# PalamaraLab/FastSMC

Measured on AMD Instinct MI355X. Metric: haplotype-pairs decoded/sec (whole node) + GB/s vs HBM roofline, 69-state HMM, higher is better.
Workload: dtype f32; 1 GPU; synthetic 1000 haplotypes x 50000 sites, K=69, all 499500 pairs per GPU, FastSMC-mode IBD + posterior-mean/MAP ages, no hashing; mode=ibd, resident_waves=2048, n_cu=256, chunk_sites=512, chunks_per_window=98, resident_chunks=24, beta_stride=2, kernel_member=69, record_gather=none, lib_hash=5bd750a2cb04e671

## Files before the change

### fastsmc_amd/capi.py

```python
from __future__ import annotations

import ctypes as C
import os

import numpy as np

_HERE = os.path.dirname(os.path.abspath(__file__))
LIB_PATH = os.environ.get("FSMC_HIP_LIB") or os.path.join(_HERE, "libfastsmc_hip.so")

FSMC_WANT_MEAN = 1
FSMC_WANT_MAP = 2
FSMC_WANT_SUMS = 4
FSMC_WANT_MAJOR_MINOR_SUMS = 8

FSMC_EOVERFLOW = -6

SYMBOLS = [
    "fsmc_ctx_create", "fsmc_ctx_destroy", "fsmc_last_error", "fsmc_ctx_info", "fsmc_ctx_set_workspace_limit",
    "fsmc_ctx_expect_work",
    "fsmc_ctx_set_chunk_sites", "fsmc_ctx_set_beta_stride", "fsmc_ctx_last_beta_stride", "fsmc_ctx_last_plan",
    "fsmc_ctx_last_kernel", "fsmc_ctx_set_pairing", "fsmc_ctx_last_items", "fsmc_ctx_set_two_wave_windows", "fsmc_ctx_last_waves_per_window", "fsmc_ctx_last_segment_sums_in_lds", "fsmc_ctx_set_resident_chunks",
    "fsmc_ctx_last_resident_chunks",
    "fsmc_model_create", "fsmc_model_destroy", "fsmc_haps_upload", "fsmc_worklist_upload",
    "fsmc_decode_ibd_launch", "fsmc_decode_ibd_fetch", "fsmc_sync", "fsmc_last_kernel_ms", "fsmc_phase_cycles",
    "fsmc_decode_ibd",
    "fsmc_decode_posteriors", "fsmc_decode_per_pair", "fsmc_decode_sums", "fsmc_decode_sums_batches",
    "fsmc_decode_pair_posteriors", "fsmc_ctx_set_pair_posterior_slice", "fsmc_ctx_last_pair_posterior_slices",
    "fsmc_decode_pair_minima", "fsmc_ctx_set_pair_minima_slice", "fsmc_ctx_last_pair_minima_slices",
    "fsmc_decode_pair_bins", "fsmc_ctx_set_pair_bins_slice", "fsmc_ctx_last_pair_bins_slices",
    "fsmc_decode_pair_cdf", "fsmc_ctx_set_pair_cdf_slice", "fsmc_ctx_last_pair_cdf_slices",
    "fsmc_decode_pair_tail_summaries", "fsmc_ctx_set_pair_tail_slice", "fsmc_ctx_last_pair_tail_slices",
    "fsmc_decode_pair_loglik", "fsmc_ctx_set_pair_loglik_slice", "fsmc_ctx_last_pair_loglik_slices",
    "fsmc_decode_pair_viterbi", "fsmc_ctx_set_pair_viterbi_slice", "fsmc_ctx_last_pair_viterbi_slices",
    "fsmc_identify", "fsmc_identify_ex", "fsmc_identify_fetch",
]

PAIR_DTYPE = np.dtype([("hap_a", "<u4"), ("hap_b", "<u4")])
GROUP_DTYPE = np.dtype([("first_pair", "<u4"), ("n_pairs", "<u4"), ("from", "<u4"), ("to", "<u4"),
                        ("scan_from", "<u4"), ("scan_to", "<u4")])
CANDIDATE_DTYPE = np.dtype([("hap_a", "<u4"), ("hap_b", "<u4"), ("from", "<u4"), ("to", "<u4"), ("flush_word", "<u4")])
IBD_DTYPE = np.dtype([("pair", "<u4"), ("start", "<i4"), ("end", "<i4"), ("prob", "<f4"), ("post_mean", "<f4"),
                      ("map", "<f4")])


def log_likelihood(mant, expo):
    with np.errstate(divide="ignore"):
        return np.log(np.asarray(mant, np.float64)) + np.asarray(expo, np.float64) * np.log(2.0)


class FsmcError(RuntimeError):
    def __init__(self, code: int, msg: str):
        super().__init__(f"fastsmc_hip error {code}: {msg}")
        self.code = code


class _JobWindow(C.Structure):
    _fields_ = [("window_size", C.c_uint32), ("w_i", C.c_uint32), ("w_j", C.c_uint32), ("last_job", C.c_int32),
                ("j_above_diag", C.c_int32)]


class _IdentifyOpts(C.Structure):
    _fields_ = [("word_size", C.c_uint32), ("haploid", C.c_uint32), ("max_seeds", C.c_int32),
                ("read_ahead", C.c_uint32)]


class _ModelDesc(C.Structure):
    _fields_ = [
        ("K", C.c_int32), ("S", C.c_int32),
        ("pi", C.c_void_p), ("col_ratios", C.c_void_p), ("exp_times", C.c_void_p),
        ("n_rows", C.c_int32),
        ("D", C.c_void_p), ("B", C.c_void_p), ("U", C.c_void_p), ("RR", C.c_void_p),
        ("step_row", C.c_void_p),
        ("e1", C.c_void_p), ("e0m1", C.c_void_p), ("e2m0", C.c_void_p),
        ("state_threshold", C.c_uint32), ("age_threshold", C.c_uint32), ("probability_threshold", C.c_float),
        ("sequence", C.c_int32),
        ("gap_row_f", C.c_void_p), ("site_row_f", C.c_void_p), ("gap_row_b", C.c_void_p), ("site_row_b", C.c_void_p),
        ("hom", C.c_void_p),
    ]


_lib = None


def load():
    global _lib
    if _lib is None:
        if not os.path.exists(LIB_PATH):
            raise FsmcError(-100, f"{LIB_PATH} is missing: build it with `python -c 'import __graft_entry__ as g; "
                                  "g.build()'` (there is no CPU fallback)")
        L = C.CDLL(LIB_PATH)
        vp, i32, u32, u64, sz = C.c_void_p, C.c_int32, C.c_uint32, C.c_uint64, C.c_size_t
        L.fsmc_ctx_create.argtypes = [C.c_int, vp, C.POINTER(vp)]
        L.fsmc_ctx_destroy.argtypes = [vp]
        L.fsmc_ctx_destroy.restype = None
        L.fsmc_last_error.argtypes = [vp]
        L.fsmc_last_error.restype = C.c_char_p
        L.fsmc_ctx_info.argtypes = [vp, C.POINTER(i32), C.POINTER(i32), C.POINTER(u64)]
        L.fsmc_ctx_set_workspace_limit.argtypes = [vp, u64]
        L.fsmc_ctx_expect_work.argtypes = [vp, C.c_double, C.c_int32]
        L.fsmc_ctx_set_chunk_sites.argtypes = [vp, u32]
        L.fsmc_ctx_set_beta_stride.argtypes = [vp, u32]
        L.fsmc_ctx_last_beta_stride.argtypes = [vp, C.POINTER(i32)]
        L.fsmc_ctx_last_plan.argtypes = [vp, C.POINTER(i32), C.POINTER(i32), C.POINTER(i32)]
        L.fsmc_ctx_last_kernel.argtypes = [vp, C.POINTER(i32)]
        L.fsmc_ctx_set_pairing.argtypes = [vp, u32]
        L.fsmc_ctx_set_two_wave_windows.argtypes = [vp, u32]
        L.fsmc_ctx_last_waves_per_window.argtypes = [vp, C.POINTER(i32)]
        L.fsmc_ctx_last_items.argtypes = [vp, C.POINTER(i32)]
        L.fsmc_ctx_last_segment_sums_in_lds.argtypes = [vp, C.POINTER(i32)]
        L.fsmc_model_create.argtypes = [vp, C.POINTER(_ModelDesc), C.POINTER(vp)]
        L.fsmc_model_destroy.argtypes = [vp]
        L.fsmc_model_destroy.restype = None
        L.fsmc_haps_upload.argtypes = [vp, vp, u32, u32]
        L.fsmc_worklist_upload.argtypes = [vp, vp, sz, vp, sz]
        L.fsmc_decode_ibd_launch.argtypes = [vp, vp, u32]
        L.fsmc_decode_ibd_fetch.argtypes = [vp, vp, sz, C.POINTER(sz)]
        L.fsmc_sync.argtypes = [vp]
        L.fsmc_last_kernel_ms.argtypes = [vp, C.POINTER(C.c_float)]
        L.fsmc_phase_cycles.argtypes = [vp, vp, sz]
        L.fsmc_decode_ibd.argtypes = [vp, vp, vp, sz, vp, sz, u32, vp, sz, C.POINTER(sz)]
        L.fsmc_decode_posteriors.argtypes = [vp, vp, vp, sz]
        L.fsmc_decode_per_pair.argtypes = [vp, vp, vp, vp, vp]
        L.fsmc_decode_pair_posteriors.argtypes = [vp, vp, vp, vp, vp]
        L.fsmc_ctx_set_pair_posterior_slice.argtypes = [vp, u32]
        L.fsmc_ctx_last_pair_posterior_slices.argtypes = [vp, C.POINTER(i32)]
        L.fsmc_decode_pair_minima.argtypes = [vp, vp, vp, u64, vp, vp, vp, vp]
        L.fsmc_ctx_set_pair_minima_slice.argtypes = [vp, u32]
        L.fsmc_ctx_last_pair_minima_slices.argtypes = [vp, C.POINTER(i32)]
        L.fsmc_decode_pair_bins.argtypes = [vp, vp, vp, vp, sz, vp, vp, vp, vp, vp]
        L.fsmc_ctx_set_pair_bins_slice.argtypes = [vp, u32]
        L.fsmc_ctx_last_pair_bins_slices.argtypes = [vp, C.POINTER(i32)]
        L.fsmc_decode_pair_cdf.argtypes = [vp, vp, vp, sz, vp, vp, sz, vp]
        L.fsmc_ctx_set_pair_cdf_slice.argtypes = [vp, u32]
        L.fsmc_ctx_last_pair_cdf_slices.argtypes = [vp, C.POINTER(i32)]
        L.fsmc_decode_pair_tail_summaries.argtypes = [vp, vp, vp, sz, vp, vp, sz, vp, vp, vp]
        L.fsmc_ctx_set_pair_tail_slice.argtypes = [vp, u32]
        L.fsmc_ctx_last_pair_tail_slices.argtypes = [vp, C.POINTER(i32)]
        L.fsmc_decode_pair_loglik.argtypes = [vp, vp, vp, sz, vp, vp, vp, vp]
        L.fsmc_ctx_set_pair_loglik_slice.argtypes = [vp, u32]
        L.fsmc_ctx_last_pair_loglik_slices.argtypes = [vp, C.POINTER(i32)]
        L.fsmc_decode_pair_viterbi.argtypes = [vp, vp, vp, vp, vp]
        L.fsmc_ctx_set_pair_viterbi_slice.argtypes = [vp, u32]
        L.fsmc_ctx_last_pair_viterbi_slices.argtypes = [vp, C.POINTER(i32)]
        L.fsmc_decode_sums.argtypes = [vp, vp, vp, vp, vp, vp]
        L.fsmc_decode_sums_batches.argtypes = [vp, vp, vp, sz, vp, vp, vp, vp]
        L.fsmc_identify.argtypes = [vp, vp, u32, u32, vp, C.POINTER(_JobWindow), vp, u32, i32, C.c_float, C.c_float, vp,
                                    sz, C.POINTER(sz)]
        L.fsmc_identify_ex.argtypes = [vp, vp, u32, u32, vp, C.POINTER(_JobWindow), vp, u32, i32, C.c_float, C.c_float,
                                       C.POINTER(_IdentifyOpts), vp, sz, C.POINTER(sz)]
        L.fsmc_identify_fetch.argtypes = [vp, vp, sz, C.POINTER(sz)]
        _lib = L
    return _lib


def _p(a):
    return None if a is None else a.ctypes.data_as(C.c_void_p)


def whole_sequence_groups(n_pairs: int, S: int, batch: int = 64) -> np.ndarray:
    n_groups = (n_pairs + batch - 1) // batch
    g = np.zeros(n_groups, GROUP_DTYPE)
    g["first_pair"] = np.arange(n_groups, dtype=np.uint64) * batch
    g["n_pairs"] = np.minimum(batch, n_pairs - g["first_pair"].astype(np.int64))
    g["from"] = 0
    g["to"] = S
    g["scan_from"] = 0
    g["scan_to"] = S
    return g


class Context:

    def __init__(self, device: int = 0, stream: int | None = None):
        self._L = load()
        h = C.c_void_p()
        rc = self._L.fsmc_ctx_create(device, C.c_void_p(stream) if stream else None, C.byref(h))
        if rc != 0:
            raise FsmcError(rc, (self._L.fsmc_last_error(None) or b"").decode())
        self._h = h
        self._models = []

    def _check(self, rc: int):
        if rc != 0:
            raise FsmcError(rc, (self._L.fsmc_last_error(self._h) or b"").decode())

    def close(self):
        if getattr(self, "_h", None):
            for m in list(self._models):
                m.close()
            self._L.fsmc_ctx_destroy(self._h)
            self._h = None

    def __del__(self):
        try:
            self.close()
        except Exception:
            pass

    def info(self) -> dict:
        cu, slots, hbm = C.c_int32(), C.c_int32(), C.c_uint64()
        self._check(self._L.fsmc_ctx_info(self._h, C.byref(cu), C.byref(slots), C.byref(hbm)))
        chunk, chunks = C.c_int32(), C.c_int32()
        self._check(self._L.fsmc_ctx_last_plan(self._h, C.byref(chunk), C.byref(chunks), None))
        return {"n_cu": cu.value, "n_slots": slots.value, "hbm_bytes": hbm.value, "chunk_sites": chunk.value,
                "max_chunks": chunks.value}

    def set_chunk_sites(self, sites: int):
        self._check(self._L.fsmc_ctx_set_chunk_sites(self._h, sites))

    def set_resident_chunks(self, chunks: int):
        self._check(self._L.fsmc_ctx_set_resident_chunks(self._h, chunks))

    def last_resident_chunks(self) -> int:
        v = C.c_int32(0)
        self._check(self._L.fsmc_ctx_last_resident_chunks(self._h, C.byref(v)))
        return v.value

    def set_beta_stride(self, stride: int):
        self._check(self._L.fsmc_ctx_set_beta_stride(self._h, stride))

    def last_beta_stride(self) -> int:
        v = C.c_int32(0)
        self._check(self._L.fsmc_ctx_last_beta_stride(self._h, C.byref(v)))
        return v.value

    def last_kernel(self) -> int:
        v = C.c_int32(0)
        self._check(self._L.fsmc_ctx_last_kernel(self._h, C.byref(v)))
        return v.value

    def set_two_wave_windows(self, mode: int):
        self._check(self._L.fsmc_ctx_set_two_wave_windows(self._h, mode))

    def last_waves_per_window(self) -> int:
        v = C.c_int32(0)
        self._check(self._L.fsmc_ctx_last_waves_per_window(self._h, C.byref(v)))
        return v.value

    def set_pairing(self, mode: int):
        self._check(self._L.fsmc_ctx_set_pairing(self._h, mode))

    def last_items(self) -> int:
        v = C.c_int32(0)
        self._check(self._L.fsmc_ctx_last_items(self._h, C.byref(v)))
        return v.value

    def last_segment_sums_in_lds(self) -> bool:
        v = C.c_int32(0)
        self._check(self._L.fsmc_ctx_last_segment_sums_in_lds(self._h, C.byref(v)))
        return bool(v.value)

    def set_workspace_limit(self, nbytes: int):
        self._check(self._L.fsmc_ctx_set_workspace_limit(self._h, nbytes))

    def expect_work(self, pair_sites: float, states: int):
        self._check(self._L.fsmc_ctx_expect_work(self._h, float(pair_sites), int(states)))

    def create_model(self, pm) -> "Model":
        return Model(self, pm)

    def upload_haps(self, bits: np.ndarray, n_sites: int):
        b = np.ascontiguousarray(bits, dtype=np.uint64)
        assert b.ndim == 2 and b.shape[1] == (n_sites + 63) // 64
        self._check(self._L.fsmc_haps_upload(self._h, _p(b), b.shape[0], n_sites))

    def upload_worklist(self, pairs: np.ndarray, groups: np.ndarray):
        pr = np.ascontiguousarray(pairs, dtype=PAIR_DTYPE)
        gr = np.ascontiguousarray(groups, dtype=GROUP_DTYPE)
        self._check(self._L.fsmc_worklist_upload(self._h, _p(pr), pr.size, _p(gr), gr.size))
        self._n_pairs = pr.size
        self._groups = gr

    def decode_ibd_launch(self, model: "Model", flags: int = FSMC_WANT_MEAN | FSMC_WANT_MAP):
        self._check(self._L.fsmc_decode_ibd_launch(self._h, model._h, flags))

    def decode_ibd_fetch(self) -> np.ndarray:
        cap = max(1024, 4 * getattr(self, "_n_pairs", 256))
        while True:
            out = np.zeros(cap, IBD_DTYPE)
            n = C.c_size_t()
            rc = self._L.fsmc_decode_ibd_fetch(self._h, _p(out), cap, C.byref(n))
            if rc == FSMC_EOVERFLOW:
                cap = int(n.value)
                continue
            self._check(rc)
            return out[: n.value]

    def sync(self):
        self._check(self._L.fsmc_sync(self._h))

    def last_kernel_ms(self) -> float:
        ms = C.c_float()
        self._check(self._L.fsmc_last_kernel_ms(self._h, C.byref(ms)))
        return float(ms.value)

    def phase_cycles(self) -> np.ndarray:
        out = np.zeros(128, np.uint64)
        if self._L.fsmc_phase_cycles(self._h, _p(out), 128) != 0:
            self._check(self._L.fsmc_phase_cycles(self._h, _p(out), 32))
        return out

    def decode_ibd(self, model: "Model", pairs, groups, flags: int = FSMC_WANT_MEAN | FSMC_WANT_MAP) -> np.ndarray:
        self.upload_worklist(pairs, groups)
        self.decode_ibd_launch(model, flags)
        return self.decode_ibd_fetch()

    def identify(self, words, global_ids, gen_pos, *, window_size=0, w_i=1, w_j=1, last_job=True, j_above_diag=False,
                 gap=1, skip=0.0, min_m=1.0, word_size=64, haploid=True, max_seeds=0, read_ahead=10) -> np.ndarray:
        w = np.ascontiguousarray(words, np.uint64)
        if w.ndim != 2:
            raise ValueError("words must be [n_haps][n_words]")
        ids = np.ascontiguousarray(global_ids, np.uint32)
        gen = np.ascontiguousarray(gen_pos, np.float32)
        if ids.shape != (w.shape[0],):
            raise ValueError("global_ids must have one entry per haplotype")
        jw = _JobWindow(window_size, w_i, w_j, int(bool(last_job)), int(bool(j_above_diag)))
        opts = _IdentifyOpts(word_size, int(bool(haploid)), max_seeds, read_ahead)
        cap = max(1024, 4 * w.shape[0])
        while True:
            out = np.zeros(cap, CANDIDATE_DTYPE)
            n = C.c_size_t(0)
            rc = self._L.fsmc_identify_ex(self._h, _p(w), w.shape[0], w.shape[1], _p(ids), C.byref(jw), _p(gen),
                                          gen.size, gap, skip, min_m, C.byref(opts), _p(out), cap, C.byref(n))
            if rc == -6:
                cap = int(n.value)
                out = np.zeros(cap, CANDIDATE_DTYPE)
                if self._L.fsmc_identify_fetch(self._h, _p(out), cap, C.byref(n)) == 0:
                    return out[:n.value]
                continue
            self._check(rc)
            return out[:n.value]

    def decode_per_pair(self, model: "Model", exp_coal_times, want_mean=True, want_map=True):
        et = np.ascontiguousarray(exp_coal_times, np.float32)
        mean = np.zeros((self._n_pairs, model.S), np.float32) if want_mean else None
        mp = np.zeros((self._n_pairs, model.S), np.int32) if want_map else None
        self._check(self._L.fsmc_decode_per_pair(self._h, model._h, _p(et), _p(mean), _p(mp)))
        return mean, mp

    def decode_pair_posteriors(self, model: "Model", exp_coal_times, want_rows=True, sum_into=None, rows_out=None):
        et = np.ascontiguousarray(exp_coal_times, np.float32)
        if et.shape != (model.K,):
            raise ValueError(f"exp_coal_times: shape {et.shape}, expected {(model.K,)}")
        rows = ptrs = None
        if rows_out is not None:
            rows = rows_out
            if len(rows) != self._n_pairs:
                raise ValueError("rows_out needs one array per pair of the work list")
            for r in rows:
                if r.dtype != np.float32 or not r.flags.c_contiguous or not r.flags.writeable or r.size != model.K * model.S:
                    raise ValueError("rows_out: writable C-contiguous float32 arrays of K * S values")
            ptrs = (C.c_void_p * self._n_pairs)(*[r.ctypes.data for r in rows])
        elif want_rows:
            rows = np.zeros((self._n_pairs, model.K, model.S), np.float32)
            ptrs = (C.c_void_p * self._n_pairs)(*[rows.ctypes.data + i * rows.strides[0] for i in range(self._n_pairs)])
        if sum_into is not None:
            if (sum_into.dtype != np.float32 or not sum_into.flags.c_contiguous or not sum_into.flags.writeable
                    or sum_into.shape != (model.K, model.S)):
                raise ValueError("sum_into: a writable C-contiguous float32 array [K][S]")
        self._check(self._L.fsmc_decode_pair_posteriors(self._h, model._h, _p(et), ptrs, _p(sum_into)))
        return rows, sum_into

    def set_pair_posterior_slice(self, groups: int):
        self._check(self._L.fsmc_ctx_set_pair_posterior_slice(self._h, groups))

    def last_pair_posterior_slices(self) -> int:
        v = C.c_int32(0)
        self._check(self._L.fsmc_ctx_last_pair_posterior_slices(self._h, C.byref(v)))
        return v.value

# ... 265 lines not shown
```

### fastsmc_amd/csrc/fsmc_capi.hip

```cpp
#include <hip/hip_runtime.h>

#include <algorithm>
#include <chrono>
#include <cmath>
#include <cstdio>
#include <cstdlib>
#include <cstring>
#include <new>
#include <string>
#include <type_traits>
#include <vector>

#include "fsmc_identify.h"
#include "fsmc_instances.h"
#include "fsmc_pair_bins.h"
#include "fsmc_pair_cdf.h"
#include "fsmc_pair_tail.h"
#include "fsmc_pair_minima.h"
#include "fsmc_pair_posteriors.h"

namespace fsmc
{
hipError_t idSortCandidates(hipStream_t stream, const fsmc_candidate* in, fsmc_candidate* sorted, unsigned n,
                            unsigned nHaps, unsigned nWords);
hipError_t idSeedDepths(hipStream_t stream, const unsigned long long* words, unsigned nHaps, unsigned nWords,
                        unsigned maxSeeds, unsigned readAhead, unsigned char* depthOut,
                        unsigned hapStride);
}

using namespace fsmc;

namespace fsmc
{
__global__ void add_planes_in_order_kernel(const float* __restrict__ planes, float* __restrict__ acc, size_t n,
                                           int nPlanes, size_t planeStride)
{
  for (size_t i = (size_t)blockIdx.x * blockDim.x + threadIdx.x; i < n; i += (size_t)gridDim.x * blockDim.x) {
    float s = acc[i];
    for (int sl = 0; sl < nPlanes; ++sl) {
      s = s + planes[(size_t)sl * planeStride + i];
    }
    acc[i] = s;
  }
}
}

namespace
{
thread_local std::string g_createError;

struct DevBuf {
  void* p = nullptr;
  size_t bytes = 0;
};

enum PairSlicing {
  kSlicePosteriors,
  kSliceMinima,
  kSliceBins,
  kSliceCdf,
  kSliceTail,
  kSliceLoglik,
  kSliceViterbi,
  kPairSlicings
};
}

struct fsmc_ctx {
  int device = 0;
  hipStream_t stream = nullptr;
  bool ownStream = false;
  int nCU = 0;
  uint64_t hbmBytes = 0;
  uint64_t wsLimit = 0;
  double wsEarned = 0;
  double wsAnnounced = 0;
  double wsAnnouncedCredit = 0;
  std::string err;

  unsigned long long* dHaps = nullptr;
  uint32_t nHaps = 0, nSites = 0, W = 0;

  fsmc_pair* dPairs = nullptr;
  fsmc_group* dGroups = nullptr;
  size_t nPairs = 0, nGroups = 0;
  std::vector<fsmc_pair> hPairs;
  std::vector<fsmc_group> hGroups;

  unsigned* dCounters = nullptr;
  unsigned long long* dPhase = nullptr;
  DevBuf ws;
  DevBuf recs;
  size_t recCap = 0;
  DevBuf aux;
  DevBuf out;

  hipEvent_t ev0 = nullptr, ev1 = nullptr;
  bool timed = false;
  int lastSlots = 0;
  int lastChunk = 0, lastMaxChunks = 0, lastResident = 0;
  int residentChunks = -1;
  uint32_t chunkSites = 0;
  uint32_t betaStride = 0;
  int lastStride = 1;
  bool lastSpsLds = false;
  int lastMember = 0;

  struct IbdQueues {
    uint64_t serial = 0;
    uint64_t maxLen = 0;
    uint64_t maxLenAlone = 0;
    uint32_t pairing = 0;
    bool valid = false;
    bool dual = false;
    bool reordered = false;
    bool alone = false;
    std::vector<fsmc_group> items, unions, rest;
  } q;
  uint64_t worklistSerial = 0;
  fsmc_group* dItems = nullptr;
  fsmc_group* dRest = nullptr;
  uint32_t pairing = 1;
  int lastItems = 0;
  unsigned twoWaves = 0;
  int lastWavesPerWindow = 1;
  hipStream_t side = nullptr;
  hipEvent_t evFork = nullptr, evJoin = nullptr;
  DevBuf wsSide;

  struct {
    uint32_t groups = 0;
    int last = 0;
  } pairSlices[kPairSlicings];
  DevBuf ppStage;
  DevBuf ppRows;
  DevBuf ppAcc;
  hipStream_t copyStream = nullptr;
  void* ppPinned[2] = {nullptr, nullptr};
  size_t ppPinnedBytes = 0;
  hipEvent_t evRows = nullptr, evCopied[2] = {nullptr, nullptr};
  DevBuf pmAcc;
  DevBuf pbAcc;
  DevBuf pcSpec;
  DevBuf plAcc;
  DevBuf pvAcc;
  DevBuf ptAcc;

  DevBuf idStash;
  size_t idStashCount = 0;

  const fsmc_model* ibdModel = nullptr;
  uint32_t ibdFlags = 0;
  bool ibdPending = false;
};

struct fsmc_model {
  fsmc_ctx* ctx = nullptr;
  int K = 0, KP = 0, S = 0, nRows = 0;
  int w2NW = 0;
  float *pi = nullptr, *cR = nullptr, *expT = nullptr;
  float *D = nullptr, *B = nullptr, *U = nullptr, *RR = nullptr;
  float* rowSets = nullptr;
  float* ghostMask = nullptr;
  int* stepRow = nullptr;
  bool sequence = false;
  int *rowGapF = nullptr, *rowSiteB = nullptr, *rowGapB = nullptr;
  float4* emis3 = nullptr;
  unsigned stateThr = 0, ageThr = 0;
  float probThr = 0.f;
};

namespace
{

std::vector<std::string> mappedHipRuntimes()
{
  std::vector<std::string> found;
  if (FILE* f = std::fopen("/proc/self/maps", "r")) {
    char line[4096];
    while (std::fgets(line, sizeof(line), f)) {
      const char* slash = std::strchr(line, '/');
      if (!slash || !std::strstr(slash, "libamdhip64.so")) {
        continue;
      }
      std::string path(slash);
      while (!path.empty() && (path.back() == '\n' || path.back() == ' ')) {
        path.pop_back();
      }
      if (std::find(found.begin(), found.end(), path) == found.end()) {
        found.push_back(path);
      }
    }
    std::fclose(f);
  }
  return found;
}

int fail(fsmc_ctx* ctx, int code, const std::string& msg)
{
  if (ctx) {
    ctx->err = msg;
  } else {
    g_createError = msg;
  }
  return code;
}

#define FSMC_HIP(ctx, call)                                                                                            \
  do {                                                                                                                 \
    hipError_t e_ = (call);                                                                                            \
    if (e_ != hipSuccess) {                                                                                            \
      return fail((ctx), FSMC_EHIP, std::string(#call) + ": " + hipGetErrorString(e_));                                \
    }                                                                                                                  \
  } while (0)

#define FSMC_TRY(call)                                                                                                 \
  do {                                                                                                                 \
    const int rc_ = (call);                                                                                            \
    if (rc_ != FSMC_OK) {                                                                                              \
      return rc_;                                                                                                      \
    }                                                                                                                  \
  } while (0)

int ensure(fsmc_ctx* ctx, DevBuf& b, size_t bytes)
{
  if (b.bytes >= bytes && b.p) {
    return FSMC_OK;
  }
  if (b.p) {
    (void)hipFree(b.p);
    b.p = nullptr;
    b.bytes = 0;
  }
  if (bytes == 0) {
    bytes = 16;
  }
  const bool timing = bytes >= (256u << 20) && std::getenv("FSMC_HOST_TIMING") != nullptr;
  const auto t0 = std::chrono::steady_clock::now();
  hipError_t e = hipMalloc(&b.p, bytes);
  if (e != hipSuccess) {
    b.p = nullptr;
    return fail(ctx, FSMC_ENOMEM, "hipMalloc of " + std::to_string(bytes) + " bytes failed: " + hipGetErrorString(e));
  }
  if (timing) {
    std::fprintf(stderr, "[fsmc] hipMalloc of %.2f GB took %.3f s\n", (double)bytes / 1e9,
                 std::chrono::duration<double>(std::chrono::steady_clock::now() - t0).count());
  }
  b.bytes = bytes;
  return FSMC_OK;
}

template <typename T> int upload(fsmc_ctx* ctx, T** dst, const T* src, size_t n)
{
// ... 1 lines not shown
    (void)hipFree(*dst);
    *dst = nullptr;
  }
  hipError_t e = hipMalloc((void**)dst, std::max<size_t>(n, 1) * sizeof(T));
  if (e != hipSuccess) {
    *dst = nullptr;
    return fail(ctx, FSMC_ENOMEM, std::string("hipMalloc failed: ") + hipGetErrorString(e));
  }
  if (n) {
    FSMC_HIP(ctx, hipMemcpyAsync(*dst, src, n * sizeof(T), hipMemcpyHostToDevice, ctx->stream));
    FSMC_HIP(ctx, hipStreamSynchronize(ctx->stream));
  }
  return FSMC_OK;
}

std::vector<float> padRows(const float* src, size_t rows, int K, int KP)
{
  std::vector<float> out(rows * (size_t)KP, 0.f);
  for (size_t r = 0; r < rows; ++r) {
    std::memcpy(&out[r * KP], src + r * K, sizeof(float) * (size_t)K);
  }
  return out;
}

using KernelFn = void (*)(const KParams);

int familyMember(const fsmc_model* m)
{
  if (exactMember(m->K)) {
    return m->K;
  }
  return (m->K <= 128 && m->KP % kKPad == 0 && m->KP <= 128) ? m->KP : 0;
}

template <int KT> KernelFn pickMember(int mode, bool track, bool seq, bool half, bool dual = false)
{
  if constexpr (KT > 0 && halfBuilt(KT)) {
    if (dual && half && mode == kModeIbd && !seq) {
      return track ? decode_kernel<KT, kModeIbd, true, false, true, true>
                   : decode_kernel<KT, kModeIbd, false, false, true, true>;
    }
  }
  if constexpr (KT > 0) {
    if (dual && mode == kModeIbd && !seq) {
      return track ? decode_kernel<KT, kModeIbd, true, false, false, true>
                   : decode_kernel<KT, kModeIbd, false, false, false, true>;
    }
  }
  switch (mode) {
  case kModeIbd:
    if constexpr (halfBuilt(KT)) {
      if (half && !seq) {
        return track ? decode_kernel<KT, kModeIbd, true, false, true> : decode_kernel<KT, kModeIbd, false, false, true>;
      }
    }
    if (seq) {
      return track ? decode_kernel<KT, kModeIbd, true, true, false> : decode_kernel<KT, kModeIbd, false, true, false>;
    }
    return track ? decode_kernel<KT, kModeIbd, true, false, false> : decode_kernel<KT, kModeIbd, false, false, false>;
  case kModeDump:
    return seq ? decode_kernel<KT, kModeDump, false, true, false> : decode_kernel<KT, kModeDump, false, false, false>;
  case kModePerPair:
    return seq ? decode_kernel<KT, kModePerPair, false, true, false>
               : decode_kernel<KT, kModePerPair, false, false, false>;
  case kModeSums:
    if constexpr (halfSumsBuilt(KT)) {
      if (half && !seq) {
        return decode_kernel<KT, kModeSums, false, false, true>;
      }
    }
    return seq ? decode_kernel<KT, kModeSums, false, true, false> : decode_kernel<KT, kModeSums, false, false, false>;
  default:
    return nullptr;
  }
}

bool waveGroups(int mode, const fsmc_model* m)
{
  return m->w2NW > 0 && (mode == kModeIbd || mode == kModeDump || mode == kModeSums || mode == kModePerPair);
}

struct W2Member {
  int NW, KH;
};
W2Member w2Member(int K)
{
  if (const char* v = std::getenv("FSMC_DIAG_W2_MEMBER")) {
    int nw = 0, kh = 0;
    if (std::sscanf(v, "%dx%d", &nw, &kh) == 2 && nw * kh >= K &&
        ((nw - 1) * kh < K || (kh == 48 && 2 * kh < K) || (nw * kh > 512 && (nw - 2) * kh < K))) {
#define FSMC_IS_W2(KHX, NWX)                                                                                            \
  if (kh == KHX && nw == NWX) {                                                                                        \
    return {nw, kh};                                                                                                   \
  }
      FSMC_ALL_W2(FSMC_IS_W2)
#undef FSMC_IS_W2
    }
  }
  if (K <= 192) return {4, 48};
  if (K <= 256) return {4, 64};
  if (K <= 320) return {4, 80};
  if (K <= 384) return {6, 64};
  if (K <= 448) return {7, 64};
  if (K <= 512) return {8, 64};
  if (K <= 640) return {8, 80};
  if (K <= 768) return {8, 96};
  return {8, 128};
}

template <int KH, int NW, bool SEQ> KernelFn pickWaveGroupKernelOf(int mode, bool track)
{
  if (mode == kModeIbd) {
    return track ? decode_kernel_w2<KH, kModeIbd, true, SEQ, NW> : decode_kernel_w2<KH, kModeIbd, false, SEQ, NW>;
  }
  if (mode == kModeSums) {
    return decode_kernel_w2<KH, kModeSums, false, SEQ, NW>;
  }
  if (mode == kModePerPair) {
    return decode_kernel_w2<KH, kModePerPair, false, SEQ, NW>;
  }
  return decode_kernel_w2<KH, kModeDump, false, SEQ, NW>;
}
template <int KH, int NW> KernelFn pickWaveGroupKernel(int mode, bool track, bool seq)
{
  return seq ? pickWaveGroupKernelOf<KH, NW, true>(mode, track) : pickWaveGroupKernelOf<KH, NW, false>(mode, track);
}

bool anyStates(const fsmc_model* m)
{
  return m->K > kMaxStatesW2;
}

template <bool SEQ> KernelFn pickAnyKernel(int mode, bool track)
{
  switch (mode) {
  case kModeIbd:
    return track ? decode_kernel_any<kModeIbd, true, SEQ> : decode_kernel_any<kModeIbd, false, SEQ>;
  case kModeDump:
    return decode_kernel_any<kModeDump, false, SEQ>;
  case kModePerPair:
    return decode_kernel_any<kModePerPair, false, SEQ>;
  case kModeSums:
    return decode_kernel_any<kModeSums, false, SEQ>;
  default:
    return nullptr;
  }
}

struct KernelChoice {
  KernelFn fn = nullptr;
  unsigned threads = kWave;
  int member = 0;
  int stride = 1;
};

KernelChoice chooseKernel(const fsmc_model* m, int mode, bool track, bool dual, uint32_t wantStride)
{
  KernelChoice k;
  if (anyStates(m)) {
    k.fn = m->sequence ? pickAnyKernel<true>(mode, track) : pickAnyKernel<false>(mode, track);
    return k;
  }
  if (waveGroups(mode, m)) {
    const int NW = m->w2NW, KH = m->KP / NW;
    k.threads = (unsigned)(NW * kWave);
    k.member = NW == kW2NW ? 1000 + KH : 1000 * NW + KH;
#define FSMC_PICK_W2(KHX, NWX)                                                                                          \
  if (KH == KHX && NW == NWX) {                                                                                        \
    k.fn = pickWaveGroupKernel<KHX, NWX>(mode, track, m->sequence != 0);                                               \
  }
    FSMC_ALL_W2(FSMC_PICK_W2)
#undef FSMC_PICK_W2
    return k;
  }
  k.member = familyMember(m);
  const bool half = wantStride != 1 && !m->sequence &&
                    ((mode == kModeIbd && halfBuilt(k.member)) || (mode == kModeSums && halfSumsBuilt(k.member)));
  k.stride = half ? 2 : 1;
  switch (k.member) {
#define FSMC_PICK_CASE(KTX)                                                                                             \
  case KTX:                                                                                                            \
    k.fn = pickMember<KTX>(mode, track, m->sequence, half, dual);                                                      \
    break;
    FSMC_ALL_KT(FSMC_PICK_CASE)
    FSMC_EXACT_KT(FSMC_PICK_CASE)
#undef FSMC_PICK_CASE
  default:
    break;
  }
  return k;
}

template <int KT> KernelFn pickBidirMember(int mode)
{
  switch (mode) {
  case kModeDump:
    return decode_kernel_bidir<KT, kModeDump>;
  case kModePerPair:
    return decode_kernel_bidir<KT, kModePerPair>;
  case kModeSums:
    return decode_kernel_bidir<KT, kModeSums>;
  default:
    return nullptr;
  }
}
KernelChoice chooseTwoWaveKernel(const fsmc_model* m, int mode)
{
  KernelChoice k{nullptr, 2 * kWave, familyMember(m), 1};
  if (m->sequence || anyStates(m) || waveGroups(mode, m)) {
    return k;
  }
  switch (k.member) {
#define FSMC_PICK_BIDIR(KTX)                                                                                            \
  case KTX:                                                                                                            \
    k.fn = pickBidirMember<KTX>(mode);                                                                                 \
    break;
    FSMC_ALL_KT(FSMC_PICK_BIDIR)
    FSMC_EXACT_KT(FSMC_PICK_BIDIR)
#undef FSMC_PICK_BIDIR
  default:
    break;
  }
  return k;
}

template <typename Params> struct SweepKernel {
  KernelChoice k;
  void (*fn)(const Params) = nullptr;
};
template <typename Params, typename Pick> SweepKernel<Params> chooseSweepKernel(const fsmc_model* m, Pick pick)
{
  SweepKernel<Params> s;
  s.k = KernelChoice{nullptr, kWave, m->K <= 128 ? familyMember(m) : 0, 1};
  switch (s.k.member) {
#define FSMC_PICK_SWEEP(KTX)                                                                                            \
  case KTX:                                                                                                            \
    s.fn = pick(std::integral_constant<int, KTX>{});                                                                   \
    break;
    FSMC_ALL_KT(FSMC_PICK_SWEEP)
    FSMC_EXACT_KT(FSMC_PICK_SWEEP)
#undef FSMC_PICK_SWEEP
  default:
    break;
  }
  s.k.fn = reinterpret_cast<KernelFn>(s.fn);
  return s;
}

size_t loweredByEnv(const char* name, size_t value, int divisor = 1)
{
  const char* s = std::getenv(name);
  const long v = s ? std::atol(s) / divisor : 0;
  return v >= 1 && (size_t)v < value ? (size_t)v : value;
}

hipError_t workgroupsPerCU(const KernelChoice& k, int most, int capDivisor, int& perCU)
{
  perCU = 0;
  const hipError_t e = hipOccupancyMaxActiveBlocksPerMultiprocessor(&perCU, k.fn, (int)k.threads, 0);
  if (e != hipSuccess) {
    (void)hipGetLastError();
    return e;
  }
  perCU = std::min(perCU, most);
  if (capDivisor > 0) {
    perCU = (int)loweredByEnv("FSMC_DIAG_WAVES_PER_CU", (size_t)std::max(perCU, 0), capDivisor);
  }
  return hipSuccess;
}

struct LaunchPlan {
  KernelChoice k;
  int chunk = 0;
  int chunkRows = 0;
  int maxChunks = 0;
  int residentChunks = 0;
  size_t wsSlot = 0;
  int slots = 0;
  int wavesPerWindow = 1;
  size_t bytes = 0;
};

constexpr double kAllocBytesPerSecond = 25e9;
constexpr double kEarnFraction = 0.06;
constexpr uint64_t kFreeWorkspace = 24ull << 30;

struct WsBudget {
  uint64_t hard, soft;
};

uint64_t freeWorkspace()
{
  if (const char* v = std::getenv("FSMC_DIAG_WS_FREE")) {
    return std::strtoull(v, nullptr, 10);
  }
  return kFreeWorkspace;
}

WsBudget workspaceBudget(const fsmc_ctx* ctx, const DevBuf& cur)
{
  size_t freeB = 0, totalB = 0;
  const bool known = hipMemGetInfo(&freeB, &totalB) == hipSuccess;
  const uint64_t reachable = (uint64_t)freeB + cur.bytes;
  const uint64_t margin = (uint64_t)(0.04 * (double)ctx->hbmBytes);
  if (ctx->wsLimit) {
    uint64_t lim = ctx->wsLimit;
    if (known && reachable > margin && reachable - margin < lim && reachable - margin >= lim / 4) {
      lim = reachable - margin;
    }
    return {lim, lim};
  }
  const uint64_t floor40 = (uint64_t)(0.40 * (double)ctx->hbmBytes);
  uint64_t hard = floor40;
  if (known) {
    const uint64_t want = (uint64_t)(0.80 * (double)ctx->hbmBytes);
    hard = std::max<uint64_t>(floor40, std::min<uint64_t>(want, reachable > margin ? reachable - margin : 0));
  }
  uint64_t earned = (uint64_t)std::min(std::max(ctx->wsEarned, 0.0), 1e15);
  if (earned < hard && earned < 2 * (uint64_t)cur.bytes) {
    earned = 0;
  }
  const uint64_t freeBytes = freeWorkspace();
  const uint64_t soft = std::min<uint64_t>(hard, std::max<uint64_t>({(uint64_t)cur.bytes, earned, freeBytes}));
  return {hard, soft};
}

void payForWorkspace(fsmc_ctx* ctx, uint64_t allocatedBytes)
{
  if (ctx->wsLimit) {
    return;
  }
  const uint64_t freeBytes = freeWorkspace();
  if (allocatedBytes > freeBytes) {
    ctx->wsEarned = std::max(0.0, ctx->wsEarned - (double)(allocatedBytes - freeBytes));
  }
}

double earnScale()
{
  if (const char* v = std::getenv("FSMC_DIAG_WS_EARN_SCALE")) {
    return std::atof(v);
  }
  return 1.0;
}

void earnWorkspace(fsmc_ctx* ctx, const fsmc_model* m, int mode)
{
  double pairSites = 0;
  for (const fsmc_group& g : ctx->hGroups) {
    const uint32_t aEnd = (mode == kModeIbd) ? g.scan_to : g.to;
    pairSites += (double)g.n_pairs * (double)(aEnd > g.from ? aEnd - g.from : 0);
  }
  double seconds = pairSites * (8.0 * m->K + 0.25) / (0.8 * 8e12);
  const double announced = std::min(ctx->wsAnnounced, seconds);
  if (ctx->wsAnnounced > 0) {
    ctx->wsAnnouncedCredit *= (ctx->wsAnnounced - announced) / ctx->wsAnnounced;
  }
  ctx->wsAnnounced -= announced;
  seconds -= announced;
  ctx->wsEarned += earnScale() * kEarnFraction * seconds * kAllocBytesPerSecond;
}

int planOneWave(const fsmc_ctx* ctx, const fsmc_model* m, int mode, const KernelChoice& k,
                const std::vector<fsmc_group>& list, bool paired, const WsBudget& budget, unsigned share,
                LaunchPlan& plan, std::string& why)
{
  if (!k.fn) {
    why = "no kernel for this model";
    return FSMC_EUNSUPPORTED;
  }
  int perCU = 0;
  const hipError_t e = workgroupsPerCU(k, anyStates(m) ? 4 : 8, 1, perCU);
  if (e != hipSuccess) {
    why = std::string("occupancy query of the decode kernel: ") + hipGetErrorString(e);
    return FSMC_EHIP;
  }
  const bool w2 = waveGroups(mode, m);
  const size_t slots = std::max<size_t>(1, std::min((size_t)ctx->nCU * std::max(perCU, 1), list.size()));
  size_t L = 1;
  for (const fsmc_group& g : list) {
    const size_t aEnd = (mode == kModeIbd) ? g.scan_to : g.to;
    L = std::max<size_t>(L, aEnd - g.from);
  }
  const size_t K4 = w2 ? (size_t)m->KP / 4 : (size_t)((k.member > 0 ? k.member : m->K) + 3) / 4 + (anyStates(m) ? 1 : 0);
  const size_t vecBytes = K4 * kWave * sizeof(float4);
  const uint64_t limit = budget.hard / share;
  const bool half = k.stride == 2;
  auto chunkRows = [&](size_t c) { return half ? (c + 1) / 2 : c; };
  const size_t rowsAvail = (size_t)(limit / (vecBytes * slots));
  const size_t rowsSoft = (size_t)(budget.soft / share / (vecBytes * slots));
  const size_t sideRows = anyStates(m) ? (size_t)kAnyExtraRows + 2 : 4;
  const size_t defaultChunk = std::max<size_t>((size_t)std::ceil(std::sqrt((double)L)), w2 ? 2048 : 512);
  size_t C, maxChunks;
  if (chunkRows(L) + sideRows + 1 <= rowsAvail && (chunkRows(L) + sideRows + 1 <= rowsSoft || L <= defaultChunk) &&
      !(ctx->chunkSites && ctx->chunkSites < L)) {
    C = L;
    maxChunks = 1;
  } else {
    C = ctx->chunkSites ? (size_t)ctx->chunkSites : defaultChunk;
    C = std::min((C + 15) / 16 * 16, (L + 15) / 16 * 16);
    auto fits = [&](size_t c) { return chunkRows(c) + (L + c - 1) / c + sideRows + 1 <= rowsAvail; };
    if (!ctx->chunkSites) {
      while (C > 16 && !fits(C)) {
        C = std::max<size_t>(16, (C / 2 + 15) / 16 * 16);
      }
    }
    maxChunks = (L + C - 1) / C;
    if (!fits(C)) {
      why = "workspace limit too small for the decode window";
      return FSMC_ENOMEM;
    }
  }
  size_t resident = 0;
  if (maxChunks > 1 && (mode == kModeIbd || mode == kModeSums) && !m->sequence && !paired && !anyStates(m) &&
      (!w2 || w2ResidentBuilt(m->w2NW, false)) &&
      ctx->residentChunks != 0) {
    const size_t rowsBudget = rowsSoft;
    const size_t fixed = chunkRows(C) + maxChunks + sideRows;
    if (rowsBudget > fixed) {
      resident = std::min<size_t>((rowsBudget - fixed) / chunkRows(C), maxChunks);
      if (ctx->residentChunks > 0) {
        resident = std::min<size_t>(resident, (size_t)ctx->residentChunks);
      }
    }
  }
  plan.chunk = (int)C;
  plan.chunkRows = (int)chunkRows(C);
  plan.maxChunks = (int)maxChunks;
  plan.residentChunks = (int)resident;
  plan.wsSlot = (chunkRows(C) * (1 + resident) + maxChunks + 2 + (sideRows - 2)) * K4 * kWave;
  plan.slots = (int)slots;
  plan.k = k;
  plan.wavesPerWindow = 1;
  plan.bytes = plan.wsSlot * sizeof(float4) * slots;
  return FSMC_OK;
}

int planViterbi(const fsmc_ctx* ctx, const fsmc_model* m, const KernelChoice& k, size_t nGroups, bool wantStates,
                const WsBudget& budget, LaunchPlan& plan, std::string& why)
{
  int perCU = 0;
  const hipError_t e = workgroupsPerCU(k, 8, 1, perCU);
  if (e != hipSuccess) {
    why = std::string("occupancy query of the Viterbi kernel: ") + hipGetErrorString(e);
    return FSMC_EHIP;
  }
  size_t slots = std::max<size_t>(1, std::min((size_t)ctx->nCU * (size_t)std::max(perCU, 1), nGroups));
  const size_t L = (size_t)m->S;
  const size_t K4 = (size_t)(k.member + 3) / 4;
  const size_t psiRow = K4 * kWave * sizeof(uint32_t), ckptRow = K4 * kWave * sizeof(float4);
  auto slotBytes = [&](size_t c) { return c * psiRow + (L + c - 1) / c * ckptRow; };
  size_t C = L, bytes = psiRow;
  if (wantStates) {
    size_t cMin = std::min(L, std::max<size_t>(1, (size_t)std::ceil(2.0 * std::sqrt((double)L))));
    if (ctx->chunkSites) {
      cMin = std::min<size_t>(ctx->chunkSites, L);
    }
    slots = std::min<size_t>(slots, (size_t)(budget.hard / slotBytes(cMin)));
    if (slots == 0) {
      why = "workspace limit too small for the back-pointers of one wave";
      return FSMC_ENOMEM;
    }
    if (ctx->chunkSites) {
      C = cMin;
    } else {
      const uint64_t room = L <= 512 ? budget.hard : budget.soft;
      while (C > cMin && (uint64_t)slots * slotBytes(C) > room) {
        C = std::max(cMin, (C + 1) / 2);
      }
    }
    bytes = slotBytes(C);
  }
  plan = LaunchPlan();
  plan.k = k;
  plan.chunk = (int)C;
  plan.chunkRows = (int)C;
  plan.maxChunks = (int)((L + C - 1) / C);
  plan.wsSlot = bytes / sizeof(float4);
  plan.slots = (int)slots;
  plan.wavesPerWindow = 1;
  plan.bytes = bytes * slots;
  return FSMC_OK;
}

bool twoWavesWanted(const fsmc_ctx* ctx, const KernelChoice& k2, size_t nItems)
{
  if (ctx->twoWaves == 1 || nItems == 0 || !k2.fn) {
    return false;
  }
  if (const char* v = std::getenv("FSMC_DIAG_TWO_WAVE_WINDOWS")) {
    if (std::strcmp(v, "never") == 0) {
      return false;
    }
  }
  int perCU = 0;
  return workgroupsPerCU(k2, 4, 2, perCU) == hipSuccess && perCU >= 1 && nItems <= (size_t)ctx->nCU * perCU;
}

bool planTwoWaves(const fsmc_ctx* ctx, const KernelChoice& k2, size_t nItems, const WsBudget& budget, LaunchPlan& plan)
{
  size_t L = 1;
  for (const fsmc_group& g : ctx->hGroups) {
    L = std::max<size_t>(L, g.to - g.from);
  }
  const size_t K4 = (size_t)(k2.member + 3) / 4;
  plan = LaunchPlan();
  plan.k = k2;
  plan.chunk = (int)L;
  plan.chunkRows = (int)L;
  plan.maxChunks = 1;
  plan.wsSlot = L * K4 * kWave;
  plan.slots = (int)nItems;
  plan.wavesPerWindow = 2;
  plan.bytes = plan.wsSlot * sizeof(float4) * nItems;
  return plan.bytes <= budget.hard && (plan.bytes <= budget.soft || L <= 512);
}

int holdWorkspace(fsmc_ctx* ctx, DevBuf& buf, size_t bytes)
{
  const char* most = std::getenv("FSMC_DIAG_WS_ALLOC_MAX");
  if (most && bytes > std::strtoull(most, nullptr, 10) && !(buf.p && buf.bytes >= bytes)) {
    if (buf.p) {
      (void)hipFree(buf.p);
    }
    buf = DevBuf();
    return fail(ctx, FSMC_ENOMEM, "workspace of " + std::to_string(bytes) + " bytes refused (FSMC_DIAG_WS_ALLOC_MAX)");
  }
  const size_t held = buf.bytes;
  const int rc = ensure(ctx, buf, bytes);
  if (rc != FSMC_OK) {
    (void)hipGetLastError();
  } else if (buf.bytes != held) {
    payForWorkspace(ctx, buf.bytes);
  }
  return rc;
}

int planAndHold(fsmc_ctx* ctx, const fsmc_model* m, int mode, const KernelChoice& k, const std::vector<fsmc_group>& list,
                bool paired, unsigned share, DevBuf& buf, LaunchPlan& plan)
{
  std::string why;
  const int rc = planOneWave(ctx, m, mode, k, list, paired, workspaceBudget(ctx, buf), share, plan, why);
  return rc != FSMC_OK ? fail(ctx, rc, why) : holdWorkspace(ctx, buf, plan.bytes);
}

void recordLaunch(fsmc_ctx* ctx, const KernelChoice& k, const LaunchPlan& plan, int slotsBeside = 0)
{
  ctx->lastMember = k.member;
  ctx->lastStride = k.stride;
  ctx->lastChunk = plan.chunk;
  ctx->lastMaxChunks = plan.maxChunks;
  ctx->lastResident = plan.residentChunks;
  ctx->lastWavesPerWindow = plan.wavesPerWindow;
  ctx->lastSlots = plan.slots + slotsBeside;
}

int checkReady(fsmc_ctx* ctx, const fsmc_model* m)
{
  if (!ctx || !m) {
    return fail(ctx, FSMC_EINVAL, "null context or model");
  }
  if (m->ctx != ctx) {
    return fail(ctx, FSMC_EINVAL, "model belongs to another context");
  }
  if (!ctx->dHaps) {
    return fail(ctx, FSMC_ESTATE, "no haplotypes uploaded (fsmc_haps_upload)");
  }
  if (!ctx->dPairs || !ctx->dGroups || ctx->nGroups == 0) {
    return fail(ctx, FSMC_ESTATE, "no work list uploaded (fsmc_worklist_upload)");
  }
  if ((uint32_t)m->S != ctx->nSites) {
    return fail(ctx, FSMC_EINVAL, "model has " + std::to_string(m->S) + " sites but haplotypes have " +
                                      std::to_string(ctx->nSites));
  }
  for (const fsmc_pair& pr : ctx->hPairs) {
    if (pr.hap_a >= ctx->nHaps || pr.hap_b >= ctx->nHaps) {
      return fail(ctx, FSMC_EINVAL, "pair refers to a haplotype row outside the uploaded matrix");
    }
  }
  for (const fsmc_group& g : ctx->hGroups) {
    if (g.to > (uint32_t)m->S) {
      return fail(ctx, FSMC_EINVAL, "group window exceeds the number of sites");
    }
  }
  if (m->K > kMaxStatesAny) {
    return fail(ctx, FSMC_EUNSUPPORTED, "more than " + std::to_string(kMaxStatesAny) + " states");
  }
  return FSMC_OK;
}

void fillParams(const fsmc_ctx* ctx, const fsmc_model* m, const LaunchPlan& plan, uint32_t flags, KParams& p)
{
  std::memset(&p, 0, sizeof(p));
  p.K = m->K;
  p.KP = m->KP;
  p.S = m->S;
  p.W = (int)ctx->W;
  p.nGroups = (int)ctx->nGroups;
  p.chunk = plan.chunk;
  p.chunkRows = plan.chunkRows;
  p.maxChunks = plan.maxChunks;
  p.residentChunks = plan.residentChunks;
  p.flags = flags;
  p.pi = m->pi;
  p.cR = m->cR;
  p.expT = m->expT;
  p.D = m->D;
  p.B = m->B;
  p.U = m->U;
  p.rowSets = m->rowSets;
  p.RR = m->RR;
  p.ghostMask = m->ghostMask;
  p.stepRow = m->stepRow;
  p.rowGapF = m->rowGapF;
  p.rowSiteB = m->rowSiteB;
  p.rowGapB = m->rowGapB;
  p.emis3 = m->emis3;
  p.haps = ctx->dHaps;
  p.pairs = ctx->dPairs;
  p.groups = ctx->dGroups;
  p.counters = ctx->dCounters;
  p.phaseCycles = ctx->dPhase;
  p.ws = (float4*)ctx->ws.p;
  p.wsSlot = plan.wsSlot;
  p.stateThr = m->stateThr;
  p.ageThr = m->ageThr;
  p.spsLds = 0u;
  p.thr[0] = 1000 * m->probThr;
  p.thr[1] = 100 * m->probThr;
  p.thr[2] = 10 * m->probThr;
  p.thr[3] = m->probThr;
  p.recs = (fsmc_ibd_record*)ctx->recs.p;
  p.recCap = (unsigned)ctx->recCap;
}

int checkWorkspace(fsmc_ctx* ctx, const KParams& p, int slots)
{
  const DevBuf& buf = p.ws == (float4*)ctx->wsSide.p ? ctx->wsSide : ctx->ws;
  if (!p.ws || p.ws != (float4*)buf.p || slots < 1 || buf.bytes / sizeof(float4) / (size_t)slots < p.wsSlot) {
    return fail(ctx, FSMC_ESTATE, "the workspace does not hold the launch planned for it");
  }
  return FSMC_OK;
}

int launch(fsmc_ctx* ctx, const KernelChoice& k, const KParams& p, int slots, size_t dynLds = 0, bool continues = false)
{
  if (checkWorkspace(ctx, p, slots) != FSMC_OK) {
    return FSMC_ESTATE;
  }
  FSMC_HIP(ctx, hipMemsetAsync(ctx->dCounters, 0, 4 * sizeof(unsigned), ctx->stream));
  if (!continues) {
    FSMC_HIP(ctx, hipEventRecord(ctx->ev0, ctx->stream));
  }
  hipLaunchKernelGGL(k.fn, dim3((unsigned)slots), dim3(k.threads), dynLds, ctx->stream, p);
  FSMC_HIP(ctx, hipGetLastError());
  FSMC_HIP(ctx, hipEventRecord(ctx->ev1, ctx->stream));
  ctx->timed = true;
  return FSMC_OK;
}

int launchBeside(fsmc_ctx* ctx, const KernelChoice& kSide, KParams& pSide, int slotsSide, const KernelChoice& kMain,
                 KParams& pMain, int slotsMain)
{
  if (checkWorkspace(ctx, pSide, slotsSide) != FSMC_OK || checkWorkspace(ctx, pMain, slotsMain) != FSMC_OK) {
    return FSMC_ESTATE;
  }
  FSMC_HIP(ctx, hipMemsetAsync(ctx->dCounters, 0, 4 * sizeof(unsigned), ctx->stream));
  FSMC_HIP(ctx, hipEventRecord(ctx->ev0, ctx->stream));
  FSMC_HIP(ctx, hipEventRecord(ctx->evFork, ctx->stream));
  FSMC_HIP(ctx, hipStreamWaitEvent(ctx->side, ctx->evFork, 0));
  pMain.groupBase = 0;
  pSide.groupBase = 2;
  hipLaunchKernelGGL(kSide.fn, dim3((unsigned)slotsSide), dim3(kSide.threads), 0, ctx->side, pSide);
  FSMC_HIP(ctx, hipGetLastError());
  hipLaunchKernelGGL(kMain.fn, dim3((unsigned)slotsMain), dim3(kMain.threads), 0, ctx->stream, pMain);
  FSMC_HIP(ctx, hipGetLastError());
  FSMC_HIP(ctx, hipEventRecord(ctx->evJoin, ctx->side));
  FSMC_HIP(ctx, hipStreamWaitEvent(ctx->stream, ctx->evJoin, 0));
  FSMC_HIP(ctx, hipEventRecord(ctx->ev1, ctx->stream));
  ctx->timed = true;
  return FSMC_OK;
}

uint64_t stagingLimit(const fsmc_ctx* ctx, uint64_t held, unsigned parts)
{
  uint64_t limit = ctx->wsLimit ? ctx->wsLimit : (uint64_t)(0.25 * (double)ctx->hbmBytes);
  size_t freeB = 0, totalB = 0;
  if (hipMemGetInfo(&freeB, &totalB) == hipSuccess) {
    const uint64_t room = (uint64_t)freeB + held;
    const uint64_t reserve = 2ull << 30;
    limit = std::min<uint64_t>(limit, room > reserve ? (room - reserve) / parts : 0);
  }
  return limit;
}

int ensureRowCopies(fsmc_ctx* ctx, size_t need)
{
  if (ctx->ppPinnedBytes < need) {
    for (int i = 0; i < 2; ++i) {
      if (ctx->ppPinned[i]) {
        (void)hipHostFree(ctx->ppPinned[i]);
        ctx->ppPinned[i] = nullptr;
      }
    }
    ctx->ppPinnedBytes = 0;
    for (int i = 0; i < 2; ++i) {
      const hipError_t e = hipHostMalloc(&ctx->ppPinned[i], need, hipHostMallocDefault);
      if (e != hipSuccess) {
        ctx->ppPinned[i] = nullptr;
        return fail(ctx, FSMC_ENOMEM, std::string("hipHostMalloc of the row buffers failed: ") + hipGetErrorString(e));
      }
    }
    ctx->ppPinnedBytes = need;
  }
  if (!ctx->copyStream) {
    FSMC_HIP(ctx, hipStreamCreateWithFlags(&ctx->copyStream, hipStreamNonBlocking));
    FSMC_HIP(ctx, hipEventCreateWithFlags(&ctx->evRows, hipEventDisableTiming));
    FSMC_HIP(ctx, hipEventCreateWithFlags(&ctx->evCopied[0], hipEventDisableTiming));
    FSMC_HIP(ctx, hipEventCreateWithFlags(&ctx->evCopied[1], hipEventDisableTiming));
  }
  return FSMC_OK;
}

int prepareDecode(fsmc_ctx* ctx, const fsmc_model* m, int mode, uint32_t wantStride,
                  const std::vector<fsmc_group>& list, size_t nItems, size_t stagingPerItem, LaunchPlan& plan)
{
  const KernelChoice k = chooseKernel(m, mode, false, false, wantStride);
  earnWorkspace(ctx, m, mode);
  int rc = planAndHold(ctx, m, mode, k, list, false, 1, ctx->ws, plan);
  if (rc != FSMC_OK) {
    return rc;
  }
  size_t staged = nItems;
  if (stagingPerItem) {
    staged = std::max<size_t>(1, (size_t)(stagingLimit(ctx, ctx->out.bytes, 1) / stagingPerItem));
    staged = loweredByEnv("FSMC_DIAG_SUMS_SLOTS", staged);
    plan.slots = (int)std::min({(size_t)plan.slots, nItems, staged});
  }
  const KernelChoice k2 = chooseTwoWaveKernel(m, mode);
  LaunchPlan plan2;
  if (staged >= nItems && twoWavesWanted(ctx, k2, nItems) &&
      planTwoWaves(ctx, k2, nItems, workspaceBudget(ctx, ctx->ws), plan2)) {
    if (holdWorkspace(ctx, ctx->ws, plan2.bytes) == FSMC_OK) {
      plan = plan2;
    } else {
      ctx->err.clear();
      rc = holdWorkspace(ctx, ctx->ws, plan.bytes);
      if (rc != FSMC_OK) {
        return rc;
      }
    }
  }
  recordLaunch(ctx, plan.k, plan);
  return FSMC_OK;
}

int setPairSlice(fsmc_ctx* ctx, PairSlicing kind, uint32_t groups)
{
  if (!ctx) {
    return FSMC_EINVAL;
  }
  ctx->pairSlices[kind].groups = groups;
  return FSMC_OK;
}

int lastPairSlices(const fsmc_ctx* ctx, PairSlicing kind, int32_t* slices)
{
  if (!ctx || !slices) {
    return FSMC_EINVAL;
  }
  *slices = ctx->pairSlices[kind].last;
  return FSMC_OK;
}

struct WorkSlices {
  const fsmc_ctx* ctx = nullptr;
  size_t slice = 0;
  size_t nSlices = 0;
  size_t slicePairsMax = 0;
  LaunchPlan plan;
  float* stageMean = nullptr;
  int* stageMap = nullptr;
  std::vector<size_t> hOffsets;
  std::vector<float> hCoal;

  size_t firstGroup(size_t sl) const { return sl * slice; }
  size_t groups(size_t sl) const { return std::min(slice, ctx->nGroups - sl * slice); }
  size_t firstPair(size_t sl) const { return ctx->hGroups[firstGroup(sl)].first_pair; }
  size_t pairs(size_t sl) const
  {
    const fsmc_group& last = ctx->hGroups[firstGroup(sl) + groups(sl) - 1];
    return (size_t)last.first_pair + last.n_pairs - firstPair(sl);
// ... 289 lines not shown
      return fail(nullptr, code, msg);
    }
  }
  *out = ctx;
  return FSMC_OK;
}

void fsmc_ctx_destroy(fsmc_ctx* ctx)
{
  if (!ctx) {
    return;
  }
  (void)hipSetDevice(ctx->device);
  if (ctx->stream) {
    (void)hipStreamSynchronize(ctx->stream);
  }
  if (ctx->dHaps) (void)hipFree(ctx->dHaps);
  if (ctx->dPairs) (void)hipFree(ctx->dPairs);
  if (ctx->dGroups) (void)hipFree(ctx->dGroups);
  if (ctx->dItems) (void)hipFree(ctx->dItems);
  if (ctx->dRest) (void)hipFree(ctx->dRest);
  if (ctx->dCounters) (void)hipFree(ctx->dCounters);
  if (ctx->dPhase) (void)hipFree(ctx->dPhase);
  if (ctx->idStash.p) (void)hipFree(ctx->idStash.p);
  if (ctx->ws.p) (void)hipFree(ctx->ws.p);
  if (ctx->recs.p) (void)hipFree(ctx->recs.p);
  if (ctx->aux.p) (void)hipFree(ctx->aux.p);
  if (ctx->out.p) (void)hipFree(ctx->out.p);
  if (ctx->ev0) (void)hipEventDestroy(ctx->ev0);
  if (ctx->ev1) (void)hipEventDestroy(ctx->ev1);
  if (ctx->evFork) (void)hipEventDestroy(ctx->evFork);
  if (ctx->evJoin) (void)hipEventDestroy(ctx->evJoin);
  if (ctx->side) (void)hipStreamDestroy(ctx->side);
  if (ctx->wsSide.p) (void)hipFree(ctx->wsSide.p);
  if (ctx->copyStream) (void)hipStreamSynchronize(ctx->copyStream);
  if (ctx->ppStage.p) (void)hipFree(ctx->ppStage.p);
  if (ctx->ppRows.p) (void)hipFree(ctx->ppRows.p);
  if (ctx->pcSpec.p) (void)hipFree(ctx->pcSpec.p);
  if (ctx->ptAcc.p) (void)hipFree(ctx->ptAcc.p);
  if (ctx->ppAcc.p) (void)hipFree(ctx->ppAcc.p);
  if (ctx->pmAcc.p) (void)hipFree(ctx->pmAcc.p);
  if (ctx->pbAcc.p) (void)hipFree(ctx->pbAcc.p);
  if (ctx->plAcc.p) (void)hipFree(ctx->plAcc.p);
  if (ctx->pvAcc.p) (void)hipFree(ctx->pvAcc.p);
  for (int i = 0; i < 2; ++i) {
    if (ctx->ppPinned[i]) (void)hipHostFree(ctx->ppPinned[i]);
    if (ctx->evCopied[i]) (void)hipEventDestroy(ctx->evCopied[i]);
  }
  if (ctx->evRows) (void)hipEventDestroy(ctx->evRows);
  if (ctx->copyStream) (void)hipStreamDestroy(ctx->copyStream);
  if (ctx->ownStream && ctx->stream) (void)hipStreamDestroy(ctx->stream);
  delete ctx;
}

int fsmc_ctx_info(const fsmc_ctx* ctx, int32_t* n_cu, int32_t* n_slots, uint64_t* hbm_bytes)
{
  if (!ctx) {
    return FSMC_EINVAL;
  }
  if (n_cu) *n_cu = ctx->nCU;
  if (n_slots) *n_slots = ctx->lastSlots;
  if (hbm_bytes) *hbm_bytes = ctx->hbmBytes;
  return FSMC_OK;
}

int fsmc_ctx_set_workspace_limit(fsmc_ctx* ctx, uint64_t bytes)
{
  if (!ctx) {
    return FSMC_EINVAL;
  }
  ctx->wsLimit = bytes;
  return FSMC_OK;
}

int fsmc_ctx_expect_work(fsmc_ctx* ctx, double pair_sites, int32_t states)
{
  if (!ctx) {
    return fail(nullptr, FSMC_EINVAL, "null context");
  }
  if (!(pair_sites >= 0) || states < 1) {
    return fail(ctx, FSMC_EINVAL, "expected work: pair-sites >= 0 and states >= 1");
  }
  if (pair_sites == 0) {
    ctx->wsEarned = std::max(0.0, ctx->wsEarned - ctx->wsAnnouncedCredit);
    ctx->wsAnnounced = 0;
    ctx->wsAnnouncedCredit = 0;
    return FSMC_OK;
  }
  const double seconds = pair_sites * (8.0 * states + 0.25) / (0.8 * 8e12);
  const double credit = std::min(earnScale() * kEarnFraction * seconds * kAllocBytesPerSecond,
                                 std::max(0.0, (double)ctx->hbmBytes - ctx->wsAnnouncedCredit));
  ctx->wsAnnounced += seconds;
  ctx->wsAnnouncedCredit += credit;
  ctx->wsEarned += credit;
  return FSMC_OK;
}

int fsmc_ctx_set_chunk_sites(fsmc_ctx* ctx, uint32_t sites)
{
  if (!ctx) {
    return FSMC_EINVAL;
  }
  ctx->chunkSites = sites;
  return FSMC_OK;
}

int fsmc_ctx_set_beta_stride(fsmc_ctx* ctx, uint32_t stride)
{
  if (!ctx || stride > 2) {
    return fail(ctx, FSMC_EINVAL, "beta stride must be 0 (automatic), 1 or 2");
  }
  ctx->betaStride = stride;
  return FSMC_OK;
}

int fsmc_ctx_last_beta_stride(const fsmc_ctx* ctx, int32_t* stride)
{
  if (!ctx || !stride) {
    return FSMC_EINVAL;
  }
  *stride = ctx->lastStride;
  return FSMC_OK;
}

int fsmc_ctx_last_plan(const fsmc_ctx* ctx, int32_t* chunk_sites, int32_t* max_chunks, int32_t* n_slots)
{
  if (!ctx) {
    return FSMC_EINVAL;
  }
  if (chunk_sites) *chunk_sites = ctx->lastChunk;
  if (max_chunks) *max_chunks = ctx->lastMaxChunks;
  if (n_slots) *n_slots = ctx->lastSlots;
  return FSMC_OK;
}

int fsmc_ctx_set_resident_chunks(fsmc_ctx* ctx, int32_t chunks)
{
  if (!ctx || chunks < -1) {
    return fail(ctx, FSMC_EINVAL, "resident chunks: -1 (automatic), 0 (none) or a count");
  }
  ctx->residentChunks = chunks;
  return FSMC_OK;
}

int fsmc_ctx_last_resident_chunks(const fsmc_ctx* ctx, int32_t* chunks)
{
  if (!ctx || !chunks) {
    return FSMC_EINVAL;
  }
  *chunks = ctx->lastResident;
  return FSMC_OK;
}

int fsmc_ctx_set_pair_posterior_slice(fsmc_ctx* ctx, uint32_t groups) { return setPairSlice(ctx, kSlicePosteriors, groups); }
int fsmc_ctx_last_pair_posterior_slices(const fsmc_ctx* ctx, int32_t* slices) { return lastPairSlices(ctx, kSlicePosteriors, slices); }
int fsmc_ctx_set_pair_minima_slice(fsmc_ctx* ctx, uint32_t groups) { return setPairSlice(ctx, kSliceMinima, groups); }
int fsmc_ctx_last_pair_minima_slices(const fsmc_ctx* ctx, int32_t* slices) { return lastPairSlices(ctx, kSliceMinima, slices); }
int fsmc_ctx_set_pair_bins_slice(fsmc_ctx* ctx, uint32_t groups) { return setPairSlice(ctx, kSliceBins, groups); }
int fsmc_ctx_last_pair_bins_slices(const fsmc_ctx* ctx, int32_t* slices) { return lastPairSlices(ctx, kSliceBins, slices); }
int fsmc_ctx_set_pair_cdf_slice(fsmc_ctx* ctx, uint32_t groups) { return setPairSlice(ctx, kSliceCdf, groups); }
int fsmc_ctx_last_pair_cdf_slices(const fsmc_ctx* ctx, int32_t* slices) { return lastPairSlices(ctx, kSliceCdf, slices); }
int fsmc_ctx_set_pair_tail_slice(fsmc_ctx* ctx, uint32_t groups) { return setPairSlice(ctx, kSliceTail, groups); }
int fsmc_ctx_last_pair_tail_slices(const fsmc_ctx* ctx, int32_t* slices) { return lastPairSlices(ctx, kSliceTail, slices); }
int fsmc_ctx_set_pair_loglik_slice(fsmc_ctx* ctx, uint32_t groups) { return setPairSlice(ctx, kSliceLoglik, groups); }
int fsmc_ctx_last_pair_loglik_slices(const fsmc_ctx* ctx, int32_t* slices) { return lastPairSlices(ctx, kSliceLoglik, slices); }
int fsmc_ctx_set_pair_viterbi_slice(fsmc_ctx* ctx, uint32_t groups) { return setPairSlice(ctx, kSliceViterbi, groups); }
int fsmc_ctx_last_pair_viterbi_slices(const fsmc_ctx* ctx, int32_t* slices) { return lastPairSlices(ctx, kSliceViterbi, slices); }

int fsmc_ctx_last_kernel(const fsmc_ctx* ctx, int32_t* member)
{
  if (!ctx || !member) {
    return FSMC_EINVAL;
  }
  *member = ctx->lastMember;
  return FSMC_OK;
}

int fsmc_model_create(fsmc_ctx* ctx, const fsmc_model_desc* d, fsmc_model** out)
{
  if (!ctx || !d || !out) {
    return fail(ctx, FSMC_EINVAL, "null argument");
  }
  *out = nullptr;
  if (d->K < 2 || d->S < 1 || d->n_rows < 1) {
    return fail(ctx, FSMC_EINVAL, "need K >= 2, S >= 1, n_rows >= 1");
  }
  if (d->K > kMaxStatesAny) {
    return fail(ctx, FSMC_EUNSUPPORTED, "more than " + std::to_string(kMaxStatesAny) + " states");
  }
  if (!d->pi || !d->col_ratios || !d->exp_times || !d->D || !d->B || !d->U || !d->RR || !d->step_row || !d->e1 ||
      !d->e0m1 || !d->e2m0) {
    return fail(ctx, FSMC_EINVAL, "null table pointer in model description");
  }
  if (d->state_threshold > (uint32_t)d->K || d->age_threshold > (uint32_t)d->K) {
    return fail(ctx, FSMC_EINVAL, "state/age threshold larger than K");
  }
  const bool seq = d->sequence != 0;
  if (seq && (!d->gap_row_f || !d->site_row_f || !d->gap_row_b || !d->site_row_b || !d->hom)) {
    return fail(ctx, FSMC_EINVAL, "sequence mode needs gap_row_f, site_row_f, gap_row_b, site_row_b and hom");
  }
  const int32_t* rowArrays[5] = {d->step_row, seq ? d->gap_row_f : nullptr, seq ? d->site_row_f : nullptr,
                                 seq ? d->gap_row_b : nullptr, seq ? d->site_row_b : nullptr};
  static const char* const rowNames[5] = {"step_row", "gap_row_f", "site_row_f", "gap_row_b", "site_row_b"};
  for (int a = 0; a < 5; ++a) {
    for (int32_t s = 1; rowArrays[a] && s < d->S; ++s) {
      if (rowArrays[a][s] < 0 || rowArrays[a][s] >= d->n_rows) {
        return fail(ctx, FSMC_EINVAL,
                    std::string(rowNames[a]) + "[" + std::to_string(s) + "] outside the transition tables");
      }
    }
  }
  FSMC_HIP(ctx, hipSetDevice(ctx->device));
  fsmc_model* m = new (std::nothrow) fsmc_model();
  if (!m) {
    return fail(ctx, FSMC_ENOMEM, "host allocation failed");
  }
  m->ctx = ctx;
  m->K = d->K;
  m->KP = (d->K + kKPad - 1) / kKPad * kKPad;
  if (d->K > 128 && d->K <= kMaxStatesW2) {
    const W2Member w = w2Member(d->K);
    m->w2NW = w.NW;
    m->KP = w.NW * w.KH;
  }
  m->S = d->S;
  m->nRows = d->n_rows;
  m->stateThr = d->state_threshold;
  m->ageThr = d->age_threshold;
  m->probThr = d->probability_threshold;
  const int K = m->K, KP = m->KP;
  int rc = FSMC_OK;
  auto up = [&](float** dst, const float* src, size_t rows) {
    if (rc == FSMC_OK) {
      std::vector<float> padded = padRows(src, rows, K, KP);
      rc = upload(ctx, dst, padded.data(), padded.size());
    }
  };
  up(&m->pi, d->pi, 1);
  up(&m->cR, d->col_ratios, 1);
  up(&m->expT, d->exp_times, 1);
  up(&m->D, d->D, (size_t)d->n_rows);
  up(&m->B, d->B, (size_t)d->n_rows);
  up(&m->U, d->U, (size_t)d->n_rows);
  up(&m->RR, d->RR, (size_t)d->n_rows);
  if (rc == FSMC_OK) {
    const size_t n = (size_t)d->n_rows;
    std::vector<float> rs(n * kRowSetParts * (size_t)KP, 0.f);
    for (size_t r = 0; r < n; ++r) {
      float* q = &rs[r * kRowSetParts * KP];
      for (int k = 0; k < K; ++k) {
        q[kRowD * KP + k] = d->D[r * K + k];
        q[kRowB * KP + k] = d->B[r * K + k];
        q[kRowU * KP + k] = d->U[r * K + k];
        q[kRowRR * KP + k] = d->RR[r * K + k];
        if (k >= 1) {
          q[kRowUsh * KP + k] = d->U[r * K + (k - 1)];
        }
      }
    }
    rc = upload(ctx, &m->rowSets, rs.data(), rs.size());
  }
  if (rc == FSMC_OK) {
    std::vector<float> mask((size_t)KP, 0.f);
    std::fill(mask.begin(), mask.begin() + K, 1.0f);
    rc = upload(ctx, &m->ghostMask, mask.data(), mask.size());
  }
  m->sequence = seq;
  auto upRows = [&](int** dst, const int32_t* src) {
    if (rc == FSMC_OK) {
      std::vector<int> rows(src, src + d->S);
      rows[0] = 0;
      rc = upload(ctx, dst, rows.data(), rows.size());
    }
  };
  upRows(&m->stepRow, seq ? d->site_row_f : d->step_row);
  if (seq) {
    upRows(&m->rowGapF, d->gap_row_f);
    upRows(&m->rowSiteB, d->site_row_b);
    upRows(&m->rowGapB, d->gap_row_b);
  }
  if (rc == FSMC_OK) {
    const int NC = seq ? 4 : 3;
    std::vector<float> emis((size_t)d->S * NC * KP, 0.f);
    static const float zs[3] = {0.f, 1.f, 1.f};
    static const float ts[3] = {0.f, 0.f, 1.f};
    for (int32_t s = 0; s < d->S; ++s) {
      for (int c = 0; c < 3; ++c) {
        float* dst = &emis[((size_t)s * NC + c) * KP];
        const volatile float z = zs[c];
        const volatile float t = ts[c];
        for (int k = 0; k < K; ++k) {
          const size_t i = (size_t)s * K + k;
          dst[k] = d->e1[i] + d->e0m1[i] * z + d->e2m0[i] * t;
        }
      }
      if (seq) {
        float* dst = &emis[((size_t)s * NC + 3) * KP];
        const volatile float zero = 0.f;
        for (int k = 0; k < K; ++k) {
          const float h = d->hom[(size_t)s * K + k];
          dst[k] = h + h * zero + h * zero;
        }
      }
    }
    rc = upload(ctx, (float**)&m->emis3, emis.data(), emis.size());
  }
// ... 139 lines not shown
    }
    const fsmc_group& a = groups[g];
    if (a.n_pairs <= 32 && a.to - a.from <= maxLen) {
      fsmc_group none = a;
      none.n_pairs = 0;
      items.push_back(a);
      items.push_back(none);
      unions.push_back(a);
    } else {
      rest.push_back(a);
    }
  }
  std::vector<uint32_t> order(unions.size());
  for (size_t i = 0; i < order.size(); ++i) {
    order[i] = (uint32_t)i;
  }
  std::stable_sort(order.begin(), order.end(), [&](uint32_t x, uint32_t y) {
    return unions[x].scan_to - unions[x].from > unions[y].scan_to - unions[y].from;
  });
  std::vector<fsmc_group> items2(items.size()), unions2(unions.size());
  for (size_t i = 0; i < order.size(); ++i) {
    unions2[i] = unions[order[i]];
    items2[2 * i] = items[2 * order[i]];
    items2[2 * i + 1] = items[2 * order[i] + 1];
  }
  items.swap(items2);
  unions.swap(unions2);
  return true;
}

bool longestFirst(std::vector<fsmc_group>& list)
{
  auto len = [](const fsmc_group& g) { return g.scan_to - g.from; };
  bool ordered = true;
  for (size_t i = 1; i < list.size() && ordered; ++i) {
    ordered = len(list[i]) <= len(list[i - 1]);
  }
  if (ordered) {
    return false;
  }
  std::stable_sort(list.begin(), list.end(), [&](const fsmc_group& a, const fsmc_group& b) { return len(a) > len(b); });
  return true;
}
}

int fsmc_ctx_set_pairing(fsmc_ctx* ctx, uint32_t mode)
{
  if (!ctx || mode > 1) {
    return fail(ctx, FSMC_EINVAL, "pairing must be 0 (off) or 1 (automatic)");
  }
  ctx->pairing = mode;
  return FSMC_OK;
}

int fsmc_ctx_set_two_wave_windows(fsmc_ctx* ctx, uint32_t mode)
{
  if (!ctx || mode > 1) {
    return fail(ctx, FSMC_EINVAL, "two-wave windows: 0 (automatic) or 1 (never)");
  }
  ctx->twoWaves = mode;
  return FSMC_OK;
}

int fsmc_ctx_last_waves_per_window(const fsmc_ctx* ctx, int32_t* waves)
{
  if (!ctx || !waves) {
    return FSMC_EINVAL;
  }
  *waves = ctx->lastWavesPerWindow;
  return FSMC_OK;
}

int fsmc_ctx_last_items(const fsmc_ctx* ctx, int32_t* n_items)
{
  if (!ctx || !n_items) {
    return FSMC_EINVAL;
  }
  *n_items = ctx->lastItems;
  return FSMC_OK;
}

int fsmc_ctx_last_segment_sums_in_lds(const fsmc_ctx* ctx, int32_t* in_lds)
{
  if (!ctx || !in_lds) {
    return FSMC_EINVAL;
  }
  *in_lds = ctx->lastSpsLds ? 1 : 0;
  return FSMC_OK;
}

int fsmc_decode_ibd_launch(fsmc_ctx* ctx, const fsmc_model* m, uint32_t flags)
{
  int rc = checkReady(ctx, m);
  if (rc != FSMC_OK) {
    return rc;
  }
  FSMC_HIP(ctx, hipSetDevice(ctx->device));
  const bool track = (flags & (FSMC_WANT_MEAN | FSMC_WANT_MAP)) != 0;
  earnWorkspace(ctx, m, kModeIbd);
  KernelChoice kDual;
  uint64_t maxLen = 0, maxLenAlone = 0;
  if (ctx->pairing != 0 && !m->sequence && familyMember(m) > 0) {
    kDual = chooseKernel(m, kModeIbd, track, true, ctx->betaStride);
    maxLen = maxLenAlone = 1u << 30;
  }
  fsmc_ctx::IbdQueues& q = ctx->q;
  if (!q.valid || q.serial != ctx->worklistSerial || q.maxLen != maxLen || q.maxLenAlone != maxLenAlone ||
      q.pairing != ctx->pairing) {
    q.valid = false;
    q.items.clear();
    q.unions.clear();
    q.rest.clear();
    q.dual = maxLenAlone > 0 && buildDualItems(ctx->hGroups, (uint32_t)maxLenAlone, q.items, q.unions, q.rest);
    q.alone = q.dual && q.rest.empty();
    if (q.dual && !q.alone) {
      q.items.clear();
      q.unions.clear();
      q.rest.clear();
      q.dual = maxLen > 0 && buildDualItems(ctx->hGroups, (uint32_t)maxLen, q.items, q.unions, q.rest);
    }
    if (!q.dual) {
      q.items.clear();
      q.unions.clear();
      q.rest = ctx->hGroups;
    }
    q.reordered = longestFirst(q.rest) || q.dual;
    if (q.dual) {
      rc = upload(ctx, &ctx->dItems, q.items.data(), q.items.size());
      if (rc != FSMC_OK) {
        return rc;
      }
    }
    if (q.reordered && !q.rest.empty()) {
      rc = upload(ctx, &ctx->dRest, q.rest.data(), q.rest.size());
      if (rc != FSMC_OK) {
        return rc;
      }
    }
    q.serial = ctx->worklistSerial;
    q.maxLen = maxLen;
    q.maxLenAlone = maxLenAlone;
    q.pairing = ctx->pairing;
    q.valid = true;
  }
  const bool haveRest = !q.rest.empty();
  const bool beside = q.dual && haveRest;
  LaunchPlan planDual, plan;
  if (q.dual) {
    rc = planAndHold(ctx, m, kModeIbd, kDual, q.unions, true, q.alone ? 1 : 2, ctx->ws, planDual);
    if (rc != FSMC_OK) {
      return rc;
    }
  }
  const KernelChoice k = chooseKernel(m, kModeIbd, track, false, ctx->betaStride);
  if (haveRest) {
    rc = planAndHold(ctx, m, kModeIbd, k, q.reordered ? q.rest : ctx->hGroups, false, beside ? 2 : 1,
                     beside ? ctx->wsSide : ctx->ws, plan);
    if (rc != FSMC_OK) {
      return rc;
    }
  }
  recordLaunch(ctx, k, haveRest ? plan : planDual, beside ? planDual.slots : 0);
  ctx->lastItems = q.dual ? (int)q.unions.size() : 0;
  if (ctx->recCap == 0) {
    ctx->recCap = std::max<size_t>(1u << 16, 8 * ctx->nPairs);
  }
  rc = ensure(ctx, ctx->recs, ctx->recCap * sizeof(fsmc_ibd_record));
  if (rc != FSMC_OK) {
    return rc;
  }
  KParams pDual, p;
  if (q.dual) {
    fillParams(ctx, m, planDual, flags, pDual);
    pDual.groups = ctx->dItems;
    pDual.nGroups = (int)q.unions.size();
  }
  if (haveRest) {
    fillParams(ctx, m, plan, flags, p);
    if (q.reordered) {
      p.groups = ctx->dRest;
      p.nGroups = (int)q.rest.size();
    }
    if (beside) {
      p.ws = (float4*)ctx->wsSide.p;
    }
  }
  size_t spsLdsBytes = 0;
  if (!beside && !q.dual && track && !waveGroups(kModeIbd, m) && !anyStates(m) && !m->sequence) {
    const size_t dyn = (size_t)(k.member + 3) / 4 * kWave * sizeof(float4);
    hipFuncAttributes fa;
    FSMC_HIP(ctx, hipFuncGetAttributes(&fa, reinterpret_cast<const void*>(k.fn)));
    const size_t perWave = fa.sharedSizeBytes + dyn;
    constexpr size_t kLdsPerCU = 160u << 10, kLdsPerWorkgroup = 64u << 10;
    if (perWave <= kLdsPerWorkgroup && (size_t)plan.slots * perWave <= (size_t)ctx->nCU * kLdsPerCU &&
        (size_t)plan.slots <= (size_t)ctx->nCU * (kLdsPerCU / perWave) && !std::getenv("FSMC_DIAG_NO_SPS_LDS")) {
      spsLdsBytes = dyn;
      p.spsLds = 1u;
    }
  }
  ctx->lastSpsLds = spsLdsBytes != 0;
  rc = beside ? launchBeside(ctx, k, p, plan.slots, kDual, pDual, planDual.slots)
              : q.dual ? launch(ctx, kDual, pDual, planDual.slots) : launch(ctx, k, p, plan.slots, spsLdsBytes);
  if (rc != FSMC_OK) {
    return rc;
  }
  ctx->ibdModel = m;
  ctx->ibdFlags = flags;
  ctx->ibdPending = true;
  return FSMC_OK;
}

int fsmc_identify(fsmc_ctx* ctx, const uint64_t* words, uint32_t n_haps, uint32_t n_words, const uint32_t* global_ids,
                  const fsmc_job_window* job, const float* gen_pos, uint32_t n_sites, int32_t gap, float skip,
                  float min_m, fsmc_candidate* out, size_t cap, size_t* n_out)
{
  const fsmc_identify_opts defaults = {64u, 1u, 0, 10u};
  return fsmc_identify_ex(ctx, words, n_haps, n_words, global_ids, job, gen_pos, n_sites, gap, skip, min_m, &defaults,
                          out, cap, n_out);
}

int fsmc_identify_ex(fsmc_ctx* ctx, const uint64_t* words, uint32_t n_haps, uint32_t n_words,
                     const uint32_t* global_ids, const fsmc_job_window* job, const float* gen_pos, uint32_t n_sites,
                     int32_t gap, float skip, float min_m, const fsmc_identify_opts* opts, fsmc_candidate* out,
                     size_t cap, size_t* n_out)
{
  if (!ctx) {
    return FSMC_EINVAL;
  }
  if (!opts) {
    return fail(ctx, FSMC_EINVAL, "fsmc_identify: opts is null");
  }
  if (opts->word_size < 1 || opts->word_size > 64) {
    return fail(ctx, FSMC_EINVAL, "fsmc_identify: word_size must be 1..64 (a word is one 64-bit integer)");
  }
  const bool splitSeeds = opts->max_seeds > 0;
  if (splitSeeds && (opts->read_ahead < 1 || opts->read_ahead > 32)) {
    return fail(ctx, FSMC_EINVAL, "fsmc_identify: read_ahead must be 1..32 when max_seeds is set");
  }
  if (!opts->haploid && (n_haps & 1u)) {
    return fail(ctx, FSMC_EINVAL, "fsmc_identify: haploid = 0 pairs rows 2k, 2k+1 -- n_haps must be even");
  }
  if (!n_out) {
    return fail(ctx, FSMC_EINVAL, "fsmc_identify: n_out is null");
  }
  *n_out = 0;
  if (n_haps < 2 || n_words == 0) {
    return FSMC_OK;
  }
  if (!words || !global_ids || !job || !gen_pos || (cap && !out)) {
    return fail(ctx, FSMC_EINVAL, "fsmc_identify: null argument");
  }
  if ((uint64_t)n_words * opts->word_size > n_sites) {
    return fail(ctx, FSMC_EINVAL, "fsmc_identify: n_words * word_size exceeds n_sites");
  }
  if (gap < 0 || cap > 0xFFFFFFFFull) {
    return fail(ctx, FSMC_EINVAL, "fsmc_identify: gap < 0 or cap beyond 2^32");
  }
  FSMC_HIP(ctx, hipSetDevice(ctx->device));
  const unsigned tiles = (n_haps + kIdTile - 1) / kIdTile;
  const unsigned chunks = (n_words + kIdChunk - 1) / kIdChunk;
  struct Bufs {
    void* p[8] = {};
    ~Bufs()
    {
      for (void* q : p) {
        if (q) {
          (void)hipFree(q);
        }
      }
    }
  } b;
  const size_t bytes[8] = {(size_t)n_haps * n_words * sizeof(uint64_t),
                           (size_t)n_haps * sizeof(uint32_t),
                           (size_t)n_sites * sizeof(float),
                           (size_t)chunks * tiles * kIdTile * sizeof(unsigned),
                           (size_t)chunks * sizeof(unsigned),
                           std::max<size_t>(cap, 1) * sizeof(fsmc_candidate),
                           sizeof(unsigned),
                           splitSeeds ? (size_t)chunks * kIdChunk * tiles * kIdTile : 16};
  for (int i = 0; i < 8; ++i) {
    const hipError_t e = hipMalloc(&b.p[i], bytes[i]);
    if (e != hipSuccess) {
      b.p[i] = nullptr;
      return fail(ctx, FSMC_ENOMEM, std::string("fsmc_identify: hipMalloc failed: ") + hipGetErrorString(e));
    }
  }
  FSMC_HIP(ctx, hipMemcpyAsync(b.p[0], words, bytes[0], hipMemcpyHostToDevice, ctx->stream));
  FSMC_HIP(ctx, hipMemcpyAsync(b.p[1], global_ids, bytes[1], hipMemcpyHostToDevice, ctx->stream));
  FSMC_HIP(ctx, hipMemcpyAsync(b.p[2], gen_pos, bytes[2], hipMemcpyHostToDevice, ctx->stream));
  FSMC_HIP(ctx, hipMemsetAsync(b.p[3], 0, bytes[3], ctx->stream));
  FSMC_HIP(ctx, hipMemsetAsync(b.p[6], 0, bytes[6], ctx->stream));
  IdParams p;
  p.words = (const unsigned long long*)b.p[0];
  p.nHaps = n_haps;
  p.nWords = n_words;
  p.globalId = (const unsigned*)b.p[1];
  p.job = *job;
  p.gen = (const float*)b.p[2];
  p.nSites = n_sites;
  p.gap = (int)std::min<uint32_t>((uint32_t)gap, n_words);
  p.skip = skip;
  p.minM = min_m;
  p.dupBits = (unsigned*)b.p[3];
  p.hapStride = tiles * kIdTile;
  p.usedBits = (unsigned*)b.p[4];
  p.out = (fsmc_candidate*)b.p[5];
  p.cap = (unsigned)cap;
  p.count = (unsigned*)b.p[6];
  p.wordSize = opts->word_size;
  p.depth = splitSeeds ? (const unsigned char*)b.p[7] : nullptr;
  const bool general = splitSeeds || !opts->haploid;
  const bool haploid = opts->haploid != 0;
  auto launchMatch = [&]() {
    if (!general) {
      hipLaunchKernelGGL(id_match_kernel, dim3(tiles, tiles), dim3(kIdThreads), 0, ctx->stream, p);
    } else if (haploid) {
      hipLaunchKernelGGL(id_match_general_kernel<true>, dim3(tiles, tiles), dim3(kIdThreads), 0, ctx->stream, p);
    } else {
      hipLaunchKernelGGL(id_match_general_kernel<false>, dim3(tiles, tiles), dim3(kIdThreads), 0, ctx->stream, p);
    }
    return hipGetLastError();
  };
  FSMC_HIP(ctx, hipEventRecord(ctx->ev0, ctx->stream));
  if (splitSeeds) {
    FSMC_HIP(ctx, hipMemsetAsync(b.p[7], 0, bytes[7], ctx->stream));
    const hipError_t e = idSeedDepths(ctx->stream, p.words, n_haps, n_words, (unsigned)opts->max_seeds, opts->read_ahead,
                                      (unsigned char*)b.p[7], p.hapStride);
    if (e != hipSuccess) {
      return fail(ctx, e == hipErrorOutOfMemory ? FSMC_ENOMEM : FSMC_EHIP,
                  std::string("fsmc_identify: splitting the seeds failed: ") + hipGetErrorString(e));
    }
  }
  hipLaunchKernelGGL(id_dup_kernel, dim3(tiles, tiles), dim3(kIdThreads), 0, ctx->stream, p);
  FSMC_HIP(ctx, hipGetLastError());
  hipLaunchKernelGGL(id_complexity_kernel, dim3(chunks), dim3(kIdThreads), 0, ctx->stream, p);
  FSMC_HIP(ctx, hipGetLastError());
  FSMC_HIP(ctx, launchMatch());
// ... 968 lines not shown
```

### fastsmc_amd/csrc/fsmc_inst.hip

```cpp
#include "fsmc_instances.h"

namespace fsmc
{
#if defined(FSMC_INSTANCE_KT)
FSMC_KT_KERNELS(FSMC_DEFINE_KT, FSMC_INSTANCE_KT)
FSMC_KT_BIDIR_KERNELS(FSMC_DEFINE_KT_BIDIR, FSMC_INSTANCE_KT)
#if FSMC_INSTANCE_KT > 0
FSMC_DEFINE_KT_DUAL(FSMC_INSTANCE_KT)
#endif
static_assert(halfBuilt(FSMC_INSTANCE_KT), "not a member of the library: add it to FSMC_ALL_KT or FSMC_EXACT_KT");
FSMC_KT_HALF_KERNELS(FSMC_DEFINE_KT, FSMC_INSTANCE_KT)
#if FSMC_INSTANCE_KT != 50
FSMC_KT_HALF_SUMS_KERNELS(FSMC_DEFINE_KT, FSMC_INSTANCE_KT)
#endif
FSMC_DEFINE_KT_DUAL_HALF(FSMC_INSTANCE_KT)
FSMC_KT_FWD_KERNELS(FSMC_DEFINE_KT_FWD, FSMC_INSTANCE_KT)
FSMC_KT_VITERBI_KERNELS(FSMC_DEFINE_KT_VITERBI, FSMC_INSTANCE_KT)
#elif defined(FSMC_INSTANCE_W2)
#ifndef FSMC_INSTANCE_NW
#define FSMC_INSTANCE_NW 4
#endif
#if !defined(FSMC_INSTANCE_SEQ)
FSMC_W2_KERNELS(FSMC_DEFINE_W2, FSMC_INSTANCE_W2, FSMC_INSTANCE_NW)
#elif FSMC_INSTANCE_SEQ
FSMC_W2_MODE_KERNELS(FSMC_DEFINE_W2, FSMC_INSTANCE_W2, FSMC_INSTANCE_NW, true)
#else
FSMC_W2_MODE_KERNELS(FSMC_DEFINE_W2, FSMC_INSTANCE_W2, FSMC_INSTANCE_NW, false)
#endif
#else
#error "define FSMC_INSTANCE_KT or FSMC_INSTANCE_W2"
#endif
}
```

### fastsmc_amd/csrc/fsmc_instances.h

```cpp
#pragma once

#include "fsmc_kernels.h"
#include "fsmc_kernels_any.h"
#include "fsmc_kernels_bidir.h"
#include "fsmc_kernels_w2.h"
#include "fsmc_pair_loglik.h"
#include "fsmc_pair_viterbi.h"

namespace fsmc
{

#ifndef FSMC_EXACT_KT
#define FSMC_EXACT_KT(Y) Y(50) Y(100)
#endif
#define FSMC_IS_EXACT_TERM(KTX) || KT == KTX
constexpr bool exactMember(const int KT)
{
  return KT == 69 FSMC_EXACT_KT(FSMC_IS_EXACT_TERM);
}

constexpr bool halfSumsBuilt(const int KT);
constexpr bool halfBuilt(const int KT)
{
  return KT == 16 || KT == 32 || KT == 48 || KT == 64 || KT == 80 || KT == 96 || KT == 112 || KT == 128 || exactMember(KT);
}

constexpr bool halfSumsBuilt(const int KT)
{
  return halfBuilt(KT) && KT != 50;
}

#define FSMC_KT_KERNELS(X, KT)                                                                                         \
  X(KT, kModeIbd, true, false, false)                                                                                  \
  X(KT, kModeIbd, false, false, false)                                                                                 \
  X(KT, kModeIbd, true, true, false)                                                                                   \
  X(KT, kModeIbd, false, true, false)                                                                                  \
  X(KT, kModeDump, false, false, false)                                                                                \
  X(KT, kModeDump, false, true, false)                                                                                 \
  X(KT, kModePerPair, false, false, false)                                                                             \
  X(KT, kModePerPair, false, true, false)                                                                              \
  X(KT, kModeSums, false, false, false)                                                                                \
  X(KT, kModeSums, false, true, false)
#define FSMC_KT_HALF_KERNELS(X, KT)                                                                                    \
  X(KT, kModeIbd, true, false, true)                                                                                   \
  X(KT, kModeIbd, false, false, true)
#define FSMC_KT_HALF_SUMS_KERNELS(X, KT) X(KT, kModeSums, false, false, true)

#define FSMC_DECLARE_KT(KT, MODE, TRACK, SEQ, HALF)                                                                    \
  extern template __global__ void decode_kernel<KT, MODE, TRACK, SEQ, HALF>(const KParams);
#define FSMC_DEFINE_KT(KT, MODE, TRACK, SEQ, HALF)                                                                     \
  template __global__ void decode_kernel<KT, MODE, TRACK, SEQ, HALF>(const KParams);
#define FSMC_KT_BIDIR_KERNELS(X, KT) X(KT, kModeDump) X(KT, kModePerPair) X(KT, kModeSums)
#define FSMC_DECLARE_KT_BIDIR(KT, MODE) extern template __global__ void decode_kernel_bidir<KT, MODE>(const KParams);
#define FSMC_DEFINE_KT_BIDIR(KT, MODE) template __global__ void decode_kernel_bidir<KT, MODE>(const KParams);
#define FSMC_DECLARE_KT_DUAL(KT)                                                                                       \
  extern template __global__ void decode_kernel<KT, kModeIbd, true, false, false, true>(const KParams);              \
  extern template __global__ void decode_kernel<KT, kModeIbd, false, false, false, true>(const KParams);
#define FSMC_DEFINE_KT_DUAL(KT)                                                                                        \
  template __global__ void decode_kernel<KT, kModeIbd, true, false, false, true>(const KParams);                     \
  template __global__ void decode_kernel<KT, kModeIbd, false, false, false, true>(const KParams);
#define FSMC_DECLARE_KT_DUAL_HALF(KT)                                                                                  \
  extern template __global__ void decode_kernel<KT, kModeIbd, true, false, true, true>(const KParams);               \
  extern template __global__ void decode_kernel<KT, kModeIbd, false, false, true, true>(const KParams);
#define FSMC_DEFINE_KT_DUAL_HALF(KT)                                                                                   \
  template __global__ void decode_kernel<KT, kModeIbd, true, false, true, true>(const KParams);                      \
  template __global__ void decode_kernel<KT, kModeIbd, false, false, true, true>(const KParams);
#define FSMC_KT_FWD_KERNELS(X, KT) X(KT, false) X(KT, true)
#define FSMC_DECLARE_KT_FWD(KT, SEQ) extern template __global__ void forward_kernel<KT, SEQ>(const FwdParams);
#define FSMC_DEFINE_KT_FWD(KT, SEQ) template __global__ void forward_kernel<KT, SEQ>(const FwdParams);
#define FSMC_KT_VITERBI_KERNELS(X, KT) X(KT)
#define FSMC_DECLARE_KT_VITERBI(KT) extern template __global__ void viterbi_kernel<KT>(const VitParams);
#define FSMC_DEFINE_KT_VITERBI(KT) template __global__ void viterbi_kernel<KT>(const VitParams);
#define FSMC_W2_MODE_KERNELS(X, KH, NW, SEQ)                                                                           \
  X(KH, kModeIbd, true, SEQ, NW)                                                                                       \
  X(KH, kModeIbd, false, SEQ, NW)                                                                                      \
  X(KH, kModeDump, false, SEQ, NW)                                                                                     \
  X(KH, kModeSums, false, SEQ, NW)                                                                                     \
  X(KH, kModePerPair, false, SEQ, NW)
#define FSMC_W2_KERNELS(X, KH, NW) FSMC_W2_MODE_KERNELS(X, KH, NW, false) FSMC_W2_MODE_KERNELS(X, KH, NW, true)
#define FSMC_DECLARE_W2(KH, MODE, TRACK, SEQ, NW)                                                                      \
  extern template __global__ void decode_kernel_w2<KH, MODE, TRACK, SEQ, NW>(const KParams);
#define FSMC_DEFINE_W2(KH, MODE, TRACK, SEQ, NW)                                                                       \
  template __global__ void decode_kernel_w2<KH, MODE, TRACK, SEQ, NW>(const KParams);

#define FSMC_ALL_KT(Y) Y(16) Y(32) Y(48) Y(64) Y(69) Y(80) Y(96) Y(112) Y(128)
#define FSMC_ALL_W2(Y) Y(48, 4) Y(64, 4) Y(80, 4) Y(64, 6) Y(64, 7) Y(64, 8) Y(80, 8) Y(96, 8) Y(128, 8)

#if !defined(FSMC_INSTANCE_KT) && !defined(FSMC_INSTANCE_W2)
#define FSMC_DECLARE_MEMBER(KT)                                                                                         \
  FSMC_KT_KERNELS(FSMC_DECLARE_KT, KT)                                                                                  \
  FSMC_KT_BIDIR_KERNELS(FSMC_DECLARE_KT_BIDIR, KT) FSMC_KT_FWD_KERNELS(FSMC_DECLARE_KT_FWD, KT)                        \
  FSMC_KT_VITERBI_KERNELS(FSMC_DECLARE_KT_VITERBI, KT)
FSMC_ALL_KT(FSMC_DECLARE_MEMBER)
#define FSMC_DECLARE_EXACT_MEMBER(KT)                                                                                   \
  static_assert(KT % 16 != 0 && KT <= 128, "an exact member is not a multiple of 16 states and has at most 128");       \
  FSMC_KT_KERNELS(FSMC_DECLARE_KT, KT)                                                                                  \
  FSMC_KT_BIDIR_KERNELS(FSMC_DECLARE_KT_BIDIR, KT)                                                                      \
  FSMC_KT_FWD_KERNELS(FSMC_DECLARE_KT_FWD, KT)                                                                          \
  FSMC_KT_VITERBI_KERNELS(FSMC_DECLARE_KT_VITERBI, KT)                                                                  \
  FSMC_KT_HALF_KERNELS(FSMC_DECLARE_KT, KT)                                                                             \
  FSMC_KT_HALF_SUMS_KERNELS(FSMC_DECLARE_KT, KT)                                                                        \
  FSMC_DECLARE_KT_DUAL_HALF(KT)                                                                                         \
  FSMC_DECLARE_KT_DUAL(KT)
FSMC_EXACT_KT(FSMC_DECLARE_EXACT_MEMBER)
FSMC_KT_HALF_KERNELS(FSMC_DECLARE_KT, 16) FSMC_KT_HALF_SUMS_KERNELS(FSMC_DECLARE_KT, 16)
FSMC_KT_HALF_KERNELS(FSMC_DECLARE_KT, 32) FSMC_KT_HALF_SUMS_KERNELS(FSMC_DECLARE_KT, 32)
FSMC_KT_HALF_KERNELS(FSMC_DECLARE_KT, 48) FSMC_KT_HALF_SUMS_KERNELS(FSMC_DECLARE_KT, 48)
FSMC_KT_HALF_KERNELS(FSMC_DECLARE_KT, 64) FSMC_KT_HALF_SUMS_KERNELS(FSMC_DECLARE_KT, 64)
FSMC_KT_HALF_KERNELS(FSMC_DECLARE_KT, 69) FSMC_KT_HALF_SUMS_KERNELS(FSMC_DECLARE_KT, 69)
FSMC_KT_HALF_KERNELS(FSMC_DECLARE_KT, 80) FSMC_KT_HALF_SUMS_KERNELS(FSMC_DECLARE_KT, 80)
FSMC_KT_HALF_KERNELS(FSMC_DECLARE_KT, 96) FSMC_KT_HALF_SUMS_KERNELS(FSMC_DECLARE_KT, 96)
FSMC_KT_HALF_KERNELS(FSMC_DECLARE_KT, 112) FSMC_KT_HALF_SUMS_KERNELS(FSMC_DECLARE_KT, 112)
FSMC_KT_HALF_KERNELS(FSMC_DECLARE_KT, 128) FSMC_KT_HALF_SUMS_KERNELS(FSMC_DECLARE_KT, 128)
FSMC_DECLARE_KT_DUAL_HALF(16)
FSMC_DECLARE_KT_DUAL_HALF(32)
FSMC_DECLARE_KT_DUAL_HALF(48)
FSMC_DECLARE_KT_DUAL_HALF(64)
FSMC_DECLARE_KT_DUAL_HALF(69)
FSMC_DECLARE_KT_DUAL_HALF(80)
FSMC_DECLARE_KT_DUAL_HALF(96)
FSMC_DECLARE_KT_DUAL_HALF(112)
FSMC_DECLARE_KT_DUAL_HALF(128)
FSMC_DECLARE_KT_DUAL(16)
FSMC_DECLARE_KT_DUAL(32)
FSMC_DECLARE_KT_DUAL(48)
FSMC_DECLARE_KT_DUAL(64)
FSMC_DECLARE_KT_DUAL(69)
FSMC_DECLARE_KT_DUAL(80)
FSMC_DECLARE_KT_DUAL(96)
FSMC_DECLARE_KT_DUAL(112)
FSMC_DECLARE_KT_DUAL(128)
#define FSMC_DECLARE_W2_MEMBER(KH, NW) FSMC_W2_KERNELS(FSMC_DECLARE_W2, KH, NW)
FSMC_ALL_W2(FSMC_DECLARE_W2_MEMBER)
#endif

}
```

### fastsmc_amd/csrc/fsmc_kernels.h

```cpp
#pragma once

#include <hip/hip_runtime.h>

#include <type_traits>

#include "../../include/fastsmc_hip.h"

namespace fsmc
{

constexpr int kWave = 64;

typedef const float __attribute__((address_space(4))) * cfloat_p;
typedef const int __attribute__((address_space(4))) * cint_p;
typedef const unsigned __attribute__((address_space(4))) * cuint_p;
typedef float f32x2 __attribute__((ext_vector_type(2)));
typedef float f32x4 __attribute__((ext_vector_type(4)));
typedef float f32x8 __attribute__((ext_vector_type(8)));
typedef float f32x16 __attribute__((ext_vector_type(16)));
constexpr int kMaxStates = 256;
constexpr int kMaxStatesW2 = 1024;
constexpr int kMaxStatesAny = 4096;

enum Mode : int { kModeIbd = 0, kModeDump = 1, kModePerPair = 2, kModeSums = 3 };

struct KParams {
  int K;
  int KP;
  int S;
  int W;
  int nGroups;
  int groupBase;
  int chunk;
  int chunkRows;
  int maxChunks;
  unsigned flags;
  const float* pi;
  const float* cR;
  const float* expT;
  const float* D;
  const float* B;
  const float* U;
  const float* rowSets;
  const float* RR;
  const float* ghostMask;
  const int* stepRow;
  const int* rowGapF;
  const int* rowSiteB;
  const int* rowGapB;
  const float4* emis3;
  const unsigned long long* haps;
  const fsmc_pair* pairs;
  const fsmc_group* groups;
  unsigned* counters;
  float4* ws;
  size_t wsSlot;
  unsigned stateThr, ageThr;
  unsigned spsLds;
  float thr[4];
  fsmc_ibd_record* recs;
  unsigned recCap;
  float* dumpOut;
  const size_t* dumpOffsets;
  float* ppMean;
  int* ppMap;
  const float* expCoal;
  unsigned long long* phaseCycles;
  float* sums;
  size_t sumsPlane;
  size_t sumsSlot;
  const unsigned* batchFirst;
  int residentChunks;
};

#if defined(__HIP_DEVICE_COMPILE__)
#define FSMC_GCN_ASM(...) asm volatile(__VA_ARGS__)
#else
#define FSMC_GCN_ASM(...) ((void)0)
#endif

__device__ __forceinline__ f32x4 sload4(cfloat_p p, const int byteOff)
{
  f32x4 v = {};
  FSMC_GCN_ASM("s_load_dwordx4 %0, %1, %2" : "=s"(v) : "s"(p), "i"(byteOff));
  return v;
}
__device__ __forceinline__ f32x8 sload8(cfloat_p p, const int byteOff)
{
  f32x8 v = {};
#if defined(FSMC_DIAG_NOSMEM)
  FSMC_GCN_ASM("; no load %0 %1 %2" : "=s"(v) : "s"(p), "i"(byteOff));
#else
  FSMC_GCN_ASM("s_load_dwordx8 %0, %1, %2" : "=s"(v) : "s"(p), "i"(byteOff));
#endif
  return v;
}
#if defined(FSMC_NO_TOUCH)
constexpr bool kTouch = false;
#else
constexpr bool kTouch = true;
#endif
struct Touched {
  float r[4];
};
template <int FIRST, int STEP = 16>
__device__ __forceinline__ void touchLines(Touched& t, cfloat_p p, const int firstState)
{
  FSMC_GCN_ASM("s_load_dword %0, %4, %5\n\ts_load_dword %1, %4, %6\n\ts_load_dword %2, %4, %7\n\ts_load_dword %3, %4, %8"
               : "=&s"(t.r[0]), "=&s"(t.r[1]), "=&s"(t.r[2]), "=&s"(t.r[3])
               : "s"(p), "i"((firstState + FIRST * STEP) * 4), "i"((firstState + (FIRST + 1) * STEP) * 4),
                 "i"((firstState + (FIRST + 2) * STEP) * 4), "i"((firstState + (FIRST + 3) * STEP) * 4));
}
__device__ __forceinline__ void holdTouched(Touched& a)
{
  FSMC_GCN_ASM("" : "+s"(a.r[0]), "+s"(a.r[1]), "+s"(a.r[2]), "+s"(a.r[3]));
}
#define FSMC_SWAIT_INSN "s_waitcnt lgkmcnt(0)"
__device__ __forceinline__ void swait(f32x8& a, f32x8& b)
{
  FSMC_GCN_ASM(FSMC_SWAIT_INSN : "+s"(a), "+s"(b));
}
__device__ __forceinline__ void swait(f32x16& a, f32x16& b)
{
  FSMC_GCN_ASM(FSMC_SWAIT_INSN : "+s"(a), "+s"(b));
}
__device__ __forceinline__ void swait(f32x8& a, f32x8& b, f32x8& c, f32x8& d)
{
  FSMC_GCN_ASM(FSMC_SWAIT_INSN : "+s"(a), "+s"(b), "+s"(c), "+s"(d));
}
template <int N> struct SV;
template <> struct SV<4> {
  typedef f32x4 T;
  static __device__ __forceinline__ T loadAt(cfloat_p p, const int firstState) { return sload4(p, firstState * 4); }
};
template <> struct SV<8> {
  typedef f32x8 T;
  static __device__ __forceinline__ T loadAt(cfloat_p p, const int firstState) { return sload8(p, firstState * 4); }
};
template <> struct SV<16> {
  typedef f32x16 T;
  static __device__ __forceinline__ T loadAt(cfloat_p p, const int firstState)
  {
    f32x16 v = {};
#if defined(FSMC_DIAG_NOSMEM)
    FSMC_GCN_ASM("; no load %0 %1 %2" : "=s"(v) : "s"(p), "i"(firstState * 4));
#else
    FSMC_GCN_ASM("s_load_dwordx16 %0, %1, %2" : "=s"(v) : "s"(p), "i"(firstState * 4));
#endif
    return v;
  }
};
__device__ __forceinline__ void swait(f32x4& a, f32x4& b, f32x4& c, f32x4& d)
{
  FSMC_GCN_ASM(FSMC_SWAIT_INSN : "+s"(a), "+s"(b), "+s"(c), "+s"(d));
}

#if defined(FSMC_WAIT_STAMPS)
#define FSMC_SWAIT(acc, ...)                                                                                           \
  do {                                                                                                                 \
    const long long t0_ = (long long)clock64();                                                                        \
    swait(__VA_ARGS__);                                                                                                \
    (acc) += (long long)clock64() - t0_;                                                                               \
  } while (0)
#else
#define FSMC_SWAIT(acc, ...) swait(__VA_ARGS__)
#endif

#ifndef FSMC_KB
#define FSMC_KB 16
#endif
#ifndef FSMC_KBF
#define FSMC_KBF 8
#endif
constexpr int kKB = FSMC_KB;
constexpr int kKBF = FSMC_KBF;
constexpr int kKPad = 16;
enum RowSetPart : int { kRowD = 0, kRowB = 1, kRowU = 2, kRowUsh = 3, kRowRR = 4, kRowSetParts = 5 };
// ... 32 lines not shown
  const f32x2 r = {a.x + b.x, a.y + b.y};
  return r;
#else
  return a + b;
#endif
}
template <typename V> __device__ __forceinline__ f32x2 pairOf(const V& v, const int i)
{
  const f32x2 r = {v[i], v[i + 1]};
  return r;
}
template <int N> __device__ __forceinline__ EmisBlk<N> readEmis(const float4* e, const int blk)
{
  EmisBlk<N> r;
#pragma unroll
  for (int j = 0; j < N / 4; ++j) {
#if defined(FSMC_DIAG_NOEMIS)
    FSMC_GCN_ASM("; no read" : "=v"(r.v[j].x), "=v"(r.v[j].y), "=v"(r.v[j].z), "=v"(r.v[j].w) : "v"(e));
#else
    r.v[j] = e[blk * (N / 4) + j];
#endif
  }
  return r;
}

constexpr int kDiagRegions = 30;
constexpr int kPhaseSlots = 8 + 4 * kDiagRegions;
struct Diag {
  long long waitCycles = 0;
#if defined(FSMC_REGION_STAMPS)
  unsigned acc[kDiagRegions] = {};
  unsigned last = 0;
#endif
};
#if defined(FSMC_REGION_STAMPS)
#define FSMC_END(dg, id)                                                                                               \
  do {                                                                                                                 \
    const unsigned now_ = (unsigned)__builtin_readcyclecounter();                                                      \
    (dg).acc[id] += now_ - (dg).last;                                                                                  \
    (dg).last = now_;                                                                                                  \
  } while (0)
#else
#define FSMC_END(dg, id) ((void)0)
#endif

__device__ __forceinline__ void waitLgkm0()
{
  __builtin_amdgcn_s_waitcnt(0xC07F);
}
__device__ __forceinline__ void waitVm0()
{
  __builtin_amdgcn_s_waitcnt(0x0F70);
}
template <typename V> __device__ __forceinline__ void landed(const V& a, const V& b)
{
  FSMC_GCN_ASM("" ::"s"(a), "s"(b));
}
template <typename V> __device__ __forceinline__ void landed(const V& a, const V& b, const V& c, const V& d)
{
  FSMC_GCN_ASM("" ::"s"(a), "s"(b), "s"(c), "s"(d));
}
template <typename V> __device__ __forceinline__ void landed(const V& a)
{
  FSMC_GCN_ASM("" ::"s"(a));
}
#if defined(FSMC_WAIT_STAMPS)
#define FSMC_WAIT_OPERANDS(acc)                                                                                        \
  do {                                                                                                                 \
    const long long t0_ = (long long)clock64();                                                                        \
    waitLgkm0();                                                                                                       \
    (acc) += (long long)clock64() - t0_;                                                                               \
    __builtin_amdgcn_sched_barrier(0);                                                                                 \
  } while (0)
#else
#define FSMC_WAIT_OPERANDS(acc)                                                                                        \
  do {                                                                                                                 \
    waitLgkm0();                                                                                                       \
    __builtin_amdgcn_sched_barrier(0);                                                                                 \
  } while (0)
#endif

template <int FIRST, int COUNT> __device__ __forceinline__ void touchRow(Touched& t, cfloat_p p, const int firstState)
{
  constexpr int STEP = 16;
  if constexpr (COUNT >= 4) {
    touchLines<FIRST, STEP>(t, p, firstState);
  } else if constexpr (COUNT == 3) {
    FSMC_GCN_ASM("s_load_dword %0, %3, %4\n\ts_load_dword %1, %3, %5\n\ts_load_dword %2, %3, %6"
                 : "=&s"(t.r[0]), "=&s"(t.r[1]), "=&s"(t.r[2])
                 : "s"(p), "i"((firstState + FIRST * STEP) * 4), "i"((firstState + (FIRST + 1) * STEP) * 4),
                   "i"((firstState + (FIRST + 2) * STEP) * 4));
  } else if constexpr (COUNT == 2) {
    FSMC_GCN_ASM("s_load_dword %0, %2, %3\n\ts_load_dword %1, %2, %4"
                 : "=&s"(t.r[0]), "=&s"(t.r[1])
                 : "s"(p), "i"((firstState + FIRST * STEP) * 4), "i"((firstState + (FIRST + 1) * STEP) * 4));
  } else if constexpr (COUNT == 1) {
    FSMC_GCN_ASM("s_load_dword %0, %1, %2" : "=&s"(t.r[0]) : "s"(p), "i"((firstState + FIRST * STEP) * 4));
  }
}
template <int COUNT> __device__ __forceinline__ void heldRow(const Touched& t)
{
  if constexpr (COUNT >= 4) {
    FSMC_GCN_ASM("" ::"s"(t.r[0]), "s"(t.r[1]), "s"(t.r[2]), "s"(t.r[3]));
  } else if constexpr (COUNT == 3) {
    FSMC_GCN_ASM("" ::"s"(t.r[0]), "s"(t.r[1]), "s"(t.r[2]));
  } else if constexpr (COUNT == 2) {
    FSMC_GCN_ASM("" ::"s"(t.r[0]), "s"(t.r[1]));
  } else if constexpr (COUNT == 1) {
    FSMC_GCN_ASM("" ::"s"(t.r[0]));
  }
}

template <int N, bool SY> struct LD {
  typedef typename SV<N>::T T;
  static __device__ __forceinline__ T loadAt(cfloat_p p, const int firstState)
  {
    if constexpr (!SY) {
      return SV<N>::loadAt(p, firstState);
    } else {
      T v = {};
      if constexpr (N == 16) {
        FSMC_GCN_ASM("s_load_dwordx16 %0, %1, %2\n\ts_waitcnt lgkmcnt(0)" : "=s"(v) : "s"(p), "i"(firstState * 4));
      } else if constexpr (N == 8) {
        FSMC_GCN_ASM("s_load_dwordx8 %0, %1, %2\n\ts_waitcnt lgkmcnt(0)" : "=s"(v) : "s"(p), "i"(firstState * 4));
      } else {
        FSMC_GCN_ASM("s_load_dwordx4 %0, %1, %2\n\ts_waitcnt lgkmcnt(0)" : "=s"(v) : "s"(p), "i"(firstState * 4));
      }
      return v;
    }
  }
};

template <int KT> struct BetaOps {
  typename SV<kKB>::T u, rr;
  Touched tu, trr;
  EmisBlk<kKB> em;
};

template <int KT, bool SY = false>
__device__ __forceinline__ void beta_issue_pk(BetaOps<KT>& o, cfloat_p rowSet, const float4* e)
{
  constexpr int KPc = ((KT + kKPad - 1) / kKPad) * kKPad;
  constexpr int NB = (KT + kKB - 1) / kKB;
  constexpr int NLINES = KPc / 16;
  o.u = LD<kKB, SY>::loadAt(rowSet, kRowUsh * KPc + (NB - 1) * kKB);
  o.rr = LD<kKB, SY>::loadAt(rowSet, kRowRR * KPc + (NB - 1) * kKB);
  if constexpr (kTouch && !SY) {
    touchRow<0, NLINES - 1>(o.tu, rowSet, kRowUsh * KPc);
    touchRow<0, NLINES - 1>(o.trr, rowSet, kRowRR * KPc);
  }
  o.em = readEmis<kKB>(e, NB - 1);
}

template <int KT, int KA, bool GHOST, bool SY = false>
__device__ __forceinline__ float beta_core_pk(float (&b)[KA], float (&w)[KA], BetaOps<KT>& ops, cfloat_p rowSet,
                                              const float4* e, cfloat_p ghostMask, Diag& dg)
{
  constexpr int K = KT;
  constexpr int KPc = ((KT + kKPad - 1) / kKPad) * kKPad;
  typedef typename SV<kKB>::T SVec;
  constexpr int NB = (K + kKB - 1) / kKB;
  constexpr int R = kKB / 8;
  constexpr int NLINES = KPc / 16;
  static_assert(kKB == 16, "line warm-up and ghost masking are laid out for operand blocks of one 64-byte line");
  static_assert(!GHOST || K % kKB == 0, "ghost padding fills whole operand blocks");
  SVec u, rr, nu, nrr;
  EmisBlk<kKB> em, nem;
  SVec d, bt, nd, nbt, mk;
  Touched td, tbt;
  float tcarry = 0.f;
#pragma unroll
  for (int blk = NB - 1; blk >= 0; --blk) {
    FSMC_WAIT_OPERANDS(dg.waitCycles);
    if (blk == NB - 1) {
      landed(ops.u, ops.rr);
      if constexpr (kTouch && !SY) {
        heldRow<NLINES - 1>(ops.tu);
        heldRow<NLINES - 1>(ops.trr);
      }
      u = ops.u;
      rr = ops.rr;
      em = ops.em;
    } else {
      landed(nu, nrr);
      u = nu;
      rr = nrr;
      em = nem;
    }
    if (blk > 0) {
      nu = LD<kKB, SY>::loadAt(rowSet, kRowUsh * KPc + (blk - 1) * kKB);
      nrr = LD<kKB, SY>::loadAt(rowSet, kRowRR * KPc + (blk - 1) * kKB);
      nem = readEmis<kKB>(e, blk - 1);
    } else {
      d = LD<kKB, SY>::loadAt(rowSet, kRowD * KPc);
      bt = LD<kKB, SY>::loadAt(rowSet, kRowB * KPc);
      if constexpr (kTouch && !SY) {
        touchRow<1, NLINES - 1>(td, rowSet, kRowD * KPc);
        touchRow<1, NLINES - 1>(tbt, rowSet, kRowB * KPc);
      }
      if constexpr (GHOST && NB == 1) {
        mk = LD<kKB, SY>::loadAt(ghostMask, 0);
      }
    }
    __builtin_amdgcn_sched_barrier(0);
#pragma unroll
    for (int sbi = R - 1; sbi >= 0; --sbi) {
      const int sb = blk * R + sbi;
      const int o = sbi * 8;
      if (sb * 8 >= K) {
        continue;
      }
      float T[9];
      T[8] = tcarry;
#pragma unroll
      for (int i = 0; i < 8; i += 2) {
        const int k = sb * 8 + i;
        if (k + 1 < K) {
          f32x2 v = {b[k], b[k + 1]};
          v = pmul(v, em.pair(o + i));
          const f32x2 t = pmul(pairOf(u, o + i), v);
          b[k] = v.x;
          b[k + 1] = v.y;
          T[i] = t.x;
          T[i + 1] = t.y;
        } else if (k < K) {
          b[k] = b[k] * em.at(o + i);
          T[i] = u[o + i] * b[k];
        }
      }
#pragma unroll
      for (int i = 7; i >= 0; --i) {
        const int k = sb * 8 + i;
        if (k < K) {
          if (k == K - 1) {
            w[k] = 0.f;
          } else {
            w[k] = T[i + 1] + rr[o + i] * w[k + 1];
          }
        }
      }
      tcarry = T[0];
    }
  }
  FSMC_END(dg, 2);
  float BL = 0.f;
  float sum = 0.f;
#pragma unroll
  for (int blk = 0; blk < NB; ++blk) {
    FSMC_WAIT_OPERANDS(dg.waitCycles);
    if (blk > 0) {
      landed(nd, nbt);
      d = nd;
      bt = nbt;
    } else {
      landed(d, bt);
      if constexpr (kTouch && !SY) {
        heldRow<NLINES - 1>(td);
        heldRow<NLINES - 1>(tbt);
      }
    }
    if constexpr (GHOST) {
      if (blk == NB - 1) {
        landed(mk);
      }
    }
    if (blk + 1 < NB) {
      nd = LD<kKB, SY>::loadAt(rowSet, kRowD * KPc + (blk + 1) * kKB);
      nbt = LD<kKB, SY>::loadAt(rowSet, kRowB * KPc + (blk + 1) * kKB);
      if constexpr (GHOST) {
        if (blk + 1 == NB - 1) {
          mk = LD<kKB, SY>::loadAt(ghostMask, (NB - 1) * kKB);
        }
      }
    }
    __builtin_amdgcn_sched_barrier(0);
#pragma unroll
    for (int i = 0; i < kKB; i += 2) {
      const int k = blk * kKB + i;
      if (k + 1 < K) {
        const f32x2 v = {b[k], b[k + 1]};
        const f32x2 dv = pmul(pairOf(d, i), v);
        const f32x2 bv = pmul(pairOf(bt, i), v);
        f32x2 bl;
        bl.x = BL;
        bl.y = BL + bv.x;
        f32x2 x = padd(bl, dv);
        const f32x2 bu = {w[k], w[k + 1]};
        x = padd(x, bu);
        if constexpr (GHOST) {
          if (blk == NB - 1) {
            x = pmul(x, pairOf(mk, i));
          }
        }
        w[k] = x.x;
        w[k + 1] = x.y;
        sum = sum + x.x;
        sum = sum + x.y;
        BL = (k + 1 < K - 1) ? bl.y + bv.y : bl.y;
      } else if (k < K) {
        w[k] = (BL + d[i] * b[k]) + w[k];
        sum = sum + w[k];
        if (k < K - 1) {
          BL = BL + bt[i] * b[k];
        }
      }
    }
  }
  FSMC_END(dg, 3);
  return sum;
}

template <int KT, int KA> __device__ __forceinline__ void scale_pk(float (&v)[KA], const float (&w)[KA], const float sum)
{
  constexpr int K = KT;
  const float c = 1.0f / sum;
  const f32x2 cc = {c, c};
#pragma unroll
  for (int k = 0; k < K; k += 2) {
    if (k + 1 < K) {
      const f32x2 x = {w[k], w[k + 1]};
      const f32x2 y = pmul(x, cc);
      v[k] = y.x;
      v[k + 1] = y.y;
    } else {
      v[k] = w[k] * c;
    }
  }
}

template <int KT, int KA, bool SCALE, bool GHOST, bool SY = false>
__device__ __forceinline__ void beta_step_pk(float (&b)[KA], float (&w)[KA], cfloat_p rowSet, const float4* e,
                                             cfloat_p ghostMask, Diag& dg)
{
  BetaOps<KT> ops;
  beta_issue_pk<KT, SY>(ops, rowSet, e);
  const float sum = beta_core_pk<KT, KA, GHOST, SY>(b, w, ops, rowSet, e, ghostMask, dg);
  if constexpr (SCALE) {
    scale_pk<KT, KA>(b, w, sum);
  } else {
#pragma unroll
    for (int k = 0; k < KT; ++k) {
      b[k] = w[k];
    }
  }
}

template <int KT, int KA, bool SCALE = true, bool SY = false>
__device__ __forceinline__ void alpha_step_pk(float (&a)[KA], float (&w)[KA], cfloat_p rowSet, cfloat_p cR,
                                              const float4* e, Diag& dg)
{
  constexpr int K = KT;
  constexpr int KPc = ((KT + kKPad - 1) / kKPad) * kKPad;
  static_assert(K >= 2, "packed step needs at least two states");
  typedef typename SV<kKBF>::T SVec;
  constexpr int NB = (K + kKBF - 1) / kKBF;
  constexpr int NLINES = KPc / 16;
  SVec d = LD<kKBF, SY>::loadAt(rowSet, kRowD * KPc), bt = LD<kKBF, SY>::loadAt(rowSet, kRowB * KPc),
       u = LD<kKBF, SY>::loadAt(rowSet, kRowU * KPc), c4 = LD<kKBF, SY>::loadAt(cR, 0);
  Touched td, tbt, tu;
  if constexpr (kTouch && !SY) {
    touchRow<1, NLINES - 1>(td, rowSet, kRowD * KPc);
    touchRow<1, NLINES - 1>(tbt, rowSet, kRowB * KPc);
    touchRow<1, NLINES - 1>(tu, rowSet, kRowU * KPc);
  }
  SVec nd, nbt, nu, nc;
  EmisBlk<kKBF> em = readEmis<kKBF>(e, 0), nem;
  __builtin_amdgcn_sched_barrier(0);
  w[K - 2] = a[K - 1];
#pragma unroll
  for (int k = K - 2; k >= 1; --k) {
    w[k - 1] = w[k] + a[k];
  }
  float AU = 0.f;
  float sum = 0.f;
  FSMC_END(dg, 5);
#pragma unroll
  for (int blk = 0; blk < NB; ++blk) {
    FSMC_WAIT_OPERANDS(dg.waitCycles);
    if (blk > 0) {
      landed(nd, nbt, nu, nc);
      d = nd;
      bt = nbt;
      u = nu;
      c4 = nc;
      em = nem;
    } else {
      landed(d, bt, u, c4);
      if constexpr (kTouch && !SY) {
        heldRow<NLINES - 1>(td);
        heldRow<NLINES - 1>(tbt);
        heldRow<NLINES - 1>(tu);
      }
    }
    if (blk + 1 < NB) {
      nd = LD<kKBF, SY>::loadAt(rowSet, kRowD * KPc + (blk + 1) * kKBF);
      nbt = LD<kKBF, SY>::loadAt(rowSet, kRowB * KPc + (blk + 1) * kKBF);
      nu = LD<kKBF, SY>::loadAt(rowSet, kRowU * KPc + (blk + 1) * kKBF);
      nc = LD<kKBF, SY>::loadAt(cR, (blk + 1) * kKBF);
      nem = readEmis<kKBF>(e, blk + 1);
    }
    __builtin_amdgcn_sched_barrier(0);
#pragma unroll
    for (int i = 0; i < kKBF; i += 2) {
      const int k = blk * kKBF + i;
      if (k + 1 < K - 1) {
        const f32x2 av = {a[k], a[k + 1]};
        const f32x2 da = pmul(pairOf(d, i), av);
        const f32x2 ua = pmul(pairOf(u, i), av);
        const f32x2 ac = {w[k], w[k + 1]};
        const f32x2 bw = pmul(pairOf(bt, i), ac);
        f32x2 au;
        au.x = AU;
        au.y = ua.x + c4[i] * AU;
        f32x2 term = padd(au, da);
        term = padd(term, bw);
        const f32x2 ov = pmul(em.pair(i), term);
        w[k] = ov.x;
        w[k + 1] = ov.y;
        sum = sum + ov.x;
        sum = sum + ov.y;
        AU = ua.y + c4[i + 1] * au.y;
      } else {
#pragma unroll
        for (int ii = i; ii < i + 2; ++ii) {
          const int kk = blk * kKBF + ii;
          if (kk < K) {
            float term = AU + d[ii] * a[kk];
            if (kk < K - 1) {
              term = term + bt[ii] * w[kk];
            }
            w[kk] = em.at(ii) * term;
            sum = sum + w[kk];
            if (kk < K - 1) {
              AU = u[ii] * a[kk] + c4[ii] * AU;
            }
          }
        }
      }
    }
  }
  FSMC_END(dg, 6);
  if constexpr (SCALE) {
    scale_pk<KT, KA>(a, w, sum);
  } else {
#pragma unroll
    for (int k = 0; k < K; ++k) {
      a[k] = w[k];
    }
  }
  FSMC_END(dg, 7);
}



struct Tables {
  cfloat_p rowSets, cR, ghostMask;
};

template <int KT> constexpr bool kGhost = KT % kKPad == 0;

template <int KT> __device__ __forceinline__ cfloat_p rowSetOf(const Tables& t, const int row)
{
  constexpr int KPc = ((KT + kKPad - 1) / kKPad) * kKPad;
  return t.rowSets + (size_t)row * (kRowSetParts * KPc);
}

template <int MODE, bool SEQ, bool DUAL> constexpr bool kSpsLdsBuilt = MODE == kModeIbd && !SEQ && !DUAL;
#if defined(FSMC_SEQ_SYNC_LOADS)
template <bool SEQ, int KT, int MODE> constexpr bool kSeqSyncLoads = SEQ;
#else
template <bool SEQ, int KT, int MODE> constexpr bool kSeqSyncLoads = SEQ && (KT <= 32 || MODE != kModeIbd);
#endif
template <int KT, int KA, bool SCALE = true, bool SY = false>
__device__ __forceinline__ void beta_step(const int K, float (&b)[KA], float (&w)[KA], const Tables& t, const int row,
                                          const float4* e, Diag& dg)
{
  (void)K;
  beta_step_pk<KT, KA, SCALE, kGhost<KT>, SY>(b, w, rowSetOf<KT>(t, row), e, t.ghostMask, dg);
}

template <int KT, int KA, bool SCALE = true, bool SY = false>
__device__ __forceinline__ void alpha_step(const int K, float (&a)[KA], float (&w)[KA], const Tables& t, const int row,
                                           const float4* e, Diag& dg)
{
  (void)K;
  alpha_step_pk<KT, KA, SCALE, SY>(a, w, rowSetOf<KT>(t, row), t.cR, e, dg);
}

template <int KT, int KA>
__device__ __forceinline__ void alpha_init(const int K, float (&a)[KA], cfloat_p pi, const float4* e)
{
  float sum = 0.f;
  float4 ev = {0.f, 0.f, 0.f, 0.f};
#pragma unroll
  for (int k = 0; k < K; ++k) {
    if ((k & 3) == 0) {
      ev = e[k >> 2];
    }
    const float em = (k & 3) == 0 ? ev.x : (k & 3) == 1 ? ev.y : (k & 3) == 2 ? ev.z : ev.w;
    a[k] = pi[k] * em;
    sum = sum + a[k];
  }
  const float c = 1.0f / sum;
#pragma unroll
  for (int k = 0; k < K; ++k) {
    a[k] = a[k] * c;
  }
}

template <int KT, int KA> __device__ __forceinline__ void beta_init(const int K, const int Kreal, float (&b)[KA])
{
  float sum = 0.f;
#pragma unroll
  for (int k = 0; k < K; ++k) {
    b[k] = (!kGhost<KT> || k < Kreal) ? 1.0f : 0.f;
    sum = sum + b[k];
  }
  const float c = 1.0f / sum;
#pragma unroll
  for (int k = 0; k < K; ++k) {
    b[k] = b[k] * c;
  }
}

typedef char __attribute__((address_space(1))) * gchar_p;
typedef f32x4 __attribute__((address_space(1))) * gf32x4_p;
__device__ __forceinline__ gchar_p uniformPtr(const void* p)
{
  const unsigned long long v = reinterpret_cast<unsigned long long>(p);
  const unsigned lo = __builtin_amdgcn_readfirstlane((unsigned)v);
  const unsigned hi = __builtin_amdgcn_readfirstlane((unsigned)(v >> 32));
  return (gchar_p)(((unsigned long long)hi << 32) | lo);
}
__device__ __forceinline__ gf32x4_p rowSlot(const gchar_p base, const int k4, const unsigned laneOff)
{
  return (gf32x4_p)(base + (size_t)k4 * (kWave * sizeof(float4)) + laneOff);
}
#if defined(__clang__)
#pragma clang diagnostic push
#pragma clang diagnostic ignored "-Winline-asm"
#endif
__device__ __forceinline__ void dmaToLds(const gf32x4_p src, const void* ldsDst)
{
#if defined(__HIP_DEVICE_COMPILE__)
  const unsigned lds = (unsigned)(unsigned long long)(const char __attribute__((address_space(3)))*)ldsDst;
  asm volatile("s_mov_b32 m0, %1\n\ts_nop 0\n\tglobal_load_lds_dwordx4 %0, off" ::"v"(src), "s"(lds) : "memory", "m0");
#endif
}
#if defined(__clang__)
#pragma clang diagnostic pop
#endif

template <int KT, int KA>
__device__ __forceinline__ void store_vec(const int K, float4* row, const unsigned laneOff, const float (&v)[KA])
{
  const gchar_p base = uniformPtr(row);
  const int K4 = (K + 3) >> 2;
#pragma unroll
  for (int k4 = 0; k4 < K4; ++k4) {
    float4 o;
    o.x = v[4 * k4];
    o.y = (4 * k4 + 1 < K) ? v[4 * k4 + 1] : 0.f;
    o.z = (4 * k4 + 2 < K) ? v[4 * k4 + 2] : 0.f;
    o.w = (4 * k4 + 3 < K) ? v[4 * k4 + 3] : 0.f;
    const f32x4 ov = {o.x, o.y, o.z, o.w};
    __builtin_nontemporal_store(ov, rowSlot(base, k4, laneOff));
  }
}

template <int KT, int KA>
__device__ __forceinline__ void load_vec(const int K, const float4* row, const unsigned laneOff, float (&v)[KA])
{
  const gchar_p base = uniformPtr(row);
  const int K4 = (K + 3) >> 2;
#pragma unroll
  for (int k4 = 0; k4 < K4; ++k4) {
    const f32x4 ov = __builtin_nontemporal_load(rowSlot(base, k4, laneOff));
    const float4 o = make_float4(ov.x, ov.y, ov.z, ov.w);
    v[4 * k4] = o.x;
    if (4 * k4 + 1 < K) v[4 * k4 + 1] = o.y;
    if (4 * k4 + 2 < K) v[4 * k4 + 2] = o.z;
    if (4 * k4 + 3 < K) v[4 * k4 + 3] = o.w;
  }
}

__device__ __forceinline__ float spsAt(const float4* sps, const int k)
{
  return reinterpret_cast<const float*>(sps + (size_t)(k >> 2) * kWave)[k & 3];
}
__device__ __forceinline__ void segment_ages(const int K, const unsigned nAge, const float4* sps, cfloat_p pi,
                                             cfloat_p expT, const bool wantMean, const bool wantMap, float& mean,
                                             float& mapv)
{
  mean = 0.f;
  mapv = 0.f;
  const int n = (unsigned)K < nAge ? K : (int)nAge;
  if (wantMean) {
    float acc = 0.f;
#pragma nounroll
    for (int k = 0; k < n; ++k) {
      acc = acc + spsAt(sps, k);
    }
    const float norm = 1.f / acc;
#pragma nounroll
    for (int k = 0; k < n; ++k) {
      mean = mean + (norm * spsAt(sps, k)) * expT[k];
    }
  }
  if (wantMap) {
    float best = 0.f;
    float bestT = 0.f;
#pragma nounroll
    for (int k = 0; k < n; ++k) {
      const float r = spsAt(sps, k) / pi[k];
      if (k == 0 || best < r) {
        best = r;
        bestT = expT[k];
      }
    }
    mapv = bestT;
  }
}

__device__ __forceinline__ unsigned launderScalar(unsigned v)
{
  FSMC_GCN_ASM("" : "+s"(v));
  return v;
}
template <int KA, int K, int K4>
__device__ __forceinline__ void scanBlocks(float (&w)[KA], float& s, const float cq, const unsigned nPost)
{
#pragma unroll
  for (int k4 = 0; k4 < K4; ++k4) {
    if ((unsigned)(4 * k4) >= nPost) {
      break;
    }
#pragma unroll
    for (int i = 0; i < 4; ++i) {
      if (4 * k4 + i < K) {
        w[4 * k4 + i] = w[4 * k4 + i] * cq;
        s = s + ((unsigned)(4 * k4 + i) < nPost ? w[4 * k4 + i] : 0.f);
      }
    }
  }
}

}

#include "fsmc_lane_scaffold.h"
#include "fsmc_site_consumers.h"

namespace fsmc
{

constexpr int minWavesPerSimd(const int KT)
{
  return KT >= 70 ? 1 : 2;
}
template <int KT, int MODE, bool TRACK, bool SEQ, bool HALF, bool DUAL = false>
__global__ __launch_bounds__(kWave, minWavesPerSimd(KT)) void decode_kernel(const KParams p)
{
  static_assert(!HALF || (!SEQ && (MODE == kModeIbd || MODE == kModeSums)),
                "beta stride 2 is built for the array-mode IBD decode and the array-mode sums over pairs");
  static_assert(KT > 0 && KT <= kMaxStates, "a member of the kernel family (fsmc_instances.h)");
  static_assert(!DUAL || (MODE == kModeIbd && !SEQ), "two half-groups per wave: array-mode IBD");
  constexpr bool kRotate = !SEQ;
  constexpr int KA = KT;
  constexpr int K4A = (KA + 3) / 4;
  constexpr int E4A = ((KA + kKPad - 1) / kKPad) * (kKPad / 4);
  constexpr int NC = SEQ ? 4 : 3;
  constexpr int NL = (NC * E4A + kWave - 1) / kWave;
  constexpr int K = KT;
  const int Kreal = kGhost<KT> ? p.K : K;
  constexpr int K4 = (K + 3) >> 2;
  const int KP = p.KP;
  const int E4 = KP >> 2;

  __shared__ float4 emisLds[2][NC * E4A];
  constexpr int kLandF4 = (MODE == kModeSums && (KA * 65 + 3) / 4 > K4A * kWave) ? (KA * 65 + 3) / 4 : K4A * kWave;
  __shared__ float4 betaLds[kLandF4];
  __shared__ float coalLds[MODE == kModePerPair ? KA : 1];

  const int lane = threadIdx.x;
  const cfloat_p tPi = (cfloat_p)p.pi, tCR = (cfloat_p)p.cR, tExpT = (cfloat_p)p.expT;
  const Tables tabs = {(cfloat_p)p.rowSets, tCR, (cfloat_p)p.ghostMask};
  const cint_p tStepRow = (cint_p)p.stepRow;
  const cint_p tRowGapF = (cint_p)p.rowGapF, tRowSiteB = (cint_p)(SEQ ? p.rowSiteB : p.stepRow),
               tRowGapB = (cint_p)p.rowGapB;
  const size_t vecF4 = (size_t)K4 * kWave;
  float4* const chunkbuf = p.ws + (size_t)blockIdx.x * p.wsSlot;
  float4* const ckpt = chunkbuf + (size_t)p.chunkRows * vecF4;
  float4* const saveA = ckpt + (size_t)(p.maxChunks + 2) * vecF4;
  float4* const saveS = saveA + vecF4;
  float4* const resBase = saveS + vecF4;
  constexpr bool kResidentBuilt = !SEQ && !DUAL && (MODE == kModeIbd || MODE == kModeSums);
  const int nResident = kResidentBuilt ? p.residentChunks : 0;
  const int C = p.chunk;
  extern __shared__ float4 spsDyn[];
  const bool spsInLds = TRACK && kSpsLdsBuilt<MODE, SEQ, DUAL> && p.spsLds != 0;
  const float4* const spsMem = spsInLds ? (const float4*)(spsDyn + threadIdx.x) : (const float4*)(saveS + threadIdx.x);
  const unsigned laneOff = threadIdx.x * (unsigned)sizeof(float4);
#if defined(FSMC_DIAG_SAMEROW)
  auto slotOf = [](const int rel) -> size_t { return (size_t)(rel & 0); };
#else
  auto slotOf = [](const int rel) -> size_t { return (size_t)(HALF ? (rel >> 1) : rel); };
#endif

  struct EmisRegs {
    float4 v[NL];
  };
  if (MODE == kModePerPair) {
    for (int k = lane; k < K; k += kWave) {
      coalLds[k] = (k < Kreal) ? p.expCoal[k] : 0.f;
    }
    __builtin_amdgcn_fence(__ATOMIC_RELEASE, "wavefront");
    __builtin_amdgcn_wave_barrier();
  }

  for (unsigned round = 0;; ++round) {
#if defined(FSMC_DIAG_GROUP_TIMES)
    const unsigned long long diagT0 = __builtin_amdgcn_s_memrealtime();
#endif
    unsigned g = 0;
    if (MODE == kModeSums) {
      g = sumsGroupOf(p, round);
    } else {
      if (lane == 0) {
        g = atomicAdd(&p.counters[p.groupBase], 1u);
      }
      g = __builtin_amdgcn_readfirstlane(g);
    }
    if (g >= (unsigned)p.nGroups) {
      break;
    }
    const cuint_p gw = (cuint_p)(p.groups + (DUAL ? 2 * (size_t)g : (size_t)g));
    const unsigned firstPair = gw[0];
    const int nPairsInGroup = (int)gw[1];
    int from = (int)gw[2];
    int to = (int)gw[3];
    int scanFrom = (int)gw[4];
    int aEnd = (MODE == kModeIbd) ? (int)gw[5] : to;
    const LanePair me = laneInGroup(firstPair, nPairsInGroup, lane);
    bool valid = me.valid;
    unsigned pairIdx = me.pairIdx;
    int myFrom = from, myTo = to, mySF = scanFrom, myST = aEnd;
    int toA = to, toB = to, fromA = from, fromB = from, stA = aEnd, stB = aEnd;
    if constexpr (DUAL) {
      const int nB = (int)gw[7];
      if (nB > 0) {
        fromB = (int)gw[8];
        toB = (int)gw[9];
        stB = (int)gw[11];
        const bool half = lane >= 32;
        valid = half ? (lane - 32 < nB) : (lane < nPairsInGroup);
        pairIdx = half ? gw[6] + (valid ? (unsigned)(lane - 32) : 0u) : firstPair + (valid ? (unsigned)lane : 0u);
        myFrom = half ? fromB : fromA;
        myTo = half ? toB : toA;
        mySF = half ? (int)gw[10] : scanFrom;
        myST = half ? stB : stA;
        from = fromA < fromB ? fromA : fromB;
        to = toA > toB ? toA : toB;
        scanFrom = scanFrom < (int)gw[10] ? scanFrom : (int)gw[10];
        aEnd = stA > stB ? stA : stB;
      } else {
        valid = lane < nPairsInGroup && lane < 32;
      }
    }
    const HapRows hap = hapRows(p, pairIdx);
    const unsigned long long* rowA = hap.rowA;
    const unsigned long long* rowB = hap.rowB;

    const int nA = aEnd - from;
    const int nChunks = (nA + C - 1) / C;
    const bool single = nChunks <= 1;
    __builtin_amdgcn_s_setprio(3);

    int wordIdx = -1;
    unsigned long long xw = 0, aw = 0;
    auto obsClass = [&](const int q) -> int {
      const int wi = q >> 6;
      if (__builtin_expect(wi != wordIdx, 0)) {
        const unsigned long long wa = rowA[wi];
        const unsigned long long wb = rowB[wi];
        xw = wa ^ wb;
        aw = wa & wb;
        wordIdx = wi;
      }
      const int bit = q & 63;
      const int x = (int)((xw >> bit) & 1ull);
      const int t = (int)((aw >> bit) & 1ull);
      return x ? 0 : 1 + t;
    };
    auto prefetchEmis = [&](const int q) -> EmisRegs {
      EmisRegs r;
#pragma unroll
      for (int i = 0; i < NL; ++i) {
        const int idx = lane + i * kWave;
        r.v[i] = make_float4(0.f, 0.f, 0.f, 0.f);
        if (idx < NC * E4) {
          r.v[i] = p.emis3[(size_t)q * (NC * E4) + idx];
        }
      }
      return r;
    };
    auto commitEmis = [&](const int q, const EmisRegs& r) {
#pragma unroll
      for (int i = 0; i < NL; ++i) {
        const int idx = lane + i * kWave;
        if (idx < NC * E4) {
          emisLds[q & 1][idx] = r.v[i];
        }
      }
      __builtin_amdgcn_wave_barrier();
    };

    auto stageEmis = [&](const int q) {
      const gchar_p src = uniformPtr(p.emis3 + (size_t)q * (NC * E4));
#pragma unroll
      for (int i = 0; i < NL; ++i) {
        const int idx = lane + i * kWave;
        if (idx < NC * E4) {
          dmaToLds((gf32x4_p)(src + (size_t)i * (kWave * sizeof(float4)) + laneOff), &emisLds[q & 1][i * kWave]);
        }
      }
    };
    RowIndexBlock stepRows;
    auto stepRowOf = [&](const int site) -> int { return stepRows.at(p.stepRow, p.S, lane, site); };
    auto waitEmisRows = [&](const bool storesBehind) {
      constexpr unsigned n = (unsigned)K4A;
      if (storesBehind && n < 64) {
        __builtin_amdgcn_s_waitcnt(0x0F70 | (n & 15u) | ((n >> 4) << 14));
      } else {
        waitVm0();
      }
    };

    float w[KA];
    Diag cycW;
#if defined(FSMC_REGION_STAMPS)
    cycW.last = (unsigned)__builtin_readcyclecounter();
#endif
#if defined(FSMC_PHASE_STAMPS)
    long long cycB = 0, cycR = 0, cycA = 0;
    long long stamp = (long long)clock64();
#define FSMC_STAMP(acc)                                                                                                \
  do {                                                                                                                 \
    const long long now_ = (long long)clock64();                                                                       \
    (acc) += now_ - stamp;                                                                                             \
    stamp = now_;                                                                                                      \
  } while (0)
#else
#define FSMC_STAMP(acc) ((void)0)
#endif

    auto betaGapStep = [&](float (&b)[KA], const int q, const EmisRegs& rows) {
      commitEmis(q, rows);
      const int row = tRowGapB[q];
      beta_step<KT, KA, false, kSeqSyncLoads<SEQ, KT, MODE>>(K, b, w, tabs, row, &emisLds[q & 1][3 * E4], cycW);
    };
    auto betaSeqStep = [&](float (&b)[KA], const int pos) {
      const int q = pos + 1;
      const bool gap = pos > from;
      EmisRegs ev;
      if (gap) {
        ev = prefetchEmis(pos);
      }
      const int c = obsClass(q);
      const int row = tRowSiteB[q];
      beta_step<KT, KA, true, kSeqSyncLoads<SEQ, KT, MODE>>(K, b, w, tabs, row, &emisLds[q & 1][c * E4], cycW);
      if (gap) {
        betaGapStep(b, pos, ev);
      }
    };

    {
      float b[KA];
      if constexpr (!kRotate) {
        beta_init<KT, KA>(K, p.K, b);
      }
      int ckJ = (aEnd < to) ? nChunks : nChunks - 1;
      int ckPos = (aEnd < to) ? aEnd : from + ckJ * C;
      auto afterBeta = [&](const int pos) -> bool {
        if (single) {
          const int rel = pos - from;
          if (pos < aEnd && (!HALF || (rel & 1) || pos == aEnd - 1)) {
            store_vec<KT, KA>(K, chunkbuf + slotOf(rel) * vecF4, laneOff, b);
            return true;
          }
        } else {
          bool out = false;
          if (kResidentBuilt && ckJ < nResident && pos < aEnd) {
            const int relc = pos - ckPos;
            const int hiJ = ckPos + C < aEnd ? ckPos + C : aEnd;
            if (!HALF || (relc & 1) || pos == hiJ - 1) {
              store_vec<KT, KA>(K, resBase + ((size_t)ckJ * p.chunkRows + slotOf(relc)) * vecF4, laneOff, b);
              out = true;
            }
          }
          if (__builtin_expect(pos == ckPos && ckJ >= 1, 0)) {
            store_vec<KT, KA>(K, ckpt + (size_t)ckJ * vecF4, laneOff, b);
            ckJ -= 1;
            ckPos = from + ckJ * C;
            out = true;
          }
          return out;
        }
        return false;
      };
      if constexpr (SEQ) {
        if (to - 1 > from) {
          betaGapStep(b, to - 1, prefetchEmis(to - 1));
        }
      }
      if constexpr (!kRotate) {
        afterBeta(to - 1);
      }
      if constexpr (SEQ) {
        for (int pos = to - 2; pos >= from; --pos) {
          betaSeqStep(b, pos);
          afterBeta(pos);
        }
      } else {
        if (to - 2 >= from) {
          stageEmis(to - 1);
        }
        if constexpr (kRotate) {
          float bsum = 0.f;
#pragma unroll
          for (int k = 0; k < K; ++k) {
            w[k] = (!kGhost<KT> || k < p.K) ? 1.0f : 0.f;
            bsum = bsum + w[k];
          }
          const float bsumInit = bsum;
          auto openBeta = [&](const int q) {
            if constexpr (DUAL) {
              if (q == toA - 1 || q == toB - 1) {
                const bool sel = myTo - 1 == q;
#pragma unroll
                for (int k = 0; k < K; ++k) {
                  w[k] = sel ? ((!kGhost<KT> || k < p.K) ? 1.0f : 0.f) : w[k];
                }
                bsum = sel ? bsumInit : bsum;
              }
            }
          };
          bool stored = false;
          for (int pos = to - 2; pos >= from; --pos) {
            const int q = pos + 1;
            openBeta(q);
            waitEmisRows(stored);
            __builtin_amdgcn_wave_barrier();
            if (pos - 1 >= from) {
              stageEmis(q - 1);
            }
            const int row = stepRowOf(q);
            const int c = obsClass(q);
            const float4* e = &emisLds[q & 1][c * E4];
            const cfloat_p rs = rowSetOf<KT>(tabs, row);
            BetaOps<KT> ops;
            beta_issue_pk<KT>(ops, rs, e);
            FSMC_END(cycW, 0);
            scale_pk<KT, KA>(b, w, bsum);
            stored = afterBeta(q);
            FSMC_END(cycW, 1);
            bsum = beta_core_pk<KT, KA, kGhost<KT>>(b, w, ops, rs, e, tabs.ghostMask, cycW);
          }
          openBeta(from);
          scale_pk<KT, KA>(b, w, bsum);
          afterBeta(from);
        } else {
          for (int pos = to - 2; pos >= from; --pos) {
            const int q = pos + 1;
            waitVm0();
            __builtin_amdgcn_wave_barrier();
            if (pos - 1 >= from) {
              stageEmis(q - 1);
            }
            const int row = stepRowOf(q);
            const int c = obsClass(q);
            beta_step<KT, KA, true, kSeqSyncLoads<SEQ, KT, MODE>>(K, b, w, tabs, row, &emisLds[q & 1][c * E4], cycW);
            afterBeta(pos);
          }
        }
      }
    }

    FSMC_STAMP(cycB);
    int cur = 4;
    int segStart = 0;
    float acc = 0.f;
    float a[KA];

    auto emit = [&](const int s0, const int s1) {
#if defined(FSMC_DIAG_NOSMEM) || defined(FSMC_DIAG_NOEMIS) || defined(FSMC_DIAG_SAMEROW)
      if (s0 >= 0) {
        return;
      }
#endif
      emitIbdRecord<TRACK>(p, K, spsMem, tPi, tExpT, pairIdx, s0, s1, acc);
    };
    auto fetchBeta = [&](const float4* row) {
      const gchar_p base = uniformPtr(row);
#pragma unroll
      for (int k4 = 0; k4 < K4; ++k4) {
#if defined(__HIP_DEVICE_COMPILE__)
        __builtin_amdgcn_global_load_lds(rowSlot(base, k4, laneOff), &betaLds[k4 * kWave], 16, 0, 2 );
#endif
      }
    };

    for (int j = 0; j < (nChunks > 0 ? nChunks : 0); ++j) {
      {
        const int left = (8 * (nChunks - j)) / (3 * nChunks);
        if (left >= 2) {
          __builtin_amdgcn_s_setprio(2);
        } else if (left == 1) {
          __builtin_amdgcn_s_setprio(1);
        } else {
          __builtin_amdgcn_s_setprio(0);
        }
      }
      const int lo = from + j * C;
      const int hi = (lo + C < aEnd) ? lo + C : aEnd;
      const bool resident = kResidentBuilt && !single && j < nResident;
      float4* const cbuf = resident ? resBase + (size_t)j * p.chunkRows * vecF4 : chunkbuf;
      if (!single && !resident) {
        if (j > 0) {
          store_vec<KT, KA>(K, saveA, laneOff, a);
        }
        auto storeRow = [&](const int site, const float (&row)[KA]) -> bool {
          const int rel = site - lo;
          if (!HALF || (rel & 1) || site == hi - 1) {
            store_vec<KT, KA>(K, chunkbuf + slotOf(rel) * vecF4, laneOff, row);
            return true;
          }
          return false;
        };
        if constexpr (kRotate) {
          float b[KA];
          float bsum = 0.f;
          int pos;
          if (hi == to) {
#pragma unroll
            for (int k = 0; k < K; ++k) {
              w[k] = (!kGhost<KT> || k < p.K) ? 1.0f : 0.f;
              bsum = bsum + w[k];
            }
            pos = to - 2;
          } else {
            load_vec<KT, KA>(K, ckpt + (size_t)(j + 1) * vecF4, laneOff, w);
            bsum = 1.0f;
            pos = hi - 1;
          }
          if (pos >= lo) {
            stageEmis(pos + 1);
          }
          auto reopenBeta = [&](const int q) {
            if constexpr (DUAL) {
              if (q == toA - 1 || q == toB - 1) {
                const bool sel = myTo - 1 == q;
                float ones = 0.f;
#pragma unroll
                for (int k = 0; k < K; ++k) {
                  const float one = (!kGhost<KT> || k < p.K) ? 1.0f : 0.f;
                  w[k] = sel ? one : w[k];
                  ones = ones + one;
                }
                bsum = sel ? ones : bsum;
              }
            }
          };
          bool stored = false;
          for (; pos >= lo; --pos) {
            const int q = pos + 1;
            reopenBeta(q);
            waitEmisRows(stored);
            __builtin_amdgcn_wave_barrier();
            if (pos - 1 >= lo) {
              stageEmis(q - 1);
            }
            const int row = stepRowOf(q);
            const int c = obsClass(q);
            const float4* e = &emisLds[q & 1][c * E4];
            const cfloat_p rs = rowSetOf<KT>(tabs, row);
            BetaOps<KT> ops;
            beta_issue_pk<KT>(ops, rs, e);
            FSMC_END(cycW, 0);
            scale_pk<KT, KA>(b, w, bsum);
            stored = q < hi && storeRow(q, b);
            FSMC_END(cycW, 1);
            bsum = beta_core_pk<KT, KA, kGhost<KT>>(b, w, ops, rs, e, tabs.ghostMask, cycW);
          }
          reopenBeta(pos + 1);
          scale_pk<KT, KA>(b, w, bsum);
          if (pos + 1 < hi) {
            storeRow(pos + 1, b);
          }
        } else {
          float b[KA];
          int pos;
          if (hi == to) {
            beta_init<KT, KA>(K, p.K, b);
            if constexpr (SEQ) {
              if (to - 1 > from) {
                betaGapStep(b, to - 1, prefetchEmis(to - 1));
              }
            }
            store_vec<KT, KA>(K, chunkbuf + slotOf(to - 1 - lo) * vecF4, laneOff, b);
            pos = to - 2;
          } else {
            load_vec<KT, KA>(K, ckpt + (size_t)(j + 1) * vecF4, laneOff, b);
            pos = hi - 1;
            if constexpr (SEQ) {
              commitEmis(hi, prefetchEmis(hi));
            }
          }
          if constexpr (SEQ) {
            for (; pos >= lo; --pos) {
              betaSeqStep(b, pos);
              store_vec<KT, KA>(K, chunkbuf + (size_t)(pos - lo) * vecF4, laneOff, b);
            }
          } else {
            if (pos >= lo) {
              stageEmis(pos + 1);
            }
            for (; pos >= lo; --pos) {
              const int q = pos + 1;
              waitVm0();
              __builtin_amdgcn_wave_barrier();
              if (pos - 1 >= lo) {
                stageEmis(q - 1);
              }
              const int row = stepRowOf(q);
              const int c = obsClass(q);
              beta_step<KT, KA, true, kSeqSyncLoads<SEQ, KT, MODE>>(K, b, w, tabs, row, &emisLds[q & 1][c * E4], cycW);
              storeRow(pos, b);
            }
          }
        }
        if (j > 0) {
          load_vec<KT, KA>(K, saveA, laneOff, a);
        }
      }

      FSMC_END(cycW, 13);
      FSMC_STAMP(cycR);
      __builtin_amdgcn_fence(__ATOMIC_RELEASE, "wavefront");
      waitVm0();
      fetchBeta(cbuf);
      EmisRegs ev;
      if constexpr (SEQ) {
        ev = prefetchEmis(lo);
        commitEmis(lo, ev);
      } else {
        stageEmis(lo);
        if (lo + 1 < hi) {
          stageEmis(lo + 1);
        }
      }
      waitVm0();
      for (int pos = lo; pos < hi; ++pos) {
        const bool rec = HALF && ((pos - lo) & 1) == 0 && pos + 1 < hi;

        if constexpr (SEQ) {
          if (pos < to - 1) {
            ev = prefetchEmis(pos + 1);
          }
        }
        const int c = obsClass(pos);
        const float4* e = &emisLds[pos & 1][c * E4];
        FSMC_END(cycW, 4);
        if (__builtin_expect(pos == from, 0)) {
          alpha_init<KT, KA>(K, a, tPi, e);
        } else {
          alpha_step<KT, KA, true, kSeqSyncLoads<SEQ, KT, MODE>>(K, a, w, tabs, stepRowOf(pos), e, cycW);
          if constexpr (DUAL) {
            if (pos == fromA || pos == fromB) {
              alpha_init<KT, KA>(K, w, tPi, e);
              const bool sel = myFrom == pos;
#pragma unroll
              for (int k = 0; k < K; ++k) {
                a[k] = sel ? w[k] : a[k];
              }
            }
          }
        }
        if constexpr (SEQ) {
          if (pos < to - 1) {
            commitEmis(pos + 1, ev);
            const int row = tRowGapF[pos + 1];
            alpha_step<KT, KA, false, kSeqSyncLoads<SEQ, KT, MODE>>(K, a, w, tabs, row, &emisLds[(pos + 1) & 1][3 * E4],
                                            cycW);
          }
        }

        waitVm0();
        __builtin_amdgcn_wave_barrier();
        FSMC_END(cycW, 8);
        float sumq = 0.f;
        if (rec) {
          float b[KA];
          const int q = pos + 1;
          const int cq1 = obsClass(q);
          const int rowq = stepRowOf(q);
          const float4* eq = &emisLds[q & 1][cq1 * E4];
          auto readLanded = [&]() {
#pragma unroll
            for (int k4 = 0; k4 < K4; ++k4) {
              const float4 o = betaLds[k4 * kWave + lane];
              b[4 * k4] = o.x;
              if (4 * k4 + 1 < K) b[4 * k4 + 1] = o.y;
              if (4 * k4 + 2 < K) b[4 * k4 + 2] = o.z;
              if (4 * k4 + 3 < K) b[4 * k4 + 3] = o.w;
            }
          };
          {
            const cfloat_p rs = rowSetOf<KT>(tabs, rowq);
            BetaOps<KT> ops;
            beta_issue_pk<KT>(ops, rs, eq);
            readLanded();
            FSMC_END(cycW, 9);
            const float bsum = beta_core_pk<KT, KA, kGhost<KT>>(b, w, ops, rs, eq, tabs.ghostMask, cycW);
            scale_pk<KT, KA>(b, w, bsum);
            if constexpr (DUAL) {
              if (__builtin_expect(pos == toA - 1 || pos == toB - 1, 0)) {
                float ones = 0.f;
#pragma unroll
                for (int k = 0; k < K; ++k) {
                  ones = ones + ((!kGhost<KT> || k < p.K) ? 1.0f : 0.f);
                }
                const float c1 = 1.0f / ones;
                const bool sel = myTo - 1 == pos;
#pragma unroll
                for (int k = 0; k < K; ++k) {
                  const float init = ((!kGhost<KT> || k < p.K) ? 1.0f : 0.f) * c1;
                  b[k] = sel ? init : b[k];
                }
              }
            }
          }
          FSMC_END(cycW, 9);
#pragma unroll
          for (int k = 0; k < K; k += 2) {
            if (k + 1 < K) {
              const f32x2 av = {a[k], a[k + 1]};
              const f32x2 bv = {b[k], b[k + 1]};
              const f32x2 q = pmul(av, bv);
// ... 380 lines not shown
```

### include/fastsmc_hip.h

```cpp
#ifndef FASTSMC_HIP_H
#define FASTSMC_HIP_H

#include <stddef.h>
#include <stdint.h>

#ifdef __cplusplus
extern "C" {
#endif

#define FSMC_OK 0
#define FSMC_EINVAL (-1)
#define FSMC_ENODEVICE (-2)
#define FSMC_EHIP (-3)
#define FSMC_ENOMEM (-4)
#define FSMC_ESTATE (-5)
#define FSMC_EOVERFLOW (-6)
#define FSMC_EUNSUPPORTED (-7)
#define FSMC_ERUNTIME (-8)

typedef struct fsmc_ctx fsmc_ctx;
typedef struct fsmc_model fsmc_model;

typedef struct {
  int32_t K;
  int32_t S;
  const float* pi;
  const float* col_ratios;
  const float* exp_times;
  int32_t n_rows;
  const float* D;
  const float* B;
  const float* U;
  const float* RR;
  const int32_t* step_row;
  const float* e1;
  const float* e0m1;
  const float* e2m0;
  uint32_t state_threshold;
  uint32_t age_threshold;
  float probability_threshold;
  int32_t sequence;
  const int32_t* gap_row_f;
  const int32_t* site_row_f;
  const int32_t* gap_row_b;
  const int32_t* site_row_b;
  const float* hom;
} fsmc_model_desc;

typedef struct {
  uint32_t hap_a;
  uint32_t hap_b;
} fsmc_pair;

typedef struct {
  uint32_t first_pair;
  uint32_t n_pairs;
  uint32_t from, to;
  uint32_t scan_from, scan_to;
} fsmc_group;

typedef struct {
  uint32_t pair;
  int32_t start;
  int32_t end;
  float prob;
  float post_mean;
  float map;
} fsmc_ibd_record;

#define FSMC_WANT_MEAN 1u
#define FSMC_WANT_MAP 2u
#define FSMC_WANT_SUMS 4u
#define FSMC_WANT_MAJOR_MINOR_SUMS 8u

int fsmc_ctx_create(int device_id, void* stream, fsmc_ctx** out);
void fsmc_ctx_destroy(fsmc_ctx* ctx);
const char* fsmc_last_error(const fsmc_ctx* ctx);
int fsmc_ctx_info(const fsmc_ctx* ctx, int32_t* n_cu, int32_t* n_slots, uint64_t* hbm_bytes);
int fsmc_ctx_set_workspace_limit(fsmc_ctx* ctx, uint64_t bytes);
int fsmc_ctx_expect_work(fsmc_ctx* ctx, double pair_sites, int32_t states);
int fsmc_ctx_set_chunk_sites(fsmc_ctx* ctx, uint32_t sites);
int fsmc_ctx_set_beta_stride(fsmc_ctx* ctx, uint32_t stride);
int fsmc_ctx_last_beta_stride(const fsmc_ctx* ctx, int32_t* stride);
int fsmc_ctx_last_plan(const fsmc_ctx* ctx, int32_t* chunk_sites, int32_t* max_chunks, int32_t* n_slots);
int fsmc_ctx_set_resident_chunks(fsmc_ctx* ctx, int32_t chunks);
int fsmc_ctx_last_resident_chunks(const fsmc_ctx* ctx, int32_t* chunks);
int fsmc_ctx_set_pairing(fsmc_ctx* ctx, uint32_t mode);
int fsmc_ctx_last_items(const fsmc_ctx* ctx, int32_t* n_items);
int fsmc_ctx_set_two_wave_windows(fsmc_ctx* ctx, uint32_t mode);
int fsmc_ctx_last_waves_per_window(const fsmc_ctx* ctx, int32_t* waves);
int fsmc_ctx_last_segment_sums_in_lds(const fsmc_ctx* ctx, int32_t* in_lds);
int fsmc_ctx_set_pair_posterior_slice(fsmc_ctx* ctx, uint32_t groups);
int fsmc_ctx_last_pair_posterior_slices(const fsmc_ctx* ctx, int32_t* slices);
int fsmc_ctx_set_pair_minima_slice(fsmc_ctx* ctx, uint32_t groups);
int fsmc_ctx_last_pair_minima_slices(const fsmc_ctx* ctx, int32_t* slices);
int fsmc_ctx_set_pair_bins_slice(fsmc_ctx* ctx, uint32_t groups);
int fsmc_ctx_last_pair_bins_slices(const fsmc_ctx* ctx, int32_t* slices);
int fsmc_ctx_set_pair_cdf_slice(fsmc_ctx* ctx, uint32_t groups);
int fsmc_ctx_last_pair_cdf_slices(const fsmc_ctx* ctx, int32_t* slices);
int fsmc_ctx_set_pair_tail_slice(fsmc_ctx* ctx, uint32_t groups);
int fsmc_ctx_last_pair_tail_slices(const fsmc_ctx* ctx, int32_t* slices);
int fsmc_ctx_set_pair_loglik_slice(fsmc_ctx* ctx, uint32_t groups);
int fsmc_ctx_last_pair_loglik_slices(const fsmc_ctx* ctx, int32_t* slices);
int fsmc_ctx_set_pair_viterbi_slice(fsmc_ctx* ctx, uint32_t groups);
int fsmc_ctx_last_pair_viterbi_slices(const fsmc_ctx* ctx, int32_t* slices);
int fsmc_ctx_last_kernel(const fsmc_ctx* ctx, int32_t* member);

int fsmc_model_create(fsmc_ctx* ctx, const fsmc_model_desc* desc, fsmc_model** out);
void fsmc_model_destroy(fsmc_model* m);
int fsmc_haps_upload(fsmc_ctx* ctx, const uint64_t* bits, uint32_t n_haps, uint32_t n_sites);
int fsmc_worklist_upload(fsmc_ctx* ctx, const fsmc_pair* pairs, size_t n_pairs, const fsmc_group* groups,
                         size_t n_groups);

int fsmc_decode_ibd_launch(fsmc_ctx* ctx, const fsmc_model* m, uint32_t flags);
int fsmc_decode_ibd_fetch(fsmc_ctx* ctx, fsmc_ibd_record* out, size_t cap, size_t* n_out);
typedef struct {
  uint32_t window_size;
  uint32_t w_i, w_j;
  int32_t last_job;
  int32_t j_above_diag;
} fsmc_job_window;

typedef struct {
  uint32_t hap_a, hap_b;
  uint32_t from, to;
  uint32_t flush_word;
} fsmc_candidate;

int fsmc_identify(fsmc_ctx* ctx, const uint64_t* words, uint32_t n_haps, uint32_t n_words, const uint32_t* global_ids,
                  const fsmc_job_window* job, const float* gen_pos, uint32_t n_sites, int32_t gap, float skip,
                  float min_m, fsmc_candidate* out, size_t cap, size_t* n_out);
typedef struct {
  uint32_t word_size;
  uint32_t haploid;
  int32_t max_seeds;
  uint32_t read_ahead;
} fsmc_identify_opts;
int fsmc_identify_ex(fsmc_ctx* ctx, const uint64_t* words, uint32_t n_haps, uint32_t n_words,
                     const uint32_t* global_ids, const fsmc_job_window* job, const float* gen_pos, uint32_t n_sites,
                     int32_t gap, float skip, float min_m, const fsmc_identify_opts* opts, fsmc_candidate* out,
                     size_t cap, size_t* n_out);
int fsmc_identify_fetch(fsmc_ctx* ctx, fsmc_candidate* out, size_t cap, size_t* n_out);

int fsmc_sync(fsmc_ctx* ctx);
int fsmc_last_kernel_ms(fsmc_ctx* ctx, float* ms);

int fsmc_phase_cycles(fsmc_ctx* ctx, uint64_t* out, size_t n);

int fsmc_decode_ibd(fsmc_ctx* ctx, const fsmc_model* m, const fsmc_pair* pairs, size_t n_pairs,
                    const fsmc_group* groups, size_t n_groups, uint32_t flags, fsmc_ibd_record* out, size_t cap,
                    size_t* n_out);

int fsmc_decode_posteriors(fsmc_ctx* ctx, const fsmc_model* m, float* out, size_t out_floats);

int fsmc_decode_per_pair(fsmc_ctx* ctx, const fsmc_model* m, const float* exp_coal_times, float* mean, int32_t* map);

int fsmc_decode_pair_posteriors(fsmc_ctx* ctx, const fsmc_model* m, const float* exp_coal_times,
                                float* const* post_rows, float* sum);

int fsmc_decode_pair_minima(fsmc_ctx* ctx, const fsmc_model* m, const float* exp_coal_times, uint64_t pair_base,
                            float* min_mean, int32_t* argmin_mean, int32_t* min_map, int32_t* argmin_map);

int fsmc_decode_pair_bins(fsmc_ctx* ctx, const fsmc_model* m, const float* exp_coal_times, const int32_t* bin_edges,
                          size_t n_bins, float* bin_mean, float* bin_min_mean, int32_t* bin_argmin_mean,
                          int32_t* bin_min_map, int32_t* bin_argmin_map);

int fsmc_decode_pair_loglik(fsmc_ctx* ctx, const fsmc_model* m, const int32_t* bin_edges, size_t n_bins, double* mant,
                            int32_t* expo, double* bin_mant, int32_t* bin_expo);

int fsmc_decode_pair_viterbi(fsmc_ctx* ctx, const fsmc_model* m, uint8_t* states, double* mant, int32_t* expo);

int fsmc_decode_pair_cdf(fsmc_ctx* ctx, const fsmc_model* m, const int32_t* tail_states, size_t n_tail,
                         float* const* tail_rows, const float* quantiles, size_t n_quantiles,
                         int32_t* const* quantile_rows);

int fsmc_decode_pair_tail_summaries(fsmc_ctx* ctx, const fsmc_model* m, const int32_t* tail_states, size_t n_tail,
                                    double* tail_sum, const int32_t* bin_edges, size_t n_bins, float* bin_tail_mean,
                                    const float* site_weights, float* bin_tail_length);

int fsmc_decode_sums(fsmc_ctx* ctx, const fsmc_model* m, float* sums, float* sums00, float* sums01, float* sums11);
int fsmc_decode_sums_batches(fsmc_ctx* ctx, const fsmc_model* m, const uint32_t* batch_first_group, size_t n_batches,
                             float* sums, float* sums00, float* sums01, float* sums11);

#ifdef __cplusplus
}
#endif
#endif
```

Baseline: 272,700 pairs/s.

## Record backward scale factors on first pass and reuse them in chunk recompute

For the K=69 half-stride IBD kernel, the first backward sweep writes each site's reciprocal beta normaliser to a per-lane track buffer carved out of the workspace. Chunk recomputation then reads these stored factors and skips the per-site sum reduction and reciprocal in beta_core. This removes serial add and divide work from the recompute loop. In exchange it adds a global store and load per site and a larger workspace slot, and the reuse path is used only when the chunk plan stays the same.

Result: no change. 273,200 pairs/s, median of 6 (+0.2%).

```diff
diff --git a/fastsmc_amd/capi.py b/fastsmc_amd/capi.py
--- a/fastsmc_amd/capi.py
+++ b/fastsmc_amd/capi.py
@@ -20,7 +20,7 @@
     "fsmc_ctx_expect_work",
     "fsmc_ctx_set_chunk_sites", "fsmc_ctx_set_beta_stride", "fsmc_ctx_last_beta_stride", "fsmc_ctx_last_plan",
     "fsmc_ctx_last_kernel", "fsmc_ctx_set_pairing", "fsmc_ctx_last_items", "fsmc_ctx_set_two_wave_windows", "fsmc_ctx_last_waves_per_window", "fsmc_ctx_last_segment_sums_in_lds", "fsmc_ctx_set_resident_chunks",
-    "fsmc_ctx_last_resident_chunks",
+    "fsmc_ctx_last_resident_chunks", "fsmc_ctx_last_scale_reuse",
     "fsmc_model_create", "fsmc_model_destroy", "fsmc_haps_upload", "fsmc_worklist_upload",
     "fsmc_decode_ibd_launch", "fsmc_decode_ibd_fetch", "fsmc_sync", "fsmc_last_kernel_ms", "fsmc_phase_cycles",
     "fsmc_decode_ibd",
@@ -216,6 +216,11 @@
         self._check(self._L.fsmc_ctx_last_resident_chunks(self._h, C.byref(v)))
         return v.value
 
+    def last_scale_reuse(self) -> bool:
+        v = C.c_int32(0)
+        self._check(self._L.fsmc_ctx_last_scale_reuse(self._h, C.byref(v)))
+        return bool(v.value)
+
     def set_beta_stride(self, stride: int):
         self._check(self._L.fsmc_ctx_set_beta_stride(self._h, stride))
 
diff --git a/fastsmc_amd/csrc/fsmc_capi.hip b/fastsmc_amd/csrc/fsmc_capi.hip
--- a/fastsmc_amd/csrc/fsmc_capi.hip
+++ b/fastsmc_amd/csrc/fsmc_capi.hip
@@ -99,6 +99,7 @@
   bool timed = false;
   int lastSlots = 0;
   int lastChunk = 0, lastMaxChunks = 0, lastResident = 0;
+  bool lastScaleReuse = false;
   int residentChunks = -1;
   uint32_t chunkSites = 0;
   uint32_t betaStride = 0;
@@ -406,6 +407,8 @@
   unsigned threads = kWave;
   int member = 0;
   int stride = 1;
+  bool scaleReuse = false;
+  KernelFn reuseFn = nullptr;
 };
 
 KernelChoice chooseKernel(const fsmc_model* m, int mode, bool track, bool dual, uint32_t wantStride)
@@ -431,6 +434,10 @@
   const bool half = wantStride != 1 && !m->sequence &&
                     ((mode == kModeIbd && halfBuilt(k.member)) || (mode == kModeSums && halfSumsBuilt(k.member)));
   k.stride = half ? 2 : 1;
+  if (half && !dual && mode == kModeIbd && k.member == 69) {
+    static_assert(scaleReuseBuilt(69, kModeIbdReuse), "fsmc_instances.h: FSMC_KT_REUSE_KERNELS");
+    k.reuseFn = track ? decode_kernel<69, kModeIbdReuse, true, false, true> : decode_kernel<69, kModeIbdReuse, false, false, true>;
+  }
   switch (k.member) {
 #define FSMC_PICK_CASE(KTX)                                                                                             \
   case KTX:                                                                                                            \
@@ -529,6 +536,7 @@
   int chunkRows = 0;
   int maxChunks = 0;
   int residentChunks = 0;
+  size_t trackF4 = 0;
   size_t wsSlot = 0;
   int slots = 0;
   int wavesPerWindow = 1;
@@ -615,9 +623,34 @@
   ctx->wsEarned += earnScale() * kEarnFraction * seconds * kAllocBytesPerSecond;
 }
 
+int planOneWaveAs(const fsmc_ctx* ctx, const fsmc_model* m, int mode, const KernelChoice& k,
+                  const std::vector<fsmc_group>& list, bool paired, const WsBudget& budget, unsigned share,
+                  LaunchPlan& plan, std::string& why);
 int planOneWave(const fsmc_ctx* ctx, const fsmc_model* m, int mode, const KernelChoice& k,
                 const std::vector<fsmc_group>& list, bool paired, const WsBudget& budget, unsigned share,
                 LaunchPlan& plan, std::string& why)
+{
+  KernelChoice plain = k;
+  plain.reuseFn = nullptr;
+  const int rc = planOneWaveAs(ctx, m, mode, plain, list, paired, budget, share, plan, why);
+  if (rc != FSMC_OK || !k.reuseFn || paired) {
+    return rc;
+  }
+  KernelChoice reuse = plain;
+  reuse.fn = k.reuseFn;
+  reuse.scaleReuse = true;
+  LaunchPlan withTrack;
+  std::string whyNot;
+  if (planOneWaveAs(ctx, m, mode, reuse, list, paired, budget, share, withTrack, whyNot) == FSMC_OK &&
+      withTrack.chunk == plan.chunk && withTrack.maxChunks == plan.maxChunks) {
+    plan = withTrack;
+  }
+  return FSMC_OK;
+}
+
+int planOneWaveAs(const fsmc_ctx* ctx, const fsmc_model* m, int mode, const KernelChoice& k,
+                  const std::vector<fsmc_group>& list, bool paired, const WsBudget& budget, unsigned share,
+                  LaunchPlan& plan, std::string& why)
 {
   if (!k.fn) {
     why = "no kernel for this model";
@@ -631,10 +664,11 @@
   }
   const bool w2 = waveGroups(mode, m);
   const size_t slots = std::max<size_t>(1, std::min((size_t)ctx->nCU * std::max(perCU, 1), list.size()));
-  size_t L = 1;
+  size_t L = 1, Lwhole = 1;
   for (const fsmc_group& g : list) {
     const size_t aEnd = (mode == kModeIbd) ? g.scan_to : g.to;
     L = std::max<size_t>(L, aEnd - g.from);
+    Lwhole = std::max<size_t>(Lwhole, g.to - g.from);
   }
   const size_t K4 = w2 ? (size_t)m->KP / 4 : (size_t)((k.member > 0 ? k.member : m->K) + 3) / 4 + (anyStates(m) ? 1 : 0);
   const size_t vecBytes = K4 * kWave * sizeof(float4);
@@ -643,7 +677,8 @@
   auto chunkRows = [&](size_t c) { return half ? (c + 1) / 2 : c; };
   const size_t rowsAvail = (size_t)(limit / (vecBytes * slots));
   const size_t rowsSoft = (size_t)(budget.soft / share / (vecBytes * slots));
-  const size_t sideRows = anyStates(m) ? (size_t)kAnyExtraRows + 2 : 4;
+  const size_t trackRows = k.scaleReuse ? (Lwhole * kWave * sizeof(float) + vecBytes - 1) / vecBytes : 0;
+  const size_t sideRows = (anyStates(m) ? (size_t)kAnyExtraRows + 2 : 4) + trackRows;
   const size_t defaultChunk = std::max<size_t>((size_t)std::ceil(std::sqrt((double)L)), w2 ? 2048 : 512);
   size_t C, maxChunks;
   if (chunkRows(L) + sideRows + 1 <= rowsAvail && (chunkRows(L) + sideRows + 1 <= rowsSoft || L <= defaultChunk) &&
@@ -683,6 +718,7 @@
   plan.maxChunks = (int)maxChunks;
   plan.residentChunks = (int)resident;
   plan.wsSlot = (chunkRows(C) * (1 + resident) + maxChunks + 2 + (sideRows - 2)) * K4 * kWave;
+  plan.trackF4 = trackRows * K4 * kWave;
   plan.slots = (int)slots;
   plan.k = k;
   plan.wavesPerWindow = 1;
@@ -805,6 +841,7 @@
   ctx->lastChunk = plan.chunk;
   ctx->lastMaxChunks = plan.maxChunks;
   ctx->lastResident = plan.residentChunks;
+  ctx->lastScaleReuse = k.scaleReuse;
   ctx->lastWavesPerWindow = plan.wavesPerWindow;
   ctx->lastSlots = plan.slots + slotsBeside;
 }
@@ -875,7 +912,7 @@
   p.groups = ctx->dGroups;
   p.counters = ctx->dCounters;
   p.phaseCycles = ctx->dPhase;
-  p.ws = (float4*)ctx->ws.p;
+  p.ws = (float4*)ctx->ws.p + plan.trackF4;
   p.wsSlot = plan.wsSlot;
   p.stateThr = m->stateThr;
   p.ageThr = m->ageThr;
@@ -890,8 +927,11 @@
 
 int checkWorkspace(fsmc_ctx* ctx, const KParams& p, int slots)
 {
-  const DevBuf& buf = p.ws == (float4*)ctx->wsSide.p ? ctx->wsSide : ctx->ws;
-  if (!p.ws || p.ws != (float4*)buf.p || slots < 1 || buf.bytes / sizeof(float4) / (size_t)slots < p.wsSlot) {
+  auto heldBy = [&](const DevBuf& b) {
+    return b.p && p.ws >= (float4*)b.p && (p.ws == (float4*)b.p || (size_t)(p.ws - (float4*)b.p) < p.wsSlot);
+  };
+  const DevBuf& buf = heldBy(ctx->wsSide) ? ctx->wsSide : ctx->ws;
+  if (!p.ws || !heldBy(buf) || slots < 1 || buf.bytes / sizeof(float4) / (size_t)slots < p.wsSlot) {
     return fail(ctx, FSMC_ESTATE, "the workspace does not hold the launch planned for it");
   }
   return FSMC_OK;
@@ -1487,6 +1527,15 @@
   return FSMC_OK;
 }
 
+int fsmc_ctx_last_scale_reuse(const fsmc_ctx* ctx, int32_t* reuse)
+{
+  if (!ctx || !reuse) {
+    return FSMC_EINVAL;
+  }
+  *reuse = ctx->lastScaleReuse ? 1 : 0;
+  return FSMC_OK;
+}
+
 int fsmc_ctx_set_pair_posterior_slice(fsmc_ctx* ctx, uint32_t groups) { return setPairSlice(ctx, kSlicePosteriors, groups); }
 int fsmc_ctx_last_pair_posterior_slices(const fsmc_ctx* ctx, int32_t* slices) { return lastPairSlices(ctx, kSlicePosteriors, slices); }
 int fsmc_ctx_set_pair_minima_slice(fsmc_ctx* ctx, uint32_t groups) { return setPairSlice(ctx, kSliceMinima, groups); }
@@ -1932,13 +1981,14 @@
       return rc;
     }
   }
-  const KernelChoice k = chooseKernel(m, kModeIbd, track, false, ctx->betaStride);
+  KernelChoice k = chooseKernel(m, kModeIbd, track, false, ctx->betaStride);
   if (haveRest) {
     rc = planAndHold(ctx, m, kModeIbd, k, q.reordered ? q.rest : ctx->hGroups, false, beside ? 2 : 1,
                      beside ? ctx->wsSide : ctx->ws, plan);
     if (rc != FSMC_OK) {
       return rc;
     }
+    k = plan.k;
   }
   recordLaunch(ctx, k, haveRest ? plan : planDual, beside ? planDual.slots : 0);
   ctx->lastItems = q.dual ? (int)q.unions.size() : 0;
@@ -1962,7 +2012,7 @@
       p.nGroups = (int)q.rest.size();
     }
     if (beside) {
-      p.ws = (float4*)ctx->wsSide.p;
+      p.ws = (float4*)ctx->wsSide.p + plan.trackF4;
     }
   }
   size_t spsLdsBytes = 0;
diff --git a/fastsmc_amd/csrc/fsmc_inst.hip b/fastsmc_amd/csrc/fsmc_inst.hip
--- a/fastsmc_amd/csrc/fsmc_inst.hip
+++ b/fastsmc_amd/csrc/fsmc_inst.hip
@@ -16,6 +16,9 @@
 FSMC_DEFINE_KT_DUAL_HALF(FSMC_INSTANCE_KT)
 FSMC_KT_FWD_KERNELS(FSMC_DEFINE_KT_FWD, FSMC_INSTANCE_KT)
 FSMC_KT_VITERBI_KERNELS(FSMC_DEFINE_KT_VITERBI, FSMC_INSTANCE_KT)
+#if FSMC_INSTANCE_KT == 69
+FSMC_KT_REUSE_KERNELS(FSMC_DEFINE_KT, FSMC_INSTANCE_KT)
+#endif
 #elif defined(FSMC_INSTANCE_W2)
 #ifndef FSMC_INSTANCE_NW
 #define FSMC_INSTANCE_NW 4
diff --git a/fastsmc_amd/csrc/fsmc_instances.h b/fastsmc_amd/csrc/fsmc_instances.h
--- a/fastsmc_amd/csrc/fsmc_instances.h
+++ b/fastsmc_amd/csrc/fsmc_instances.h
@@ -45,6 +45,10 @@
   X(KT, kModeIbd, true, false, true)                                                                                   \
   X(KT, kModeIbd, false, false, true)
 #define FSMC_KT_HALF_SUMS_KERNELS(X, KT) X(KT, kModeSums, false, false, true)
+
+#define FSMC_KT_REUSE_KERNELS(X, KT)                                                                                   \
+  X(KT, kModeIbdReuse, true, false, true)                                                                              \
+  X(KT, kModeIbdReuse, false, false, true)
 
 #define FSMC_DECLARE_KT(KT, MODE, TRACK, SEQ, HALF)                                                                    \
   extern template __global__ void decode_kernel<KT, MODE, TRACK, SEQ, HALF>(const KParams);
@@ -108,6 +112,7 @@
 FSMC_KT_HALF_KERNELS(FSMC_DECLARE_KT, 48) FSMC_KT_HALF_SUMS_KERNELS(FSMC_DECLARE_KT, 48)
 FSMC_KT_HALF_KERNELS(FSMC_DECLARE_KT, 64) FSMC_KT_HALF_SUMS_KERNELS(FSMC_DECLARE_KT, 64)
 FSMC_KT_HALF_KERNELS(FSMC_DECLARE_KT, 69) FSMC_KT_HALF_SUMS_KERNELS(FSMC_DECLARE_KT, 69)
+FSMC_KT_REUSE_KERNELS(FSMC_DECLARE_KT, 69)
 FSMC_KT_HALF_KERNELS(FSMC_DECLARE_KT, 80) FSMC_KT_HALF_SUMS_KERNELS(FSMC_DECLARE_KT, 80)
 FSMC_KT_HALF_KERNELS(FSMC_DECLARE_KT, 96) FSMC_KT_HALF_SUMS_KERNELS(FSMC_DECLARE_KT, 96)
 FSMC_KT_HALF_KERNELS(FSMC_DECLARE_KT, 112) FSMC_KT_HALF_SUMS_KERNELS(FSMC_DECLARE_KT, 112)
diff --git a/fastsmc_amd/csrc/fsmc_kernels.h b/fastsmc_amd/csrc/fsmc_kernels.h
--- a/fastsmc_amd/csrc/fsmc_kernels.h
+++ b/fastsmc_amd/csrc/fsmc_kernels.h
@@ -23,6 +23,7 @@
 constexpr int kMaxStatesAny = 4096;
 
 enum Mode : int { kModeIbd = 0, kModeDump = 1, kModePerPair = 2, kModeSums = 3 };
+constexpr int kModeIbdReuse = 4;
 
 struct KParams {
   int K;
@@ -361,7 +362,7 @@
   o.em = readEmis<kKB>(e, NB - 1);
 }
 
-template <int KT, int KA, bool GHOST, bool SY = false>
+template <int KT, int KA, bool GHOST, bool SY = false, bool SUM = true>
 __device__ __forceinline__ float beta_core_pk(float (&b)[KA], float (&w)[KA], BetaOps<KT>& ops, cfloat_p rowSet,
                                               const float4* e, cfloat_p ghostMask, Diag& dg)
 {
@@ -503,12 +504,16 @@
         }
         w[k] = x.x;
         w[k + 1] = x.y;
-        sum = sum + x.x;
-        sum = sum + x.y;
+        if constexpr (SUM) {
+          sum = sum + x.x;
+          sum = sum + x.y;
+        }
         BL = (k + 1 < K - 1) ? bl.y + bv.y : bl.y;
       } else if (k < K) {
         w[k] = (BL + d[i] * b[k]) + w[k];
-        sum = sum + w[k];
+        if constexpr (SUM) {
+          sum = sum + w[k];
+        }
         if (k < K - 1) {
           BL = BL + bt[i] * b[k];
         }
@@ -519,10 +524,10 @@
   return sum;
 }
 
-template <int KT, int KA> __device__ __forceinline__ void scale_pk(float (&v)[KA], const float (&w)[KA], const float sum)
+template <int KT, int KA>
+__device__ __forceinline__ void scale_rcp_pk(float (&v)[KA], const float (&w)[KA], const float c)
 {
   constexpr int K = KT;
-  const float c = 1.0f / sum;
   const f32x2 cc = {c, c};
 #pragma unroll
   for (int k = 0; k < K; k += 2) {
@@ -535,6 +540,10 @@
       v[k] = w[k] * c;
     }
   }
+}
+template <int KT, int KA> __device__ __forceinline__ void scale_pk(float (&v)[KA], const float (&w)[KA], const float sum)
+{
+  scale_rcp_pk<KT, KA>(v, w, 1.0f / sum);
 }
 
 template <int KT, int KA, bool SCALE, bool GHOST, bool SY = false>
@@ -680,6 +689,12 @@
 #else
 template <bool SEQ, int KT, int MODE> constexpr bool kSeqSyncLoads = SEQ && (KT <= 32 || MODE != kModeIbd);
 #endif
+constexpr bool scaleReuseBuilt(const int KT, const int MODE)
+{
+  return KT == 69 && MODE == kModeIbdReuse;
+}
+template <int KT, int MODE, bool SEQ, bool HALF, bool DUAL>
+constexpr bool kScaleReuse = HALF && !SEQ && !DUAL && scaleReuseBuilt(KT, MODE);
 template <int KT, int KA, bool SCALE = true, bool SY = false>
 __device__ __forceinline__ void beta_step(const int K, float (&b)[KA], float (&w)[KA], const Tables& t, const int row,
                                           const float4* e, Diag& dg)
@@ -734,6 +749,7 @@
 
 typedef char __attribute__((address_space(1))) * gchar_p;
 typedef f32x4 __attribute__((address_space(1))) * gf32x4_p;
+typedef float __attribute__((address_space(1))) * gfloat_p;
 __device__ __forceinline__ gchar_p uniformPtr(const void* p)
 {
   const unsigned long long v = reinterpret_cast<unsigned long long>(p);
@@ -866,9 +882,11 @@
 {
   return KT >= 70 ? 1 : 2;
 }
-template <int KT, int MODE, bool TRACK, bool SEQ, bool HALF, bool DUAL = false>
+template <int KT, int MODE_, bool TRACK, bool SEQ, bool HALF, bool DUAL = false>
 __global__ __launch_bounds__(kWave, minWavesPerSimd(KT)) void decode_kernel(const KParams p)
 {
+  constexpr int MODE = MODE_ == kModeIbdReuse ? (int)kModeIbd : MODE_;
+  static_assert(MODE_ != kModeIbdReuse || kScaleReuse<KT, MODE_, SEQ, HALF, DUAL>, "built for the members with scale reuse");
   static_assert(!HALF || (!SEQ && (MODE == kModeIbd || MODE == kModeSums)),
                 "beta stride 2 is built for the array-mode IBD decode and the array-mode sums over pairs");
   static_assert(KT > 0 && KT <= kMaxStates, "a member of the kernel family (fsmc_instances.h)");
@@ -904,6 +922,7 @@
   float4* const resBase = saveS + vecF4;
   constexpr bool kResidentBuilt = !SEQ && !DUAL && (MODE == kModeIbd || MODE == kModeSums);
   const int nResident = kResidentBuilt ? p.residentChunks : 0;
+  constexpr bool kReuse = kScaleReuse<KT, MODE_, SEQ, HALF, DUAL>;
   const int C = p.chunk;
   extern __shared__ float4 spsDyn[];
   const bool spsInLds = TRACK && kSpsLdsBuilt<MODE, SEQ, DUAL> && p.spsLds != 0;
@@ -1043,6 +1062,22 @@
         waitVm0();
       }
     };
+    auto waitEmisRowsTrack = [&](const bool storesBehind) {
+      constexpr unsigned n = (unsigned)K4A + 1;
+      static_assert(!kReuse || n < 64, "vmcnt has six bits");
+      if (storesBehind) {
+        __builtin_amdgcn_s_waitcnt(0x0F70 | (n & 15u) | ((n >> 4) << 14));
+      } else {
+        __builtin_amdgcn_s_waitcnt(0x0F70 | 1u);
+      }
+    };
+    auto trackAt = [&](const int site) -> gfloat_p {
+      return (gfloat_p)(reinterpret_cast<float*>(chunkbuf) - ((long)(to - site) * kWave - lane));
+    };
+    auto trackDown = [](gfloat_p& t) {
+      t -= kWave;
+      FSMC_GCN_ASM("" : "+v"(t));
+    };
 
     float w[KA];
     Diag cycW;
@@ -1154,10 +1189,19 @@
             }
           };
           bool stored = false;
+          gfloat_p tp = nullptr;
+          if constexpr (kReuse) {
+            tp = trackAt(to - 1);
+            *tp = 1.0f / bsum;
+          }
           for (int pos = to - 2; pos >= from; --pos) {
             const int q = pos + 1;
             openBeta(q);
-            waitEmisRows(stored);
+            if constexpr (kReuse) {
+              waitEmisRowsTrack(stored);
+            } else {
+              waitEmisRows(stored);
+            }
             __builtin_amdgcn_wave_barrier();
             if (pos - 1 >= from) {
               stageEmis(q - 1);
@@ -1169,13 +1213,26 @@
             BetaOps<KT> ops;
             beta_issue_pk<KT>(ops, rs, e);
             FSMC_END(cycW, 0);
-            scale_pk<KT, KA>(b, w, bsum);
+            if constexpr (kReuse) {
+              const float c = 1.0f / bsum;
+              scale_rcp_pk<KT, KA>(b, w, c);
+              *tp = c;
+              trackDown(tp);
+            } else {
+              scale_pk<KT, KA>(b, w, bsum);
+            }
             stored = afterBeta(q);
             FSMC_END(cycW, 1);
             bsum = beta_core_pk<KT, KA, kGhost<KT>>(b, w, ops, rs, e, tabs.ghostMask, cycW);
           }
           openBeta(from);
-          scale_pk<KT, KA>(b, w, bsum);
+          if constexpr (kReuse) {
+            const float c = 1.0f / bsum;
+            scale_rcp_pk<KT, KA>(b, w, c);
+            *tp = c;
+          } else {
+            scale_pk<KT, KA>(b, w, bsum);
+          }
           afterBeta(from);
         } else {
           for (int pos = to - 2; pos >= from; --pos) {
@@ -1261,6 +1318,12 @@
             bsum = 1.0f;
             pos = hi - 1;
           }
+          float cPend = 1.0f, cq = 1.0f;
+          gfloat_p tp = nullptr;
+          if constexpr (kReuse) {
+            cPend = 1.0f / bsum;
+            tp = trackAt(pos);
+          }
           if (pos >= lo) {
             stageEmis(pos + 1);
           }
@@ -1285,6 +1348,11 @@
             reopenBeta(q);
             waitEmisRows(stored);
             __builtin_amdgcn_wave_barrier();
+            if constexpr (kReuse) {
+              cq = cPend;
+              cPend = *tp;
+              trackDown(tp);
+            }
             if (pos - 1 >= lo) {
               stageEmis(q - 1);
             }
@@ -1295,13 +1363,25 @@
             BetaOps<KT> ops;
             beta_issue_pk<KT>(ops, rs, e);
             FSMC_END(cycW, 0);
-            scale_pk<KT, KA>(b, w, bsum);
+            if constexpr (kReuse) {
+              scale_rcp_pk<KT, KA>(b, w, cq);
+            } else {
+              scale_pk<KT, KA>(b, w, bsum);
+            }
             stored = q < hi && storeRow(q, b);
             FSMC_END(cycW, 1);
-            bsum = beta_core_pk<KT, KA, kGhost<KT>>(b, w, ops, rs, e, tabs.ghostMask, cycW);
+            if constexpr (kReuse) {
+              beta_core_pk<KT, KA, kGhost<KT>, false, false>(b, w, ops, rs, e, tabs.ghostMask, cycW);
+            } else {
+              bsum = beta_core_pk<KT, KA, kGhost<KT>>(b, w, ops, rs, e, tabs.ghostMask, cycW);
+            }
           }
           reopenBeta(pos + 1);
-          scale_pk<KT, KA>(b, w, bsum);
+          if constexpr (kReuse) {
+            scale_rcp_pk<KT, KA>(b, w, cPend);
+          } else {
+            scale_pk<KT, KA>(b, w, bsum);
+          }
           if (pos + 1 < hi) {
             storeRow(pos + 1, b);
           }
diff --git a/include/fastsmc_hip.h b/include/fastsmc_hip.h
--- a/include/fastsmc_hip.h
+++ b/include/fastsmc_hip.h
@@ -85,6 +85,7 @@
 int fsmc_ctx_last_plan(const fsmc_ctx* ctx, int32_t* chunk_sites, int32_t* max_chunks, int32_t* n_slots);
 int fsmc_ctx_set_resident_chunks(fsmc_ctx* ctx, int32_t chunks);
 int fsmc_ctx_last_resident_chunks(const fsmc_ctx* ctx, int32_t* chunks);
+int fsmc_ctx_last_scale_reuse(const fsmc_ctx* ctx, int32_t* reuse);
 int fsmc_ctx_set_pairing(fsmc_ctx* ctx, uint32_t mode);
 int fsmc_ctx_last_items(const fsmc_ctx* ctx, int32_t* n_items);
 int fsmc_ctx_set_two_wave_windows(fsmc_ctx* ctx, uint32_t mode);
```
